# lijx10/USIP

Measured on AMD Instinct MI355X. Metric: point-clouds/sec detector fwd+bwd, higher is better.
Workload: dtype f32 results; matrix-bound products emulated from 2 fp16 planes per operand (22-bit operands, 3 plane products, exact ...; 1 GPU; KITTI detector N=16384 M=512 K=64 batch=8 pairs/GPU (BASELINE configs[2]); detector=RPN_Detector_Ball, clouds_per_gpu=16, surface_normal_len=4, node_knn_k_1=16, ball_radius=2, ball_k=64, cloud=slab, matmul=f32x2, step=fwd+losses+bwd+adam, launch=HIP graph replay (ONE graph per step: forward, backward, Adam), parallelism=dp1

## Files before the change

### include/usip_hip.h

```cpp
#ifndef USIP_HIP_H
#define USIP_HIP_H

#include <stdint.h>

#ifdef __cplusplus
extern "C" {
#endif

#define USIP_OK      0
#define USIP_EINVAL (-1)

const char* usip_version(void);

enum { USIP_TUNE_INDEX_MAX_CH = 0, USIP_TUNE_INDEX_MAX_UNROLL, USIP_TUNE_X3_WGRAD_TILE, USIP_TUNE_X3_GEMM_TILE,
       USIP_TUNE_GEMM_SPLIT3, USIP_TUNE_INDEX_MAX_THREADS, USIP_TUNE_X2_DIRECT, USIP_TUNE_R5_FORMS, USIP_TUNE_COUNT };
int usip_set_tuning(const char* name, int value);
int usip_tuning_value(int knob);

int usip_launch_log(int on);
const char* usip_launch_log_entry(int i, unsigned* workgroups);

int usip_index_max_f32(const float* data, const int32_t* index, int32_t* max_idx,
                       int B, int C, int N, int K, void* stream);
int usip_index_max_geometry(int B, int C, int N, int K, int* channel_rows, int* prefetch_depth, int* threads);

int usip_index_max_f32_cpu(const float* data, const int32_t* index, int32_t* max_idx,
                           int B, int C, int N, int K, int num_threads);

int usip_ball_query_f32(const float* dist, int32_t* out_idx, float radius, int K,
                        int B, int M, int N, void* stream);

int usip_ball_query_f32_cpu(const float* dist, int32_t* out_idx, float radius, int K, int B, int M, int N);

int usip_pairwise_dist_f32_cpu(const float* a, const float* x, float* dist, int B, int M, int N);
int usip_pairwise_dist_f32(const float* a, const float* x, float* dist,
                           int B, int M, int N, void* stream);

int usip_ball_query_coords_f32(const float* node, const float* x, int32_t* out_idx, float radius,
                               int K, int B, int M, int N, void* stream);

int usip_som_assign_f32(const float* x, const float* node, int32_t* min_idx,
                        int B, int N, int M, void* stream);

int usip_som_cluster_f32(const float* x, const int32_t* min_idx, float* cluster_mean,
                         int32_t* count, float* x_decentered, int B, int N, int M, void* stream);
int usip_som_cluster_csr_f32(const float* x, const int32_t* min_idx, const int32_t* start, const int32_t* perm,
                             float* cluster_mean, int32_t* count, float* x_decentered, int B, int N, int M,
                             void* stream);

int usip_index_max_values_f32(const float* data, const int32_t* index, const int32_t* count, int32_t* max_idx,
                              float* max_val, int B, int C, int Ctot, int N, int K, void* stream);
int usip_index_max_values_backward_add_f32(const float* g, const int32_t* max_idx, const int32_t* count, float* ddata,
                                           int B, int C, int Ctot, int coff, int N, int K, void* stream);
int usip_index_max_values_backward_f32(const float* g, const int32_t* max_idx, const int32_t* count,
                                       const int32_t* index, const float* src, int Csrc, int soff, float* dz,
                                       int B, int C, int N, int K, void* stream);

int usip_csr_by_index_i32(const int32_t* idx, int32_t* start, int32_t* perm, int B, int P, int N, void* stream);
int usip_segment_sum_supported(int N, int P);
int usip_segment_sum_f32(const float* src, const int32_t* start, const int32_t* perm, float* dx,
                         int B, int C, int N, int P, int Ctot, int coff, void* stream);

long long usip_nearest_workspace(int B, int Ma, int Nb);
int usip_nearest_f32(const float* a, const float* b, float* min_d, int32_t* arg,
                     float* ws_d, int32_t* ws_j, int B, int Ma, int Nb, void* stream);
int usip_nearest_backward_f32(const float* a, const float* b, const float* d, const int32_t* arg,
                              const float* gd, float* ga, float* gb, int B, int C, int Ma, int Nb, void* stream);

int usip_detector_head_f32(const float* ks, const float* centre, float sigma_lower_bound, float* keypoints,
                           float* sigmas, int B, int M, void* stream);
int usip_detector_head_backward_f32(const float* g_keypoints, const float* g_sigmas, const float* ks, float* g_ks,
                                    int B, int M, void* stream);
int usip_rigid_transform_f32(const float* x, const float* R, const float* scale, const float* shift, float* out,
                             int transpose, int B, int M, void* stream);
int usip_detector_loss_combine_f32(const float* d, const float* chamfer, float alpha, float* out3, long long half,
                                   void* stream);
int usip_fill_scaled_f32(const float* g, float factor, float* out, long long n, void* stream);

int usip_adam_step_f32(float* param, const float* grad, float* exp_avg, float* exp_avg_sq, float* step_count,
                       float lr, float beta1, float beta2, float eps, long long n, void* stream);
int usip_adam_step_hyper_f32(float* param, const float* grad, float* exp_avg, float* exp_avg_sq, float* step_count,
                             const float* hyper, long long n, void* stream);

int usip_bn_group_dy_sum_f32(const float* gsum0, const float* gsum1, const float* coef4, float* out,
                             int nb, int C, int G, int K, void* stream);

int usip_chamfer_prob_f32(const float* a, const int32_t* J, const float* c, const int32_t* I,
                          const float* sigma_src, const float* sigma_dst, float* out3,
                          int B, int M, int N, void* stream);
int usip_chamfer_prob_backward_f32(const float* gloss, const float* a, const int32_t* J, const float* c,
                                   const int32_t* I, const float* sigma_src, const float* sigma_dst,
                                   float* da, float* dc, float* dsigma_src, float* dsigma_dst,
                                   int B, int M, int N, void* stream);

int usip_nearest_nd_f32(const float* a, const float* b, float* min_d, int32_t* arg,
                        int B, int C, int Ma, int Nb, void* stream);

int usip_mlp_gemm_tiles(int M, int P, int nb);
int usip_mlp_gemm_f32(const float* At, int lda, const float* X, const float* X2, const float* coef,
                      int pro, const float* bias, const float* rowbias, int rb_group,
                      const float* pool_dp, const int32_t* pool_arg, int pool_group,
                      float* Y, int y_rows, float* stats, int M, int K, int P, int nb, void* stream);
int usip_mlp_gemm_bf16(const float* At, int lda, const float* X, const float* X2, const float* coef,
                       int pro, const float* bias, const float* rowbias, int rb_group,
                       const float* pool_dp, const int32_t* pool_arg, int pool_group,
                        float* Y, int y_rows, float* stats, int M, int K, int P, int nb, void* stream);
int usip_mlp_gemm_f32x3(const float* At, int lda, const float* X, const float* X2, const float* coef,
                       int pro, const float* bias, const float* rowbias, int rb_group,
                       const float* pool_dp, const int32_t* pool_arg, int pool_group,
                        float* Y, int y_rows, float* stats, int M, int K, int P, int nb, void* stream);
int usip_mlp_gemm_f32x3_used(int M, int K, int P, int nb);
int usip_mlp_narrow_forward_blocks(int M, int K, int P, int nb);
int usip_mlp_narrow_forward_f32(const float* At, int lda, const float* X, const float* coef, int pro,
                                const float* bias, const float* rowbias, int rb_group, float* Y, int y_rows,
                                float* stats, int M, int K, int P, int nb, void* stream);

int usip_mlp_x3p_tile_rows(int M, int P, int nb);
typedef struct usip_split3_desc {
    const float* At; void* planes; int32_t lda, M, K, first_block;
    int32_t tile_rows, reserved;
} usip_split3_desc;
int usip_mlp_split3_blocks(int M, int K, int tile_rows);
int usip_mlp_split3_multi_f32(const usip_split3_desc* descs_device, int n, int total_blocks, void* stream);
int usip_mlp_x3p_tile_cols(int M, int P, int nb, int pro, int with_stats);
long long usip_mlp_split3_bytes(int M, int K);
int usip_mlp_split3_f32(const float* At, int lda, int M, int K, int tile_rows, void* planes, void* stream);
int usip_mlp_gemm_x3p_f32(const void* planes, const float* X, const float* X2, const float* coef, int pro,
                          const float* bias, const float* rowbias, int rb_group, const float* pool_dp,
                          const int32_t* pool_arg, int pool_group, float* Y, int y_rows, float* stats,
                          int M, int K, int P, int nb, void* stream);
int usip_mlp_split2h_f32(const float* At, int lda, int M, int K, int tile_rows, void* planes, void* stream);
int usip_mlp_gemm_x2h_f32(const void* planes, const float* X, const float* X2, const float* coef, int pro,
                          const float* bias, const float* rowbias, int rb_group, const float* pool_dp,
                          const int32_t* pool_arg, int pool_group, float* Y, int y_rows, float* stats,
                          int M, int K, int P, int nb, void* stream);

int usip_mlp_gemm_x2d_red_tiles(int M, int K, int P, int nb, int red_group);
int usip_mlp_gemm_x2h_red_f32(const void* planes, const float* X, const float* X2, const float* coef, int pro,
                              const float* pool_dp, const int32_t* pool_arg, int pool_group, float* Y,
                              const float* red_y, const float* red_coef, float* red_out, float* red_gsum,
                              int red_group, int M, int K, int P, int nb, void* stream);
int usip_mlp_gemm_x2r_tiles(int P, int nb);
int usip_mlp_gemm_x2r_f32(const void* planes, const float* X, const float* X2, const float* coef, int pro,
                          const float* bias, const float* rowbias, int rb_group, const float* pool_dp,
                          const int32_t* pool_arg, int pool_group, float* Y, int y_rows, float* stats, int M, int K,
                          int P, int nb, void* stream);

int usip_multi_transpose_f32(const float* src, float* dst, const int32_t* table, int ntensors, int total_tiles,
                             void* stream);

int usip_bn_finalize_f32(const float* stats, int tiles, int C, long long count,
                         const float* gamma, const float* beta, float eps, float momentum,
                         float* running_mean, float* running_var, float* mean, float* invstd,
                         float* coef, void* stream);

int usip_bn_apply_f32(const float* Y, const float* coef, float* Z, int relu,
                      int nb, int C, int P, void* stream);

int usip_bn_backward_reduce_f32(const float* dZ, const float* Y, const float* coef_fwd,
                                const float* mean, const float* invstd, const float* gamma, int relu,
                                float* partial, float* dgamma, float* dbeta, float* coef4,
                                float* gsum, int group, int nb, int C, int P, int want_bound, void* stream);


int usip_bn_pool_backward_reduce_f32(const float* dpooled, const int32_t* arg, const float* Y, const float* yarg,
                                     const float* coef_fwd, const float* mean, const float* invstd,
                                     const float* gamma, int relu, float* partial, float* dgamma, float* dbeta,
                                     float* coef4, int nb, int C, int M, int K, int want_bound, void* stream);

long long usip_mlp_wgrad_workspace(int M, int N, int P, int nb);
int usip_mlp_wgrad_f32(const float* G, const float* G2, const float* coef, int pro, const float* X,
                       const float* xcoef, const float* pool_dp, const int32_t* pool_arg, int pool_group,
                       float* workspace, float* dW, int ldw, int coloff,
                       int M, int N, int P, int nb, void* stream);
int usip_wgrad_defer(int on);
int usip_wgrad_defer_on(void* stream);
int usip_wgrad_defer_hold(int hold);
int usip_wgrad_flush(void* stream);

int usip_mlp_narrow_backward_supported(int Cin, int Cout, int P);
long long usip_mlp_narrow_backward_workspace(int Cout, int P, int nb);
int usip_mlp_narrow_backward_blocks(int Cout, int P, int nb);
int usip_mlp_narrow_backward_f32(const float* dZ, const float* Y, const float* coef4, const float* X, int x_rows,
                                 const float* xcoef, const float* W, int ldw, float* dX, int dx_rows,
                                 float* workspace, float* dW, int lddw, float* red_partial, int Cin, int Cout,
                                 int P, int nb, void* stream);

int usip_mlp_layer_backward_x2h_supported(int Cin, int Cout, int P, int pooled);
long long usip_mlp_layer_backward_x2h_workspace(int Cin, int Cout, int P, int nb);
int usip_mlp_layer_backward_x2h_blocks(int Cin, int Cout, int P, int nb);
int usip_mlp_layer_backward_x2h_f32(const float* dZ, const float* Y, const float* coef4, const float* pool_dp,
                                    const int32_t* pool_arg, int pool_group, const float* X, int x_rows,
                                    const float* xcoef, const void* planes, float* dX, int dx_rows, float* workspace,
                                    float* dW, int lddw, float* red_partial, float* group_sums, int Cin, int Cout,
                                    int P, int nb, void* stream);
int usip_mlp_layer_backward_x2h_ws_f32(const float* dZ, const float* Y, const float* coef4, const float* X, int x_rows,
                                       const float* xcoef, const void* planes, float* dX, int dx_rows, float* workspace,
                                       float* dW, int lddw, float* red_partial, const float* wsrc, int ws_rows,
                                       float* wsum, float* wsum3, int Cin, int Cout, int P, int nb, void* stream);
int usip_mlp_wsum_finalize_f32(const float* wsum, const float* wsum3, int blocks, int C, const float* coef4,
                               const float* mean, int ws_rows, float* dW, int lddw, void* stream);
int usip_bn_backward_finalize_f32(const float* partial, int rows, int C, long long count, const float* coef_fwd,
                                  const float* mean, const float* invstd, float* dgamma, float* dbeta, float* coef4,
                                  void* stream);
int usip_bn_backward_finalize_max_f32(const float* partial, int rows, int C, long long count, const float* coef_fwd,
                                      const float* mean, const float* invstd, float* dgamma, float* dbeta,
                                      float* coef4, const float* max0, int n0, const float* max1, int n1, void* stream);
int usip_mlp_wgrad_bf16(const float* G, const float* G2, const float* coef, int pro, const float* X,
                        const float* xcoef, const float* pool_dp, const int32_t* pool_arg, int pool_group,
                        float* workspace, float* dW, int ldw, int coloff,
                        int M, int N, int P, int nb, void* stream);
int usip_mlp_wgrad_f32x3(const float* G, const float* G2, const float* coef, int pro, const float* X,
                        const float* xcoef, const float* pool_dp, const int32_t* pool_arg, int pool_group,
                        float* workspace, float* dW, int ldw, int coloff,
                        int M, int N, int P, int nb, void* stream);
int usip_mlp_wgrad_x2h_f32(const float* G, const float* G2, const float* coef, int pro, const float* X,
                        const float* xcoef, const float* pool_dp, const int32_t* pool_arg, int pool_group,
                        float* workspace, float* dW, int ldw, int coloff,
                        int M, int N, int P, int nb, void* stream);
int usip_mlp_wgrad_f32x3_used(int M, int N, int P, int nb);

int usip_group_gather_f32(const float* x, const int32_t* idx, const float* sub, float* out,
                          int B, int C, int N, int M, int K, int nsub, int Ctot, int coff, void* stream);
int usip_group_gather_backward_f32(const float* dout, const int32_t* idx, float* dx,
                                   int B, int C, int N, int M, int K, int Ctot, int coff, void* stream);
int usip_group_max_f32(const float* z, float* pooled, int32_t* arg, long long rows, int K, void* stream);
int usip_group_max_act_f32(const float* y, const float* coef, int relu, float* pooled, int32_t* arg, float* yarg,
                           int B, int C, int M, int K, void* stream);
int usip_group_max_backward_f32(const float* dpooled, const int32_t* arg, float* dz,
                                long long rows, int K, void* stream);
int usip_group_max_backward_add_f32(const float* dpooled, const int32_t* arg, float* dz,
                                    long long rows, int K, void* stream);

int usip_knn_f32(const float* query, const float* database, int32_t* idx,
                 int B, int M, int N, int K, void* stream);

int usip_knn_layer_supported(int N, int M, int K);
int usip_knn_layer_forward_f32(const float* U, const float* W, int ldw, const float* database, const float* query,
                               const int32_t* idx, float* Y, float* stats, int B, int Cout, int N, int M, int K,
                               void* stream);
int usip_knn_layer_backward_f32(const float* dZ, const float* Y, const float* coef4, int relu, const float* dcoord,
                                const int32_t* start, const int32_t* perm, float* dU, float* dWc_part,
                                int B, int Cout, int N, int M, int K, void* stream);

int usip_knn_points_f32(const float* node, const float* x, int32_t* idx, int B, int M, int N, int K, void* stream);

int usip_fps_f32(const float* pts, const int32_t* first_idx, int32_t* out_idx, int B, int n, int k, void* stream);

int usip_nms_f32(const float* keypoints, const float* sigmas, float radius, int32_t* order, int32_t* count,
                 int B, int M, void* stream);

#define USIP_PAIRS_NPARAM 24
typedef struct usip_pairs_recipe {
    double aug_scale_lo, aug_scale_hi;
    double shift_range;
    double height_lo, height_hi;
    double pc_sigma, pc_clip;
    double sn_sigma, sn_clip;
    double node_sigma, node_clip;
    double pert_sigma, pert_clip;
    double dst_scale_thre, dst_shift_thre;
    int N, M, Cs, n_sub, row_len;
    int sn_last;
    int train;
    int rot_horizontal, rot_3d, rot_perturbation, translation_perturbation;
    int height_scaling;
    int enu_to_cam;
    int require_full;
    int dst_rot_type;
    int dst_rot_perturbation;
} usip_pairs_recipe;
typedef struct usip_pairs_draws {
    const int32_t* rows;
    const int32_t* cand;
    const int32_t* first;
    const double* jit_pc;
    const double* jit_sn;
    const double* jit_node;
    const double* params;
} usip_pairs_draws;
typedef struct usip_pairs_out {
    float* pc[2];
    float* sn[2];
    float* node[2];
    float* R;
    float* scale;
    float* shift;
    int32_t* rows;
    int32_t* node_slots;
} usip_pairs_out;
long long usip_pairs_workspace_bytes(const usip_pairs_recipe* recipe, int P);
long long usip_pairs_workspace_offset(const usip_pairs_recipe* recipe, int P, int part);
int usip_pairs_build_f32(const usip_pairs_recipe* recipe, const float* bank, const int64_t* offsets, int num_scans,
                         const int32_t* scan_ids, int P, long long min_rows, uint64_t seed, uint64_t step,
// ... 247 lines not shown
```

### usip_amd/_lib.py

```python
import ctypes
import os

_HERE = os.path.dirname(os.path.abspath(__file__))
LIB_PATH = os.environ.get("USIP_LIB") or os.path.join(_HERE, "libusip_hip.so")
ABI = 6
_lib = None

_f32p = ctypes.c_void_p
_i32p = ctypes.c_void_p
_int = ctypes.c_int
_flt = ctypes.c_float
_dbl = ctypes.c_double
_stream = ctypes.c_void_p

SIGNATURES = {
    "usip_version": ([], ctypes.c_char_p),
    "usip_set_tuning": ([ctypes.c_char_p, _int], _int),
    "usip_tuning_value": ([_int], _int),
    "usip_launch_log": ([_int], _int),
    "usip_launch_log_entry": ([_int, ctypes.POINTER(ctypes.c_uint)], ctypes.c_char_p),
    "usip_wgrad_defer": ([_int], _int),
    "usip_wgrad_defer_on": ([_stream], _int),
    "usip_wgrad_defer_hold": ([_int], _int),
    "usip_wgrad_flush": ([_stream], _int),
    "usip_index_max_f32": ([_f32p, _i32p, _i32p, _int, _int, _int, _int, _stream], _int),
    "usip_index_max_geometry": ([_int, _int, _int, _int] + [ctypes.POINTER(_int)] * 3, _int),
    "usip_index_max_f32_cpu": ([_f32p, _i32p, _i32p, _int, _int, _int, _int, _int], _int),
    "usip_ball_query_f32": ([_f32p, _i32p, _flt, _int, _int, _int, _int, _stream], _int),
    "usip_ball_query_f32_cpu": ([_f32p, _i32p, _flt, _int, _int, _int, _int], _int),
    "usip_pairwise_dist_f32_cpu": ([_f32p, _f32p, _f32p, _int, _int, _int], _int),
    "usip_pairwise_dist_f32": ([_f32p, _f32p, _f32p, _int, _int, _int, _stream], _int),
    "usip_som_assign_f32": ([_f32p, _f32p, _i32p, _int, _int, _int, _stream], _int),
    "usip_som_cluster_f32": ([_f32p, _i32p, _f32p, _i32p, _f32p, _int, _int, _int, _stream], _int),
    "usip_som_cluster_csr_f32": ([_f32p, _i32p, _i32p, _i32p, _f32p, _i32p, _f32p, _int, _int, _int, _stream], _int),
    "usip_index_max_values_f32": ([_f32p, _i32p, _i32p, _i32p, _f32p, _int, _int, _int, _int, _int, _stream], _int),
    "usip_index_max_values_backward_add_f32": ([_f32p, _i32p, _i32p, _f32p, _int, _int, _int, _int, _int, _int,
                                                _stream], _int),
    "usip_index_max_values_backward_f32": ([_f32p, _i32p, _i32p, _i32p, _f32p, _int, _int, _f32p, _int, _int, _int, _int,
                                            _stream], _int),
    "usip_mlp_narrow_forward_blocks": ([_int, _int, _int, _int], _int),
    "usip_mlp_narrow_forward_f32": ([_f32p, _int, _f32p, _f32p, _int, _f32p, _f32p, _int, _f32p, _int, _f32p, _int, _int,
                                     _int, _int, _stream], _int),
    "usip_detector_head_f32": ([_f32p, _f32p, _flt, _f32p, _f32p, _int, _int, _stream], _int),
    "usip_detector_head_backward_f32": ([_f32p, _f32p, _f32p, _f32p, _int, _int, _stream], _int),
    "usip_rigid_transform_f32": ([_f32p, _f32p, _f32p, _f32p, _f32p, _int, _int, _int, _stream], _int),
    "usip_detector_loss_combine_f32": ([_f32p, _f32p, _flt, _f32p, ctypes.c_longlong, _stream], _int),
    "usip_fill_scaled_f32": ([_f32p, _flt, _f32p, ctypes.c_longlong, _stream], _int),
    "usip_mlp_split3_blocks": ([_int, _int, _int], _int),
    "usip_mlp_split3_multi_f32": ([ctypes.c_void_p, _int, _int, _stream], _int),
    "usip_bn_group_dy_sum_f32": ([_f32p, _f32p, _f32p, _f32p, _int, _int, _int, _int, _stream], _int),
    "usip_csr_by_index_i32": ([_i32p, _i32p, _i32p, _int, _int, _int, _stream], _int),
    "usip_segment_sum_supported": ([_int, _int], _int),
    "usip_segment_sum_f32": ([_f32p, _i32p, _i32p, _f32p, _int, _int, _int, _int, _int, _int, _stream], _int),
    "usip_nearest_backward_f32": ([_f32p, _f32p, _f32p, _i32p, _f32p, _f32p, _f32p, _int, _int, _int, _int, _stream],
                                  _int),
    "usip_nearest_nd_f32": ([_f32p, _f32p, _f32p, _i32p, _int, _int, _int, _int, _stream], _int),
    "usip_chamfer_prob_f32": ([_f32p, _i32p, _f32p, _i32p, _f32p, _f32p, _f32p, _int, _int, _int, _stream], _int),
    "usip_chamfer_prob_backward_f32": ([_f32p, _f32p, _i32p, _f32p, _i32p, _f32p, _f32p, _f32p, _f32p, _f32p, _f32p,
                                        _int, _int, _int, _stream], _int),
    "usip_nearest_workspace": ([_int, _int, _int], ctypes.c_longlong),
    "usip_nearest_f32": ([_f32p, _f32p, _f32p, _i32p, _f32p, _i32p, _int, _int, _int, _stream], _int),
    "usip_mlp_gemm_tiles": ([_int, _int, _int], _int),
    "usip_mlp_gemm_f32": ([_f32p, _int, _f32p, _f32p, _f32p, _int, _f32p, _f32p, _int, _f32p, _i32p, _int,
                           _f32p, _int, _f32p, _int, _int, _int, _int, _stream], _int),
    "usip_mlp_gemm_bf16": ([_f32p, _int, _f32p, _f32p, _f32p, _int, _f32p, _f32p, _int, _f32p, _i32p, _int,
                            _f32p, _int, _f32p, _int, _int, _int, _int, _stream], _int),
    "usip_mlp_gemm_f32x3": ([_f32p, _int, _f32p, _f32p, _f32p, _int, _f32p, _f32p, _int, _f32p, _i32p, _int,
                             _f32p, _int, _f32p, _int, _int, _int, _int, _stream], _int),
    "usip_mlp_gemm_f32x3_used": ([_int, _int, _int, _int], _int),
    "usip_mlp_x3p_tile_rows": ([_int, _int, _int], _int),
    "usip_mlp_x3p_tile_cols": ([_int, _int, _int, _int, _int], _int),
    "usip_mlp_split3_bytes": ([_int, _int], ctypes.c_longlong),
    "usip_mlp_split3_f32": ([_f32p, _int, _int, _int, _int, ctypes.c_void_p, _stream], _int),
    "usip_mlp_gemm_x3p_f32": ([ctypes.c_void_p, _f32p, _f32p, _f32p, _int, _f32p, _f32p, _int, _f32p, _i32p, _int,
                               _f32p, _int, _f32p, _int, _int, _int, _int, _stream], _int),
    "usip_mlp_gemm_x2r_tiles": ([_int, _int], _int),
    "usip_mlp_gemm_x2r_f32": ([ctypes.c_void_p, _f32p, _f32p, _f32p, _int, _f32p, _f32p, _int, _f32p, _i32p, _int, _f32p,
                               _int, _f32p, _int, _int, _int, _int, _stream], _int),
    "usip_mlp_split2h_f32": ([_f32p, _int, _int, _int, _int, ctypes.c_void_p, _stream], _int),
    "usip_mlp_gemm_x2h_f32": ([ctypes.c_void_p, _f32p, _f32p, _f32p, _int, _f32p, _f32p, _int, _f32p, _i32p, _int,
                               _f32p, _int, _f32p, _int, _int, _int, _int, _stream], _int),
    "usip_mlp_gemm_x2d_red_tiles": ([_int, _int, _int, _int, _int], _int),
    "usip_mlp_gemm_x2h_red_f32": ([ctypes.c_void_p, _f32p, _f32p, _f32p, _int, _f32p, _i32p, _int, _f32p, _f32p, _f32p, _f32p,
                                   _f32p, _int, _int, _int, _int, _int, _stream], _int),
    "usip_mlp_wgrad_f32x3_used": ([_int, _int, _int, _int], _int),
    "usip_bn_pool_backward_reduce_f32": ([_f32p, _i32p, _f32p, _f32p, _f32p, _f32p, _f32p, _f32p, _int, _f32p, _f32p,
                                          _f32p, _f32p, _int, _int, _int, _int, _int, _stream], _int),
    "usip_bn_finalize_f32": ([_f32p, _int, _int, ctypes.c_longlong, _f32p, _f32p, _flt, _flt, _f32p, _f32p, _f32p,
                              _f32p, _f32p, _stream], _int),
    "usip_bn_apply_f32": ([_f32p, _f32p, _f32p, _int, _int, _int, _int, _stream], _int),
    "usip_bn_backward_reduce_f32": ([_f32p, _f32p, _f32p, _f32p, _f32p, _f32p, _int, _f32p, _f32p, _f32p, _f32p,
                                     _f32p, _int, _int, _int, _int, _int, _stream], _int),
    "usip_mlp_wgrad_workspace": ([_int, _int, _int, _int], ctypes.c_longlong),
    "usip_mlp_wgrad_f32": ([_f32p, _f32p, _f32p, _int, _f32p, _f32p, _f32p, _i32p, _int, _f32p, _f32p, _int, _int,
                            _int, _int, _int, _int, _stream], _int),
    "usip_mlp_wgrad_bf16": ([_f32p, _f32p, _f32p, _int, _f32p, _f32p, _f32p, _i32p, _int, _f32p, _f32p, _int, _int,
                             _int, _int, _int, _int, _stream], _int),
    "usip_mlp_wgrad_f32x3": ([_f32p, _f32p, _f32p, _int, _f32p, _f32p, _f32p, _i32p, _int, _f32p, _f32p, _int, _int,
                              _int, _int, _int, _int, _stream], _int),
    "usip_mlp_wgrad_x2h_f32": ([_f32p, _f32p, _f32p, _int, _f32p, _f32p, _f32p, _i32p, _int, _f32p, _f32p, _int, _int,
                                _int, _int, _int, _int, _stream], _int),
    "usip_mlp_narrow_backward_supported": ([_int, _int, _int], _int),
    "usip_mlp_narrow_backward_workspace": ([_int, _int, _int], ctypes.c_longlong),
    "usip_mlp_narrow_backward_blocks": ([_int, _int, _int], _int),
    "usip_mlp_layer_backward_x2h_supported": ([_int, _int, _int, _int], _int),
    "usip_mlp_layer_backward_x2h_workspace": ([_int, _int, _int, _int], ctypes.c_longlong),
    "usip_mlp_layer_backward_x2h_blocks": ([_int, _int, _int, _int], _int),
    "usip_mlp_layer_backward_x2h_f32": ([_f32p, _f32p, _f32p, _f32p, _i32p, _int, _f32p, _int, _f32p, ctypes.c_void_p,
                                         _f32p, _int, _f32p, _f32p, _int, _f32p, _f32p, _int, _int, _int, _int, _stream],
                                        _int),
    "usip_mlp_layer_backward_x2h_ws_f32": ([_f32p, _f32p, _f32p, _f32p, _int, _f32p, ctypes.c_void_p, _f32p, _int, _f32p,
                                            _f32p, _int, _f32p, _f32p, _int, _f32p, _f32p, _int, _int, _int, _int, _stream],
                                           _int),
    "usip_mlp_wsum_finalize_f32": ([_f32p, _f32p, _int, _int, _f32p, _f32p, _int, _f32p, _int, _stream], _int),
    "usip_mlp_narrow_backward_f32": ([_f32p, _f32p, _f32p, _f32p, _int, _f32p, _f32p, _int, _f32p, _int, _f32p, _f32p,
                                      _int, _f32p, _int, _int, _int, _int, _stream], _int),
    "usip_bn_backward_finalize_f32": ([_f32p, _int, _int, ctypes.c_longlong, _f32p, _f32p, _f32p, _f32p, _f32p, _f32p,
                                       _stream], _int),
    "usip_bn_backward_finalize_max_f32": ([_f32p, _int, _int, ctypes.c_longlong, _f32p, _f32p, _f32p, _f32p, _f32p, _f32p,
                                           _f32p, _int, _f32p, _int, _stream], _int),
    "usip_group_max_act_f32": ([_f32p, _f32p, _int, _f32p, _i32p, _f32p, _int, _int, _int, _int, _stream], _int),
    "usip_group_gather_f32": ([_f32p, _i32p, _f32p, _f32p, _int, _int, _int, _int, _int, _int, _int, _int,
                               _stream], _int),
    "usip_group_gather_backward_f32": ([_f32p, _i32p, _f32p, _int, _int, _int, _int, _int, _int, _int, _stream], _int),
    "usip_group_max_f32": ([_f32p, _f32p, _i32p, ctypes.c_longlong, _int, _stream], _int),
    "usip_group_max_backward_f32": ([_f32p, _i32p, _f32p, ctypes.c_longlong, _int, _stream], _int),
    "usip_group_max_backward_add_f32": ([_f32p, _i32p, _f32p, ctypes.c_longlong, _int, _stream], _int),
    "usip_multi_transpose_f32": ([_f32p, _f32p, _i32p, _int, _int, _stream], _int),
    "usip_adam_step_f32": ([_f32p, _f32p, _f32p, _f32p, _f32p, _flt, _flt, _flt, _flt, ctypes.c_longlong, _stream], _int),
    "usip_adam_step_hyper_f32": ([_f32p, _f32p, _f32p, _f32p, _f32p, _f32p, ctypes.c_longlong, _stream], _int),
    "usip_knn_f32": ([_f32p, _f32p, _i32p, _int, _int, _int, _int, _stream], _int),
    "usip_knn_points_f32": ([_f32p, _f32p, _i32p, _int, _int, _int, _int, _stream], _int),
    "usip_knn_layer_supported": ([_int, _int, _int], _int),
    "usip_knn_layer_forward_f32": ([_f32p, _f32p, _int, _f32p, _f32p, _i32p, _f32p, _f32p, _int, _int, _int, _int, _int,
                                    _stream], _int),
    "usip_knn_layer_backward_f32": ([_f32p, _f32p, _f32p, _int, _f32p, _i32p, _i32p, _f32p, _f32p, _int, _int, _int, _int,
                                     _int, _stream], _int),
    "usip_fps_f32": ([_f32p, _i32p, _i32p, _int, _int, _int, _stream], _int),
    "usip_nms_f32": ([_f32p, _f32p, _flt, _i32p, _i32p, _int, _int, _stream], _int),
    "usip_ball_query_coords_f32": ([_f32p, _f32p, _i32p, _flt, _int, _int, _int, _int, _stream], _int),
    "usip_pairs_workspace_bytes": ([ctypes.c_void_p, _int], ctypes.c_longlong),
    "usip_pairs_workspace_offset": ([ctypes.c_void_p, _int, _int], ctypes.c_longlong),
    "usip_pairs_build_f32": ([ctypes.c_void_p, _f32p, ctypes.c_void_p, _int, _i32p, _int, ctypes.c_longlong,
                              ctypes.c_uint64, ctypes.c_uint64, ctypes.c_longlong, ctypes.c_void_p, ctypes.c_void_p,
                              _stream], _int),
    "usip_pairs_apply_f32": ([ctypes.c_void_p, ctypes.c_void_p, _f32p, ctypes.c_void_p, _int, _i32p, _int,
                              ctypes.c_longlong, ctypes.c_void_p, ctypes.c_void_p, _stream], _int),
    "usip_pairs_build_f32_cpu": ([ctypes.c_void_p, ctypes.c_void_p, _f32p, ctypes.c_void_p, _int, _i32p, _int,
                                  ctypes.c_uint64, ctypes.c_uint64, ctypes.c_longlong, ctypes.c_void_p], _int),
    "usip_ransac_trials_f32": ([_f32p, _f32p, _i32p, _int, _int, _int, _dbl, ctypes.c_uint64, ctypes.c_void_p, _i32p,
                                ctypes.c_void_p, _i32p, _stream], _int),
    "usip_ransac_trials_explicit_f32": ([_f32p, _f32p, _i32p, _int, _int, _int, _dbl, _i32p, _i32p, ctypes.c_void_p,
                                         _stream], _int),
    "usip_ransac_select_f32": ([_f32p, _f32p, _i32p, _int, _int, _int, _int, _dbl, ctypes.c_uint64, ctypes.c_void_p,
                                _i32p, _i32p] + [ctypes.c_void_p] * 9 + [_stream], _int),
    "usip_compare_transform_f64": ([ctypes.c_void_p] * 2 + [_int] + [ctypes.c_void_p] * 2 + [_stream], _int),
    "usip_repeatability_f32": ([_f32p, _i32p, _f32p, _i32p, ctypes.c_void_p, _dbl, _int, _int, _int, ctypes.c_void_p,
                                _i32p, ctypes.c_void_p, _stream], _int),
    "usip_nearest_nd_counted_f32": ([_f32p, _f32p, _i32p, _i32p, _f32p, _i32p, _int, _int, _int, _int, _stream], _int),
    "usip_ransac_trials_f32_cpu": ([_f32p, _f32p, _i32p, _int, _int, _int, _dbl, ctypes.c_uint64, ctypes.c_void_p, _i32p,
                                    _i32p, ctypes.c_void_p, _i32p, _int], _int),
    "usip_ransac_select_f32_cpu": ([_f32p, _f32p, _i32p, _int, _int, _int, _int, _dbl, ctypes.c_uint64, ctypes.c_void_p,
                                    _i32p, _i32p] + [ctypes.c_void_p] * 9, _int),
    "usip_compare_transform_f64_cpu": ([ctypes.c_void_p] * 2 + [_int] + [ctypes.c_void_p] * 2, _int),
    "usip_repeatability_f32_cpu": ([_f32p, _i32p, _f32p, _i32p, ctypes.c_void_p, _dbl, _int, _int, _int, ctypes.c_void_p,
                                    _i32p, ctypes.c_void_p], _int),
    "usip_nearest_nd_counted_f32_cpu": ([_f32p, _f32p, _i32p, _i32p, _f32p, _i32p, _int, _int, _int, _int], _int),
    "usip_scan_knn_f32": ([_f32p, _i32p, _int, _int, _i32p, _i32p, _stream], _int),
    "usip_scan_normals_f32": ([_f32p, _i32p, _int, _int, ctypes.c_void_p, ctypes.c_void_p, _f32p, _stream], _int),
    "usip_scan_voxel_keys_f32": ([_f32p, _int, _f32p, _dbl, ctypes.c_void_p, _stream], _int),
    "usip_scan_voxel_average_f32": ([_f32p, ctypes.c_void_p, _i32p, _i32p, _int, _int, _f32p, _stream], _int),
    "usip_scan_knn_f32_cpu": ([_f32p, _int, _int, _i32p, _int], _int),
    "usip_scan_normals_f32_cpu": ([_f32p, _i32p, _int, _int, ctypes.c_void_p, ctypes.c_void_p, _f32p], _int),
    "usip_scan_voxel_keys_f32_cpu": ([_f32p, _int, _f32p, _dbl, ctypes.c_void_p], _int),
    "usip_scan_voxel_average_f32_cpu": ([_f32p, ctypes.c_void_p, _i32p, _i32p, _int, _int, _f32p], _int),
    "usip_desc_pairs_workspace_bytes": ([ctypes.c_void_p, _int], ctypes.c_longlong),
    "usip_desc_pairs_workspace_offset": ([ctypes.c_void_p, _int, _int], ctypes.c_longlong),
    "usip_desc_pairs_build_f32": ([ctypes.c_void_p, ctypes.c_void_p, _i32p, _int, ctypes.c_uint64, ctypes.c_uint64,
                                   ctypes.c_longlong, ctypes.c_void_p, ctypes.c_void_p, _stream], _int),
    "usip_desc_pairs_apply_f32": ([ctypes.c_void_p, ctypes.c_void_p, ctypes.c_void_p, _i32p, _int, ctypes.c_void_p,
                                   ctypes.c_void_p, _stream], _int),
    "usip_desc_pairs_build_f32_cpu": ([ctypes.c_void_p, ctypes.c_void_p, ctypes.c_void_p, _i32p, _int, ctypes.c_uint64,
                                       ctypes.c_uint64, ctypes.c_longlong, ctypes.c_void_p], _int),
    "usip_knn_nd_counted_f32": ([_f32p, _f32p, _i32p, _i32p, _int, _f32p, _i32p, _i32p, _int, _int, _int, _int, _stream],
                                _int),
    "usip_match_union_i32": ([_i32p] * 4 + [_int] * 4 + [_i32p, _i32p, _stream], _int),
    "usip_information_f32": ([_f32p, ctypes.c_void_p, _int, _int, ctypes.c_void_p, _stream], _int),
    "usip_overlap_keys_f32": ([_f32p, _int, ctypes.c_void_p, _int, ctypes.c_longlong, _i32p, ctypes.c_void_p, _int, _int,
                               ctypes.c_void_p, _stream], _int),
    "usip_overlap_ratio_f32": ([_f32p, _int, ctypes.c_void_p, _int, ctypes.c_longlong, _i32p, _i32p, ctypes.c_void_p, _i32p,
                                _i32p, _int, _int, _dbl, _i32p, ctypes.c_void_p, _stream], _int),
    "usip_knn_nd_counted_f32_cpu": ([_f32p, _f32p, _i32p, _i32p, _int, _f32p, _i32p, _i32p, _int, _int, _int, _int, _int],
                                    _int),
    "usip_match_union_i32_cpu": ([_i32p] * 4 + [_int] * 4 + [_i32p, _i32p], _int),
    "usip_information_f32_cpu": ([_f32p, ctypes.c_void_p, _int, _int, ctypes.c_void_p], _int),
    "usip_overlap_keys_f32_cpu": ([_f32p, _int, ctypes.c_void_p, _int, ctypes.c_longlong, _i32p, ctypes.c_void_p, _int, _int,
                                   ctypes.c_void_p], _int),
    "usip_overlap_ratio_f32_cpu": ([_f32p, _int, ctypes.c_void_p, _int, ctypes.c_longlong, _i32p, _i32p, ctypes.c_void_p,
                                    _i32p, _i32p, _int, _int, _dbl, _int, _i32p, ctypes.c_void_p, _int], _int),
    "usip_iss_saliency_f32": ([_f32p, _i32p, _i32p, _int, _int, _dbl, _dbl, _dbl, _int, ctypes.c_void_p, _i32p, _i32p,
                               _stream], _int),
    "usip_iss_nms_f32": ([_f32p, _i32p, _i32p, ctypes.c_void_p, _int, _int, _dbl, _int, ctypes.c_void_p, _stream], _int),
    "usip_iss_saliency_f32_cpu": ([_f32p, _i32p, _int, _int, _dbl, _dbl, _dbl, _int, ctypes.c_void_p, _i32p, _int], _int),
    "usip_iss_nms_f32_cpu": ([_f32p, _i32p, ctypes.c_void_p, _int, _int, _dbl, _int, ctypes.c_void_p, _int], _int),
    "usip_fgr_tuples_f32": ([_f32p, _f32p] + [_i32p] * 4 + [_int, _int, ctypes.c_uint64, ctypes.c_void_p, _i32p, _i32p,
                            ctypes.c_void_p, _i32p, _i32p, _i32p, _i32p, _int, _stream], _int),
    "usip_fgr_tuples_explicit_f32": ([_f32p, _f32p] + [_i32p] * 4 + [_int, _int, _i32p, _int, _i32p, _i32p, ctypes.c_void_p,
                                     _i32p, _i32p, _i32p, _stream], _int),
    "usip_fgr_optimize_f32": ([_f32p, _f32p, _i32p, _i32p, ctypes.c_void_p, _i32p, _i32p, _int, _int, _dbl]
                              + [ctypes.c_void_p] * 3 + [_i32p, _stream], _int),
    "usip_fgr_tuples_f32_cpu": ([_f32p, _f32p] + [_i32p] * 4 + [_int, _int, ctypes.c_uint64, ctypes.c_void_p, _i32p, _int,
                                _i32p, _i32p, ctypes.c_void_p, _i32p, _i32p, _i32p, _i32p, _int, _int], _int),
    "usip_fgr_tuples_explicit_f32_cpu": ([_f32p, _f32p] + [_i32p] * 4 + [_int, _int, _i32p, _int, _i32p, _i32p,
                                         ctypes.c_void_p, _i32p, _i32p, _i32p, _int], _int),
    "usip_fgr_optimize_f32_cpu": ([_f32p, _f32p, _i32p, _i32p, ctypes.c_void_p, _i32p, _i32p, _int, _int, _dbl]
                                  + [ctypes.c_void_p] * 3 + [_i32p, _int], _int),
    "usip_fgr_sincos_f64_cpu": ([ctypes.c_void_p, _int, ctypes.c_void_p, ctypes.c_void_p], _int),
    "usip_icp_workspace_bytes": ([_int, _int], ctypes.c_longlong),
    "usip_icp_nearest_f32": ([_f32p, _int, ctypes.c_void_p, _int, ctypes.c_longlong, _i32p, _i32p, _i32p]
                             + [ctypes.c_void_p] * 2 + [_i32p, _int, _int, _i32p, ctypes.c_void_p, ctypes.c_void_p, _stream],
                             _int),
    "usip_icp_refine_f32": ([_f32p, _int, ctypes.c_void_p, _int, ctypes.c_longlong, _i32p, _i32p, _i32p]
                            + [ctypes.c_void_p] * 2 + [_i32p, _int, _int, _dbl, _int, _dbl, _dbl, _dbl, ctypes.c_void_p,
                                                       ctypes.c_longlong, ctypes.c_void_p, _i32p, ctypes.c_void_p,
                                                       ctypes.c_void_p, _i32p, ctypes.c_void_p, ctypes.c_void_p, _i32p,
                                                       ctypes.c_void_p, ctypes.c_void_p, _stream], _int),
    "usip_icp_nearest_f32_cpu": ([_f32p, _int, ctypes.c_void_p, _int, ctypes.c_longlong, _i32p, _i32p, _i32p]
                                 + [ctypes.c_void_p] * 2 + [_i32p, _int, _int, _i32p, ctypes.c_void_p, _int], _int),
    "usip_icp_refine_f32_cpu": ([_f32p, _int, ctypes.c_void_p, _int, ctypes.c_longlong, _i32p, _i32p, _i32p]
                                + [ctypes.c_void_p] * 2 + [_i32p, _int, _int, _dbl, _int, _dbl, _dbl, _dbl, ctypes.c_void_p,
                                                           _i32p, ctypes.c_void_p, ctypes.c_void_p, _i32p, ctypes.c_void_p,
                                                           ctypes.c_void_p, _i32p, _i32p, ctypes.c_void_p, _int], _int),
    "usip_icp_information_f32": ([_f32p, _int, ctypes.c_void_p, _int, ctypes.c_longlong, _i32p, _i32p, _i32p]
                                 + [ctypes.c_void_p] * 2 + [_int, _int, _dbl, ctypes.c_void_p, _i32p, _stream], _int),
    "usip_posegraph_workspace_bytes": ([_int, _int, _int], ctypes.c_longlong),
    "usip_posegraph_optimize_f64": ([_i32p] * 4 + [ctypes.c_void_p] * 3 + [_int, _int, _int, _dbl, _dbl, _int, _int,
                                                                           ctypes.c_void_p, ctypes.c_longlong]
# ... 80 lines not shown
```

### usip_amd/csrc/gemm_x2f.hip

```cpp
#include "mlp_common.h"
#include "split_common.h"
#include <type_traits>

using namespace usip_mlp;

namespace {

constexpr int FBM = 256, FBN = 256, FNT = 256, FSLOTS = 4;
constexpr int FPL = FBM * 32;
constexpr int FSTAGE = 2 * FPL;
constexpr int FTRS = 68;
constexpr int FSCR_FLOATS = 4 * 2 * 32 * FTRS + 2 * 4 * FBM;

__device__ __forceinline__ int f_lds_off(int row, int half) { return row * 32 + ((half ^ (row >> 3)) & 1) * 16; }

__device__ __forceinline__ void f_split_pair(float x, float y, unsigned& hi, unsigned& lo)
{
    const f32x2 v = {x, y};
    hi = __builtin_bit_cast(unsigned, __builtin_convertvector(v, f16x2));
    asm("v_fma_mixlo_f16 %0, %1, 1.0, -%2 op_sel_hi:[0,0,1]" : "=v"(lo) : "v"(x), "v"(hi));
    asm("v_fma_mixhi_f16 %0, %1, 1.0, -%2 op_sel:[0,0,1] op_sel_hi:[0,0,1]" : "+v"(lo) : "v"(y), "v"(hi));
}

typedef unsigned u32x4 __attribute__((ext_vector_type(4)));
typedef unsigned u32x2 __attribute__((ext_vector_type(2)));

__device__ __forceinline__ float f_aread(const f32x16& t, int r)
{
    float x;
    asm volatile("v_accvgpr_read_b32 %0, %1" : "=v"(x) : "a"(t[r]));
    return x;
}

__device__ __forceinline__ void stats_flush_x2f(const GemmArgs& a, const float* scratch, int m0, int tn128, int tpc128)
{
    const float* red = scratch + 4 * 2 * 32 * FTRS;
    const int tid = threadIdx.x;
    const long long ntn = (long long)a.nb * tpc128;
#pragma unroll
    for (int hf = 0; hf < 2; ++hf) {
        const float s = red[(2 * hf) * FBM + tid] + red[(2 * hf + 1) * FBM + tid];
        const float q = red[4 * FBM + (2 * hf) * FBM + tid] + red[4 * FBM + (2 * hf + 1) * FBM + tid];
        a.stats[(long long)(m0 + tid) * ntn + tn128 + hf] = s;
        a.stats[ntn * a.M + (long long)(m0 + tid) * ntn + tn128 + hf] = q;
    }
}

template <int EPI, bool RB>
__device__ __forceinline__ void epilogue_x2f(const GemmArgs& a, f32x16 (&acc)[8][2], float out_scale, float* scratch,
                                             int b, int m0, int p0, int prev_m0, int prev_tn128, int tpc128)
{
    if (EPI != EPI_NONE && prev_tn128 >= 0) {
        stats_flush_x2f(a, scratch, prev_m0, prev_tn128, tpc128);
        asm volatile("s_waitcnt lgkmcnt(0)" ::: "memory");
        __builtin_amdgcn_s_barrier();
        asm volatile("" ::: "memory");
    }
    const int tid = threadIdx.x, lane = tid & 63, c = lane & 31, half = lane >> 5;
    const int wave = __builtin_amdgcn_readfirstlane(tid >> 6);
    float* tr = scratch + wave * (2 * 32 * FTRS);
    float* red = scratch + 4 * 2 * 32 * FTRS;
    const int pw = p0 + wave * 64;
    const int rr = lane >> 4, cc = lane & 15;
    const __amdgpu_buffer_rsrc_t rY = __builtin_amdgcn_make_buffer_rsrc(
        (void*)(a.Y + (long long)b * a.y_rows * a.P), 0, (unsigned)a.y_rows * (unsigned)a.P * 4u, 0x00020000);
    const int st_voff = ((m0 + rr) * a.P + pw + 4 * cc) * 4;
    float* const trw = tr + c * FTRS + 8 * half;
    const float* const trr = tr + rr * FTRS + 4 * cc;
    const int ngrp = RB ? a.P / a.rb_group : 0;
    int grp[4];
#pragma unroll
    for (int g = 0; g < 4; ++g) grp[g] = RB ? (pw + 16 * g + 8 * half) / a.rb_group : 0;
    const float* rbp = RB ? a.rowbias + ((long long)b * a.M + m0 + c) * ngrp : nullptr;
    const float* biasp = a.bias ? a.bias + m0 + c : nullptr;
    const f32x2 os2 = {out_scale, out_scale};
    auto produce = [&](int i) {
#if defined(USIP_X2F_EXP) && USIP_X2F_EXP == 2
        return;
#endif
        const float bv = biasp ? biasp[i * 32] : 0.0f;
        float rb[4] = {0.f, 0.f, 0.f, 0.f};
        if (RB) {
#pragma unroll
            for (int g = 0; g < 4; ++g) rb[g] = rbp[(long long)i * 32 * ngrp + grp[g]];
        }
        f32x2 s2g[4], q2g[4];
        float* w = trw + (i & 1) * (32 * FTRS);
#pragma unroll
        for (int g = 0; g < 4; ++g) {
            f32x2 u[4];
#pragma unroll
            for (int e = 0; e < 4; ++e) {
#if defined(USIP_X2F_EXP) && USIP_X2F_EXP == 3
#pragma unroll
                for (int bk = 0; bk < 2; ++bk) {
                    float t = __builtin_fmaf(f_aread(acc[i][bk], 4 * g + e), out_scale, bv);
                    if (RB) t += rb[g];
                    u[e][bk] = t;
                }
                if (EPI == EPI_STATS) {
                    s2g[g] = (e == 0) ? u[e] : s2g[g] + u[e];
                    q2g[g] = (e == 0) ? u[e] * u[e] : __builtin_elementwise_fma(u[e], u[e], q2g[g]);
                }
                continue;
#endif
                const f32x2 av = {f_aread(acc[i][0], 4 * g + e), f_aread(acc[i][1], 4 * g + e)};
                u[e] = __builtin_elementwise_fma(av, os2, (f32x2){bv, bv});
                if (RB) u[e] = u[e] + (f32x2){rb[g], rb[g]};
                if (EPI == EPI_STATS) {
                    s2g[g] = (e == 0) ? u[e] : s2g[g] + u[e];
                    q2g[g] = (e == 0) ? u[e] * u[e] : __builtin_elementwise_fma(u[e], u[e], q2g[g]);
                }
            }
            *reinterpret_cast<float4*>(w + 16 * g) = make_float4(u[0][0], u[0][1], u[1][0], u[1][1]);
            *reinterpret_cast<float4*>(w + 16 * g + 4) = make_float4(u[2][0], u[2][1], u[3][0], u[3][1]);
        }
        if (EPI != EPI_NONE) {
            const f32x2 s2 = (s2g[0] + s2g[1]) + (s2g[2] + s2g[3]), q2 = (q2g[0] + q2g[1]) + (q2g[2] + q2g[3]);
            float s = s2[0] + s2[1], q = q2[0] + q2[1];
            s += __shfl_xor(s, 32);
            q += __shfl_xor(q, 32);
            if (half == 0) { red[wave * FBM + i * 32 + c] = s; red[4 * FBM + wave * FBM + i * 32 + c] = q; }
        }
    };
    produce(0);
#pragma unroll
    for (int i = 0; i < 8; ++i) {
        asm volatile("s_waitcnt lgkmcnt(0)" ::: "memory");
        float4 w[8];
        const float* r = trr + (i & 1) * (32 * FTRS);
#pragma unroll
        for (int k = 0; k < 8; ++k) w[k] = *reinterpret_cast<const float4*>(r + 4 * k * FTRS);
        __builtin_amdgcn_sched_barrier(0);
        if (i < 7) produce(i + 1);
        __builtin_amdgcn_sched_barrier(0);
#pragma unroll
        for (int k = 0; k < 8; ++k) {
            const u32x4 d = {__float_as_uint(w[k].x), __float_as_uint(w[k].y), __float_as_uint(w[k].z), __float_as_uint(w[k].w)};
#if defined(USIP_X2F_EXP) && USIP_X2F_EXP == 1
            asm volatile("" ::"v"(d));
#else
            __builtin_amdgcn_raw_buffer_store_b128(d, rY, st_voff, (i * 32 + 4 * k) * a.P * 4, st_aux<ST_X2F_FWD>());
#endif
        }
        asm volatile("s_nop 7" ::: "memory");
        __builtin_amdgcn_sched_barrier(0);
    }
}

__device__ __forceinline__ void epilogue_x2f_direct(const GemmArgs& a, f32x16 (&acc)[8][2], float out_scale, int b, int m0, int p0)
{
    const int tid = threadIdx.x, lane = tid & 63, c = lane & 31, half = lane >> 5;
    const int wave = __builtin_amdgcn_readfirstlane(tid >> 6);
    const __amdgpu_buffer_rsrc_t rY = __builtin_amdgcn_make_buffer_rsrc(
        (void*)(a.Y + (long long)b * a.y_rows * a.P), 0, (unsigned)a.y_rows * (unsigned)a.P * 4u, 0x00020000);
    const int voff = ((m0 + 4 * half) * a.P + p0 + wave * 64 + 2 * c) * 4;
    const int rowb = a.P * 4;
#pragma unroll
    for (int i = 0; i < 8; ++i) {
#pragma unroll
        for (int g = 0; g < 4; ++g) {
            u32x2 v[4];
#pragma unroll
            for (int e = 0; e < 4; ++e)
                v[e] = u32x2{__float_as_uint(f_aread(acc[i][0], 4 * g + e) * out_scale),
                             __float_as_uint(f_aread(acc[i][1], 4 * g + e) * out_scale)};
#pragma unroll
            for (int e = 0; e < 4; ++e)
                __builtin_amdgcn_raw_buffer_store_b64(v[e], rY, voff, (i * 32 + 8 * g + e) * rowb, st_aux<ST_X2F_DGRAD>());
            asm volatile("s_nop 7" ::: "memory");
            __builtin_amdgcn_sched_barrier(0);
        }
    }
}

__host__ __device__ constexpr int f_ns(int sl) { return (sl % 6) >= 2 ? (sl / 6) * 4 + (sl % 6) - 2 : -1; }

#ifdef USIP_X2F_TRACE
}
__device__ unsigned g_x2f_trace[8 * 4 * 128];
extern "C" int usip_x2f_trace_read(void* dst, void* stream)
{
    return (int)hipMemcpyFromSymbolAsync(dst, HIP_SYMBOL(g_x2f_trace), sizeof(unsigned) * 8 * 4 * 128, 0, hipMemcpyDeviceToDevice,
                                         (hipStream_t)stream);
}
namespace {
#define X2F_TP(REG_, IDX_)                                                                                      \
    {                                                                                                           \
        unsigned long long tt_;                                                                                 \
        asm volatile("s_memtime %0\n\ts_waitcnt lgkmcnt(0)" : "=&s"(tt_)::"memory");                            \
        unsigned keep_;                                                                                         \
        asm volatile("s_mov_b32 %1, m0\n\ts_mov_b32 m0, %3\n\ts_nop 0\n\tv_writelane_b32 %0, %2, m0\n\ts_mov_b32 m0, %1" \
                     : "+v"(REG_), "=&s"(keep_) : "s"((unsigned)tt_), "s"((int)(IDX_)));                        \
    }
#else
#define X2F_TP(REG_, IDX_)
#endif

template <int PRO, int EPI, bool DIRECT>
__global__ __launch_bounds__(FNT) __attribute__((amdgpu_waves_per_eu(1, 1))) void gemm_x2f_kernel(
    const GemmArgs a, const uint4* __restrict__ planes)
{
    constexpr bool POOL = (PRO == PRO_BN_BWD_POOL);
    constexpr bool TWO = (PRO == PRO_BN_BWD) || POOL;
    constexpr int NC = TWO ? 4 : 2;
    constexpr int KMAX = TWO ? 512 : 640;
    constexpr int KPAD = KMAX + 16;
    constexpr int RING = FSLOTS * FSTAGE;
    constexpr int SCR = DIRECT ? 64 : FSCR_FLOATS * 4;
    __shared__ __attribute__((aligned(16))) unsigned char smem[RING + SCR + NC * KPAD * 4];
    float* scr = reinterpret_cast<float*>(smem + RING);
    float* cf = reinterpret_cast<float*>(smem + RING + SCR);

    const int tid = threadIdx.x, lane = tid & 63, c = lane & 31, h = lane >> 5;
    const int wave = __builtin_amdgcn_readfirstlane(tid >> 6);

    const int tpc = a.P / FBN, nmt = a.M / FBM;
    const int total = a.nb * tpc * nmt;
    const int nk = a.K / XBK;

    float xs, out_scale;
    {
        float* redm = scr;
        float bnd = 0.f;
        if (PRO == PRO_AFFINE_RELU) {
            const float rn = sqrtf((float)a.nb * (float)a.P);
            for (int k = tid; k < a.K; k += FNT) {
                const float c0 = a.coef[k], c1 = a.coef[a.K + k], mu = a.coef[2 * a.K + k], is = a.coef[3 * a.K + k];
                bnd = fmaxf(bnd, fabsf(c0) / is * rn + fabsf(__builtin_fmaf(mu, c0, c1)));
            }
        } else {
            for (int i = tid; i < (a.K + 63) / 64; i += FNT) bnd = fmaxf(bnd, a.coef[4 * a.K + i]);
        }
#pragma unroll
        for (int off = 32; off > 0; off >>= 1) bnd = fmaxf(bnd, __shfl_xor(bnd, off));
        if (lane == 0) redm[wave] = bnd;
        __syncthreads();
        bnd = fmaxf(fmaxf(redm[0], redm[1]), fmaxf(redm[2], redm[3]));
        xs = pow2_scale(bnd, X2H_TOP);
        const float ws = __uint_as_float(planes[(long long)nmt * nk * (FSTAGE / 16)].x);
        out_scale = __uint_as_float(__builtin_amdgcn_readfirstlane(__float_as_uint(1.0f / (xs * ws))));
        for (int i = tid; i < nk * XBK * NC; i += FNT) {
            const int k = i / NC, j = i % NC;
            cf[i] = a.coef[j * a.K + k] * xs;
        }
        __syncthreads();
    }

    typedef int v4i32 __attribute__((ext_vector_type(4)));
    auto make_rsrc = [](const void* base, unsigned bytes) {
        const unsigned long long p = (unsigned long long)reinterpret_cast<uintptr_t>(base);
        return v4i32{(int)__builtin_amdgcn_readfirstlane((unsigned)p),
                     (int)__builtin_amdgcn_readfirstlane((unsigned)(p >> 32) & 0xffffu),
                     (int)__builtin_amdgcn_readfirstlane(bytes), 0x00020000};
    };
    const v4i32 rAv = make_rsrc(planes, (unsigned)nmt * (unsigned)nk * FSTAGE);
    const int a_voff = wave * 4096 + lane * 16;
    const unsigned ring_lds = (unsigned)reinterpret_cast<uintptr_t>((__attribute__((address_space(3))) unsigned char*)smem);
    const int pgrp = POOL ? a.P / a.pool_group : 0;
    const unsigned x_bytes = (unsigned)a.nb * (unsigned)a.K * (unsigned)a.P * 4u;
    const unsigned pool_bytes = (unsigned)a.nb * (unsigned)a.K * (unsigned)pgrp * 4u;
    const int rs = a.P * 4, rsg = pgrp * 4;
    const __amdgpu_buffer_rsrc_t rX = __builtin_amdgcn_make_buffer_rsrc((void*)(POOL ? a.X2 : a.X), 0, x_bytes, 0x00020000);
    const __amdgpu_buffer_rsrc_t rX2 = __builtin_amdgcn_make_buffer_rsrc((void*)(TWO ? a.X2 : a.X), 0, x_bytes, 0x00020000);
    const __amdgpu_buffer_rsrc_t rPd = __builtin_amdgcn_make_buffer_rsrc((void*)(POOL ? a.pool_dp : a.X), 0,
                                                                         POOL ? pool_bytes : 4u, 0x00020000);
    const __amdgpu_buffer_rsrc_t rPa = __builtin_amdgcn_make_buffer_rsrc((void*)(POOL ? (const float*)a.pool_arg : a.X), 0,
                                                                         POOL ? pool_bytes : 4u, 0x00020000);
    const int pl = wave * 64 + 2 * c;
    int xv[8], gv[POOL ? 8 : 1];
#pragma unroll
    for (int i = 0; i < 8; ++i) {
        xv[i] = pl * 4 + (h * 8 + i) * rs;
        if (POOL) gv[POOL ? i : 0] = (pl / a.pool_group) * 4 + (h * 8 + i) * rsg;
    }
    const int xkin = POOL ? pl % a.pool_group : 0;

    struct XSet { f32x2 rx[POOL ? 1 : 8]; float rd[POOL ? 8 : 1]; int rarg[POOL ? 8 : 1]; f32x2 ry[TWO ? 8 : 1]; };
    struct Frag { f16x8 lo, hi; };
    constexpr int NX = POOL ? 24 : (TWO ? 16 : 8);
    constexpr int BARRIER_VMCNT = 2 * NX + 4;
    static_assert(BARRIER_VMCNT <= 63, "vmcnt is six bits");

    const int fa0 = f_lds_off(c, h);
    const float4* cfl = reinterpret_cast<const float4*>(cf) + h * (8 * NC / 4);

    struct Tile { int b, m0, p0, tn128; int xo, go, wo; };
    auto tile_of = [&](int v) {
        int L = v;
        if ((total & 7) == 0) L = (v & 7) * (total >> 3) + (v >> 3);
        const int mt = L % nmt, tn = L / nmt;
        const int b = tn / tpc, pt = tn % tpc;
        const int p0 = pt * FBN;
        return Tile{b, mt * FBM, p0, (b * tpc + pt) * 2, (b * a.K * a.P + p0) * 4,
                    POOL ? (b * a.K * pgrp + p0 / a.pool_group) * 4 : 0, mt * nk * FSTAGE};
    };

    XSet xs0, xs1;
    auto dma_pair = [&](int wo, int kt, int pair) {
        const unsigned dst = ring_lds + (unsigned)((kt & (FSLOTS - 1)) * FSTAGE) + (unsigned)(wave * 4096) + (unsigned)(pair * 2048);
        unsigned keep;
        asm volatile("s_mov_b32 %0, m0\n\ts_mov_b32 m0, %1\n\ts_nop 0\n\t"
                     "buffer_load_dwordx4 %2, %3, %4 offen lds\n\t"
                     "buffer_load_dwordx4 %2, %3, %4 offen offset:1024 lds\n\t"
                     "s_mov_b32 m0, %0"
                     : "=&s"(keep) : "s"(dst), "v"(a_voff), "s"(rAv), "s"(wo + kt * FSTAGE + pair * 2048) : "memory");
    };
    auto load_x1 = [&](int so, int sg, XSet& S, int i) {
        if (POOL) {
            S.rd[POOL ? i : 0] = __builtin_bit_cast(float, __builtin_amdgcn_raw_buffer_load_b32(rPd, gv[POOL ? i : 0], sg, 0));
            S.rarg[POOL ? i : 0] = (int)__builtin_amdgcn_raw_buffer_load_b32(rPa, gv[POOL ? i : 0], sg, 0);
        } else {
            S.rx[POOL ? 0 : i] = __builtin_bit_cast(f32x2, __builtin_amdgcn_raw_buffer_load_b64(rX, xv[i], so, st_aux<(PRO >= PRO_BN_BWD) ? LD_X2F_DGRAD : LD_X2F_FWD>()));
        }
        if (TWO) S.ry[TWO ? i : 0] = __builtin_bit_cast(f32x2, __builtin_amdgcn_raw_buffer_load_b64(rX2, xv[i], so, st_aux<LD_X2F_DGRAD>()));
    };

    float4 cq[TWO ? 8 : 4];
    float cv[2][8];
    auto cf_read = [&](int kt, int i) { cq[i] = cfl[kt * (XBK * NC / 4) + i]; };
    auto conv_blk = [&](const XSet& S, int i, int bk) {
        if (TWO) {
            const float4 c4 = cq[TWO ? i : 0];
            float x;
            if (POOL) x = (S.rarg[POOL ? i : 0] == xkin + bk) ? S.rd[POOL ? i : 0] : 0.f;
            else x = S.rx[POOL ? 0 : i][bk];
            cv[bk][i] = pro_apply<PRO_BN_BWD>(x, S.ry[TWO ? i : 0][bk], c4.x, c4.y, c4.z, c4.w);
        } else {
            const float4 c4 = cq[TWO ? 0 : i / 2];
            cv[bk][i] = (i & 1) ? pro_apply<PRO_AFFINE_RELU>(S.rx[POOL ? 0 : i][bk], 0.f, c4.z, c4.w, 0.f, 0.f)
                                : pro_apply<PRO_AFFINE_RELU>(S.rx[POOL ? 0 : i][bk], 0.f, c4.x, c4.y, 0.f, 0.f);
        }
    };
    auto convert_all = [&](int kt, const XSet& S, unsigned (&ph)[2][4], unsigned (&pl_)[2][4]) {
#pragma unroll
        for (int i = 0; i < (TWO ? 8 : 4); ++i) cf_read(kt, i);
#pragma unroll
        for (int i = 0; i < 8; ++i) { conv_blk(S, i, 0); conv_blk(S, i, 1); }
#pragma unroll
        for (int bk = 0; bk < 2; ++bk)
#pragma unroll
            for (int j = 0; j < 4; ++j) f_split_pair(cv[bk][2 * j], cv[bk][2 * j + 1], ph[bk][j], pl_[bk][j]);
    };

    f32x16 acc[8][2];
    Frag FA, FB;
    auto read_frag = [&](int kt, int t, int which, Frag& F) {
        const unsigned char* As = smem + (kt & (FSLOTS - 1)) * FSTAGE + fa0 + t * 1024;
        if (which == 0) F.lo = *reinterpret_cast<const f16x8*>(As + FPL);
        else F.hi = *reinterpret_cast<const f16x8*>(As);
    };

    auto stage = [&](auto first_tag, int kt, int k1, int k3, int xo3, int go3, int wo3, XSet& S, const unsigned (&chh)[2][4],
                     const unsigned (&cll)[2][4], unsigned (&nh)[2][4], unsigned (&nl)[2][4]) {
        constexpr bool FIRST = decltype(first_tag)::value;
        const f16x8 xh0 = __builtin_bit_cast(f16x8, make_uint4(chh[0][0], chh[0][1], chh[0][2], chh[0][3]));
        const f16x8 xh1 = __builtin_bit_cast(f16x8, make_uint4(chh[1][0], chh[1][1], chh[1][2], chh[1][3]));
        const f16x8 xl0 = __builtin_bit_cast(f16x8, make_uint4(cll[0][0], cll[0][1], cll[0][2], cll[0][3]));
        const f16x8 xl1 = __builtin_bit_cast(f16x8, make_uint4(cll[1][0], cll[1][1], cll[1][2], cll[1][3]));
        const int so3 = xo3 + k3 * (XBK * rs), sg3 = go3 + k3 * (XBK * rsg);
        auto slot = [&](auto sl_tag) {
            constexpr int sl = decltype(sl_tag)::value;
            constexpr int t = sl / 6, i6 = sl % 6, bk = i6 & 1, prod = i6 / 2;
            if (sl == 42) {
                asm volatile("s_waitcnt vmcnt(%0) lgkmcnt(0)" ::"n"(BARRIER_VMCNT) : "memory");
                __builtin_amdgcn_s_barrier();
            }
            {
                Frag& F = (t & 1) ? FB : FA;
                const f16x8& x = (prod == 1) ? (bk ? xl1 : xl0) : (bk ? xh1 : xh0);
                const f16x8& f = (prod == 0) ? F.lo : F.hi;
                if constexpr (FIRST && prod == 0) {
                    if constexpr (DIRECT) asm volatile("v_mfma_f32_32x32x16_f16 %0, %2, %1, 0" : "=a"(acc[t][bk]) : "v"(x), "v"(f));
                    else asm volatile("v_mfma_f32_32x32x16_f16 %0, %1, %2, 0" : "=a"(acc[t][bk]) : "v"(x), "v"(f));
                } else {
                    if constexpr (DIRECT) asm volatile("v_mfma_f32_32x32x16_f16 %0, %2, %1, %0" : "+a"(acc[t][bk]) : "v"(x), "v"(f));
                    else asm volatile("v_mfma_f32_32x32x16_f16 %0, %1, %2, %0" : "+a"(acc[t][bk]) : "v"(x), "v"(f));
                }
            }
            if (i6 < 2) {
                if (t < 7) read_frag(kt, t + 1, i6, (t & 1) ? FA : FB);
                else read_frag(kt + 1, 0, i6, FA);
            }
            constexpr int ns = f_ns(sl);
            if (ns == 28) dma_pair(wo3, k3, 0);
            if (ns == 30) dma_pair(wo3, k3, 1);
            if (!TWO) {
                if (ns == 0) { cf_read(k1, 0); cf_read(k1, 1); cf_read(k1, 2); cf_read(k1, 3); }
#pragma unroll
                for (int j = 0; j < 4; ++j) {
                    const int base = 2 + 5 * j;
                    if (ns == base) { conv_blk(S, 2 * j, 0); conv_blk(S, 2 * j, 1); }
                    if (ns == base + 1) { conv_blk(S, 2 * j + 1, 0); conv_blk(S, 2 * j + 1, 1); }
                    if (ns == base + 2) {
                        f_split_pair(cv[0][2 * j], cv[0][2 * j + 1], nh[0][j], nl[0][j]);
                        load_x1(so3, sg3, S, 2 * j);
                    }
                    if (ns == base + 3) {
                        f_split_pair(cv[1][2 * j], cv[1][2 * j + 1], nh[1][j], nl[1][j]);
                        load_x1(so3, sg3, S, 2 * j + 1);
                    }
                }
            } else {
                if (ns == 0) { cf_read(k1, 0); cf_read(k1, 1); }
                if (ns == 1) { cf_read(k1, 2); cf_read(k1, 3); }
                if (ns == 8) cf_read(k1, 4);
                if (ns == 9) cf_read(k1, 5);
                if (ns == 14) cf_read(k1, 6);
                if (ns == 15) cf_read(k1, 7);
#pragma unroll
                for (int j = 0; j < 4; ++j) {
                    const int base = 2 + 6 * j;
                    if (ns == base) conv_blk(S, 2 * j, 0);
                    if (ns == base + 1) conv_blk(S, 2 * j, 1);
                    if (ns == base + 2) conv_blk(S, 2 * j + 1, 0);
                    if (ns == base + 3) conv_blk(S, 2 * j + 1, 1);
                    if (ns == base + 4) {
                        f_split_pair(cv[0][2 * j], cv[0][2 * j + 1], nh[0][j], nl[0][j]);
                        load_x1(so3, sg3, S, 2 * j);
                    }
                    if (ns == base + 5) {
                        f_split_pair(cv[1][2 * j], cv[1][2 * j + 1], nh[1][j], nl[1][j]);
                        load_x1(so3, sg3, S, 2 * j + 1);
                    }
                }
            }
            __builtin_amdgcn_sched_barrier(0);
        };
#define USIP_X2F_SLOT(N_) slot(std::integral_constant<int, N_>{});
#define USIP_X2F_SLOT6(N_) USIP_X2F_SLOT(N_) USIP_X2F_SLOT(N_ + 1) USIP_X2F_SLOT(N_ + 2) USIP_X2F_SLOT(N_ + 3) USIP_X2F_SLOT(N_ + 4) USIP_X2F_SLOT(N_ + 5)
        USIP_X2F_SLOT6(0) USIP_X2F_SLOT6(6) USIP_X2F_SLOT6(12) USIP_X2F_SLOT6(18)
        USIP_X2F_SLOT6(24) USIP_X2F_SLOT6(30) USIP_X2F_SLOT6(36) USIP_X2F_SLOT6(42)
#undef USIP_X2F_SLOT6
#undef USIP_X2F_SLOT
    };

    [[maybe_unused]] unsigned trp = 0, trs = 0;
    [[maybe_unused]] int tix = 0;
    int v = blockIdx.x;
    if (v >= total) return;
    unsigned ah[2][4], al[2][4], bh[2][4], bl[2][4];
    Tile T = tile_of(v);
    {
#pragma unroll
        for (int st = 0; st < 3; ++st) { dma_pair(T.wo, st, 0); dma_pair(T.wo, st, 1); }
#pragma unroll
        for (int i = 0; i < 8; ++i) load_x1(T.xo, T.go, xs0, i);
#pragma unroll
        for (int i = 0; i < 8; ++i) load_x1(T.xo + XBK * rs, T.go + XBK * rsg, xs1, i);
        convert_all(0, xs0, ah, al);
#pragma unroll
        for (int i = 0; i < 8; ++i) load_x1(T.xo + 2 * XBK * rs, T.go + 2 * XBK * rsg, xs0, i);
        asm volatile("s_waitcnt vmcnt(%0)" ::"n"(2 * NX) : "memory");
        __builtin_amdgcn_s_barrier();
        read_frag(0, 0, 0, FA); read_frag(0, 0, 1, FA);
    }
    int prev_m0 = 0, prev_tn128 = -1;
    for (;;) {
        const int vn = v + (int)gridDim.x;
        const bool more = vn < total;
        const Tile Tn = more ? tile_of(vn) : T;
        X2F_TP(trp, tix * 8 + 0)
        stage(std::true_type{}, 0, 1, 3, T.xo, T.go, T.wo, xs1, ah, al, bh, bl);
        stage(std::false_type{}, 1, 2, 4 < nk ? 4 : 0, 4 < nk ? T.xo : Tn.xo, 4 < nk ? T.go : Tn.go, 4 < nk ? T.wo : Tn.wo,
              xs0, bh, bl, ah, al);
        X2F_TP(trp, tix * 8 + 1)
        X2F_TP(trp, tix * 8 + 2)
        for (int kt = 2; kt < nk; kt += 2) {
            const bool w3 = kt + 3 >= nk, w4 = kt + 4 >= nk;
            stage(std::false_type{}, kt, kt + 1, w3 ? kt + 3 - nk : kt + 3, w3 ? Tn.xo : T.xo, w3 ? Tn.go : T.go, w3 ? Tn.wo : T.wo,
                  xs1, ah, al, bh, bl);
#ifdef USIP_X2F_TRACE
            if (tix == 1 && kt < 64) X2F_TP(trs, kt)
#endif
            stage(std::false_type{}, kt + 1, kt + 2 >= nk ? 0 : kt + 2, w4 ? kt + 4 - nk : kt + 4, w4 ? Tn.xo : T.xo, w4 ? Tn.go : T.go,
                  w4 ? Tn.wo : T.wo, xs0, bh, bl, ah, al);
#ifdef USIP_X2F_TRACE
            if (tix == 1 && kt < 63) X2F_TP(trs, kt + 1)
#endif
        }
        X2F_TP(trp, tix * 8 + 3)
        X2F_TP(trp, tix * 8 + 4)
        asm volatile("s_nop 7\n\ts_nop 7\n\ts_nop 7" ::: "memory");
        __builtin_amdgcn_sched_barrier(0);
        X2F_TP(trp, tix * 8 + 5)
        if constexpr (DIRECT) epilogue_x2f_direct(a, acc, out_scale, T.b, T.m0, T.p0);
        else if (a.rowbias) epilogue_x2f<EPI, true>(a, acc, out_scale, scr, T.b, T.m0, T.p0, prev_m0, prev_tn128, tpc * 2);
        else epilogue_x2f<EPI, false>(a, acc, out_scale, scr, T.b, T.m0, T.p0, prev_m0, prev_tn128, tpc * 2);
        prev_m0 = T.m0;
        prev_tn128 = T.tn128;
        X2F_TP(trp, tix * 8 + 6)
#ifdef USIP_X2F_TRACE
        ++tix;
#endif
        if (!more) break;
        v = vn;
        T = Tn;
    }
    if constexpr (!DIRECT && EPI != EPI_NONE) {
        asm volatile("s_waitcnt lgkmcnt(0)" ::: "memory");
        __builtin_amdgcn_s_barrier();
        asm volatile("" ::: "memory");
        stats_flush_x2f(a, scr, prev_m0, prev_tn128, tpc * 2);
    }
    asm volatile("s_waitcnt vmcnt(0)" ::: "memory");
#ifdef USIP_X2F_TRACE
    if (blockIdx.x < 8) {
        g_x2f_trace[(blockIdx.x * 4 + wave) * 128 + lane] = trp;
        g_x2f_trace[(blockIdx.x * 4 + wave) * 128 + 64 + lane] = trs;
    }
#endif
}

}

namespace usip_mlp {

bool gemm_x2f_takes(const GemmArgs& a, int pro)
{
    const int knob = usip_tuning_value(USIP_TUNE_X2_DIRECT);
    if (knob != 0 && (knob < 13 || knob > 15)) return false;
    if ((knob == 13 && pro != PRO_AFFINE_RELU) || (knob == 14 && pro == PRO_BN_BWD) || (knob == 15 && pro == PRO_BN_BWD_POOL)) return false;
    if (pro != PRO_AFFINE_RELU && pro != PRO_BN_BWD && pro != PRO_BN_BWD_POOL) return false;
    if (a.red_out) return false;
    if (a.M % FBM != 0 || a.P % FBN != 0 || a.K % (4 * XBK) != 0) return false;
    if (a.K > (pro == PRO_AFFINE_RELU ? 640 : 512)) return false;
    if (!a.y_vec || (a.rowbias && a.rb_group % 8 != 0)) return false;
    if ((long long)a.y_rows * a.P * 4 >= (1LL << 31) || (long long)a.nb * a.K * a.P * 4 >= (1LL << 31)) return false;
    if ((reinterpret_cast<uintptr_t>(a.X) & 7u) != 0 || (reinterpret_cast<uintptr_t>(a.X2) & 7u) != 0) return false;
    if (pro == PRO_BN_BWD_POOL && (a.pool_group % 2 != 0 || FBN % a.pool_group != 0)) return false;
    if (pro != PRO_AFFINE_RELU && (a.stats || a.bias || a.rowbias)) return false;
    return true;
}

int launch_gemm_x2f(const GemmArgs& a_in, const uint4* pl, int pro, hipStream_t st)
{
    const GemmArgs& a = a_in;
    const int tpc = a.P / FBN, nmt = a.M / FBM;
    const long long total = (long long)a.nb * tpc * nmt;
    if (total > 0x7fffffffLL) return USIP_EINVAL;
    const int cus = usip_cu_count();
    const long long slots = (long long)cus / 8 * 8;
    dim3 grid((unsigned)((total <= slots || (total & 7)) ? total : slots)), block(FNT);
    if (pro == PRO_AFFINE_RELU) {
        if (a.stats) USIP_LAUNCH((gemm_x2f_kernel<PRO_AFFINE_RELU, EPI_STATS, false>), grid, block, 0, st, a, pl);
        else USIP_LAUNCH((gemm_x2f_kernel<PRO_AFFINE_RELU, EPI_NONE, false>), grid, block, 0, st, a, pl);
    } else if (pro == PRO_BN_BWD) {
        USIP_LAUNCH((gemm_x2f_kernel<PRO_BN_BWD, EPI_NONE, true>), grid, block, 0, st, a, pl);
    } else {
        USIP_LAUNCH((gemm_x2f_kernel<PRO_BN_BWD_POOL, EPI_NONE, true>), grid, block, 0, st, a, pl);
    }
    USIP_LAUNCH_CHECK();
    return USIP_OK;
}

}
```

### usip_amd/csrc/mlp_common.h

```cpp
#pragma once
#include "common.h"

typedef float f32x16 __attribute__((ext_vector_type(16)));

namespace usip_mlp {

enum { ST_NARROW_FWD = 1, ST_X2R = 2, ST_TILE_EPI = 4, ST_X2F_FWD = 8, ST_X2F_DGRAD = 16, ST_X2D = 32, ST_LAYER_BWD_DX = 64,
       ST_WGRAD_PART = 128, LD_WGRAD_G = 256, ST_TILE_EPI_PLAIN = 512, LD_LAYER_BWD_G = 1024, LD_X2F_FWD = 2048,
       LD_X2F_DGRAD = 4096, LD_NARROW_FWD = 8192, LD_X2R = 16384, LD_WGRAD_X = 32768, LD_WGRAD3_G = 65536,
       LD_X3P_FWD = 131072, LD_LAYER_BWD_X = 262144, LD_BN_REDUCE_Z = 524288, LD_BN_REDUCE_Y = 1048576, LD_WGRAD_GEN_G = 2097152, ST_X2R_PLAIN = 4194304 };
#ifndef USIP_ST_NT
#define USIP_ST_NT (ST_X2F_DGRAD | ST_WGRAD_PART | LD_WGRAD_G | LD_LAYER_BWD_G | LD_X2F_FWD)
#endif
template <int SITE> constexpr int st_aux() { return (USIP_ST_NT & SITE) ? 2 : 0; }
typedef float st_f4v __attribute__((ext_vector_type(4)));
template <int SITE>
__device__ __forceinline__ void st_out(float* p, float v)
{
    if (USIP_ST_NT & SITE) __builtin_nontemporal_store(v, p); else *p = v;
}
template <int SITE>
__device__ __forceinline__ float4 ld_in4(const float* p)
{
    if (USIP_ST_NT & SITE) {
        const st_f4v q = __builtin_nontemporal_load(reinterpret_cast<const st_f4v*>(p));
        return make_float4(q.x, q.y, q.z, q.w);
    }
    return *reinterpret_cast<const float4*>(p);
}
template <int SITE>
__device__ __forceinline__ void st_out4(float* p, float x, float y, float z, float w)
{
    if (USIP_ST_NT & SITE) { st_f4v q = {x, y, z, w}; __builtin_nontemporal_store(q, reinterpret_cast<st_f4v*>(p)); }
    else *reinterpret_cast<float4*>(p) = make_float4(x, y, z, w);
}

enum { PRO_NONE = 0, PRO_AFFINE_RELU = 1, PRO_BN_BWD = 2, PRO_BN_BWD_POOL = 3 };

struct GemmArgs {
    const float* At; int lda;
    const float* X;
    const float* X2;
    const float* coef;
    const float* bias;
    float* Y;
    float* stats;
    int M, K, P, nb;
    const float* rowbias; int rb_group;
    const float* pool_dp; const int* pool_arg; int pool_group;
    int a_trans;
    int y_rows;
    int y_vec;
    const float* red_y; const float* red_coef; float* red_out; float* red_gsum; int red_group;
};

template <int PRO>
__device__ __forceinline__ float pro_apply(float x, float x2, float c0, float c1, float c2, float c3)
{
    if (PRO == PRO_AFFINE_RELU) return fmaxf(__builtin_fmaf(x, c0, c1), 0.0f);
    if (PRO == PRO_BN_BWD) {
        const float dyh = (__builtin_fmaf(x2, c0, c1) > 0.0f) ? x : 0.0f;
        return __builtin_fmaf(c0, dyh, __builtin_fmaf(c2, x2, c3));
    }
    return x;
}

enum { EPI_NONE = 0, EPI_STATS = 1 };

template <int WM, int WN, int EPI, int TM = 2, int NJ = 2>
__device__ __forceinline__ void gemm_epilogue(const GemmArgs& a, f32x16 (&acc)[TM][NJ], float* scratch,
                                              int scratch_floats, int b, int m0, int p0, int tn, int tpc)
{
    constexpr int BM = WM * 32 * TM, BN = WN * 32 * NJ;
    const int tid = threadIdx.x, lane = tid & 63, c = lane & 31, half = lane >> 5;
    const int wave = __builtin_amdgcn_readfirstlane(tid >> 6);
    const int wm = wave / WN, wn = wave % WN;
    float* Yb = a.Y + (long long)b * a.y_rows * a.P;
    float* red = scratch;
    const int ngrp = a.rowbias ? a.P / a.rb_group : 0;
    float* rbs = red + 2 * WN * BM;
    const int g0 = a.rowbias ? p0 / a.rb_group : 0;
    const int G = a.rowbias ? (min(p0 + BN, a.P) - 1) / a.rb_group - g0 + 1 : 0;
    const bool rb_lds = a.rowbias && BM * G <= scratch_floats - 2 * WN * BM;
    if (rb_lds) {
        for (int e = tid; e < BM * G; e += 256) {
            const int rl = e / G, g = e % G;
            rbs[e] = (m0 + rl < a.M) ? a.rowbias[((long long)b * a.M + m0 + rl) * ngrp + g0 + g] : 0.f;
        }
        __syncthreads();
    }
    const bool run_one_group = a.rowbias && (a.rb_group % 4 == 0);
#pragma unroll
    for (int i = 0; i < TM; ++i) {
        const int row_l = (wm * TM + i) * 32 + c;
        const int row = m0 + row_l;
        const int rowc = min(row, a.M - 1);
        const bool rok = row < a.M;
        const float bv = a.bias ? a.bias[rowc] : 0.0f;
        float* yrow = Yb + (long long)rowc * a.P;
        float s = 0.f, q = 0.f;
#pragma unroll
        for (int j = 0; j < NJ; ++j) {
#pragma unroll
            for (int g = 0; g < 4; ++g) {
                const int pb = p0 + wn * (32 * NJ) + j * 32 + 8 * g + 4 * half;
                float v[4];
#pragma unroll
                for (int e = 0; e < 4; ++e) v[e] = acc[i][j][4 * g + e] + bv;
                if (a.rowbias) {
                    if (run_one_group) {
                        const int grp = min(pb, a.P - 1) / a.rb_group;
                        const float rb = rb_lds ? rbs[row_l * G + grp - g0]
                                                : a.rowbias[((long long)b * a.M + rowc) * ngrp + grp];
#pragma unroll
                        for (int e = 0; e < 4; ++e) v[e] += rb;
                    } else {
#pragma unroll
                        for (int e = 0; e < 4; ++e) {
                            const int grp = min(pb + e, a.P - 1) / a.rb_group;
                            v[e] += rb_lds ? rbs[row_l * G + grp - g0]
                                           : a.rowbias[((long long)b * a.M + rowc) * ngrp + grp];
                        }
                    }
                }
                if (rok) {
                    if (a.y_vec && pb + 3 < a.P) {
                        st_out4<(EPI == EPI_STATS) ? ST_TILE_EPI : ST_TILE_EPI_PLAIN>(yrow + pb, v[0], v[1], v[2], v[3]);
                        if (EPI == EPI_STATS) {
#pragma unroll
                            for (int e = 0; e < 4; ++e) { s += v[e]; q = __builtin_fmaf(v[e], v[e], q); }
                        }
                    } else {
#pragma unroll
                        for (int e = 0; e < 4; ++e)
                            if (pb + e < a.P) {
                                yrow[pb + e] = v[e];
                                if (EPI == EPI_STATS) { s += v[e]; q = __builtin_fmaf(v[e], v[e], q); }
                            }
                    }
                }
            }
        }
        if (EPI != EPI_NONE) {
            s += __shfl_xor(s, 32); q += __shfl_xor(q, 32);
            if (half == 0) {
                red[wn * BM + row_l] = s;
                red[WN * BM + wn * BM + row_l] = q;
            }
        }
    }
    if (EPI != EPI_NONE) {
        __syncthreads();
        if (tid < BM && m0 + tid < a.M) {
            float s = 0.f, q = 0.f;
#pragma unroll
            for (int w = 0; w < WN; ++w) { s += red[w * BM + tid]; q += red[WN * BM + w * BM + tid]; }
            const long long ntn = (long long)a.nb * tpc;
            a.stats[(long long)(m0 + tid) * ntn + tn] = s;
            a.stats[ntn * a.M + (long long)(m0 + tid) * ntn + tn] = q;
        }
    }
}

struct WgradArgs {
    const float* G;  const float* G2; const float* coef;
    const float* X;
    const float* xcoef;
    const float* pool_dp; const int* pool_arg; int pool_group;
    float* part;
    int M, N, P, nb, seglen, segs;
};

template <int N4, bool TWO, bool VEC, int Q4 = 8>
__device__ __forceinline__ void wgrad_load_rows(const float* __restrict__ base, const float* __restrict__ base2,
                                                int rows, int P, int r0, int p, int pend, int tid,
                                                float4 (&dst)[N4], float4 (&dst2)[TWO ? N4 : 1])
{
#pragma unroll
    for (int i = 0; i < N4; ++i) {
        const int f = tid + i * 256, row = f / Q4, kq = (f % Q4) * 4;
        float4 v = make_float4(0.f, 0.f, 0.f, 0.f), w = v;
        if (VEC) {
            const long long off = (long long)min(r0 + row, rows - 1) * P + min(p + kq, P - 4);
            if (TWO) {
                v = ld_in4<LD_WGRAD_GEN_G>(base + off);
                w = ld_in4<LD_WGRAD_GEN_G>(base2 + off);
            } else {
                v = *reinterpret_cast<const float4*>(base + off);
            }
        } else if (r0 + row < rows) {
            const long long off = (long long)(r0 + row) * P + p + kq;
            if (p + kq + 0 < pend) { v.x = base[off + 0]; if (TWO) w.x = base2[off + 0]; }
            if (p + kq + 1 < pend) { v.y = base[off + 1]; if (TWO) w.y = base2[off + 1]; }
            if (p + kq + 2 < pend) { v.z = base[off + 2]; if (TWO) w.z = base2[off + 2]; }
            if (p + kq + 3 < pend) { v.w = base[off + 3]; if (TWO) w.w = base2[off + 3]; }
        }
        dst[i] = v;
        if (TWO) dst2[i] = w;
    }
}

template <int TM, int TN>
__device__ __forceinline__ void wgrad_store_partial(const WgradArgs& a, f32x16 (&acc)[TM][TN], int slice,
                                                    int m0, int n0, int wm, int wn, int lane)
{
    float* out = a.part + (long long)slice * a.M * a.N;
// ... 30 lines not shown
```

### usip_amd/csrc/shared_mlp_x3.hip

```cpp
#include "mlp_common.h"
#include "split_common.h"
#include <type_traits>

using namespace usip_mlp;

namespace {

__device__ __forceinline__ int lds_off(int row, int half) { return row * 32 + ((half ^ (row >> 3)) & 1) * 16; }

constexpr int X2H_PARTS = 32;

__device__ __forceinline__ float* x2h_trailer(const usip_split3_desc& d)
{
    const int bm = d.tile_rows, ksteps = (d.K + XBK - 1) / XBK;
    return reinterpret_cast<float*>(reinterpret_cast<unsigned char*>(d.planes) +
                                    (long long)((d.M + bm - 1) / bm) * ksteps * 2 * bm * 32);
}

__device__ __forceinline__ void absmax_part(const usip_split3_desc& d, int part)
{
    __shared__ float red[4];
    const long long total = (long long)d.M * d.K, per = (total + X2H_PARTS - 1) / X2H_PARTS;
    const long long i0 = part * per, i1 = i0 + per < total ? i0 + per : total;
    float mx = 0.f;
// ... 989 lines not shown
    const int t = usip_tuning_value(USIP_TUNE_X3_GEMM_TILE);
    if (M <= 128 || t == 1) return 128;
    const long long wide = (long long)((M + 255) / 256) * nb * ((P + 127) / 128);
    return wide >= 256 ? 256 : 128;
}


extern "C" long long usip_mlp_split3_bytes(int M, int K)
{
    if (M < 1 || K < 1) return 0;
    const int bm = M > 128 ? 256 : 128;
    return (long long)((M + bm - 1) / bm) * ((K + XBK - 1) / XBK) * 3 * bm * 32;
}

extern "C" int usip_mlp_split3_f32(const float* At, int lda, int M, int K, int tile_rows, void* planes, void* stream)
{
    if (!At || !planes || M < 1 || K < 1 || lda < M || (reinterpret_cast<uintptr_t>(planes) & 15u)) return USIP_EINVAL;
    if (tile_rows != 128 && tile_rows != 256) return USIP_EINVAL;
    const int bm = tile_rows;
    const int ksteps = (K + XBK - 1) / XBK, mts = (M + bm - 1) / bm;
    USIP_LAUNCH(split3_tiles_kernel, dim3((unsigned)(mts * ksteps)), dim3(2 * bm), 0, (hipStream_t)stream, At, lda, M, K,
                reinterpret_cast<uint4*>(planes), ksteps, bm, 3);
    USIP_LAUNCH_CHECK();
    return USIP_OK;
}

extern "C" int usip_mlp_split2h_f32(const float* At, int lda, int M, int K, int tile_rows, void* planes, void* stream)
{
    if (!At || !planes || M < 1 || K < 1 || lda < M || (reinterpret_cast<uintptr_t>(planes) & 15u)) return USIP_EINVAL;
    if (tile_rows != 128 && tile_rows != 256) return USIP_EINVAL;
    const int bm = tile_rows;
    const int ksteps = (K + XBK - 1) / XBK, mts = (M + bm - 1) / bm;
    usip_split3_desc d{At, planes, lda, M, K, 0, bm, 2};
    USIP_LAUNCH(absmax_one_kernel, dim3(X2H_PARTS), dim3(256), 0, (hipStream_t)stream, d);
    USIP_LAUNCH_CHECK();
    USIP_LAUNCH(split3_tiles_kernel, dim3((unsigned)(mts * ksteps)), dim3(2 * bm), 0, (hipStream_t)stream, At, lda, M, K,
                reinterpret_cast<uint4*>(planes), ksteps, bm, 2);
    USIP_LAUNCH_CHECK();
    return USIP_OK;
}

extern "C" int usip_mlp_split3_blocks(int M, int K, int tile_rows)
{
    if (M < 1 || K < 1 || (tile_rows != 128 && tile_rows != 256)) return 0;
    const int bm = tile_rows;
    return ((M + bm - 1) / bm) * ((K + XBK - 1) / XBK);
}

extern "C" int usip_mlp_split3_multi_f32(const usip_split3_desc* descs_device, int n, int total_blocks, void* stream)
{
    if (n < 0 || total_blocks < 0) return USIP_EINVAL;
    if (n == 0 || total_blocks == 0) return USIP_OK;
    if (!descs_device) return USIP_EINVAL;
    USIP_LAUNCH(absmax_multi_kernel, dim3((unsigned)(n * X2H_PARTS)), dim3(256), 0, (hipStream_t)stream, descs_device, n);
    USIP_LAUNCH_CHECK();
    USIP_LAUNCH(split3_multi_kernel, dim3((unsigned)total_blocks), dim3(512), 0, (hipStream_t)stream, descs_device, n);
    USIP_LAUNCH_CHECK();
    return USIP_OK;
}

template <int TM, int WN, int NPL = 3>
static int launch_x3p(const GemmArgs& a, const uint4* pl, int pro, hipStream_t st)
{
    constexpr int BM = 64 * TM, BN = 64 * WN;
    const int tpc = (a.P + BN - 1) / BN, nmt = (a.M + BM - 1) / BM;
    const long long total = (long long)a.nb * tpc * nmt;
    if (total > 0x7fffffffLL) return USIP_EINVAL;
    const int epi = a.stats ? EPI_STATS : EPI_NONE;
    dim3 grid((unsigned)total), block(128 * WN);
    const bool deep = TM == 2 && !(usip_tuning_value(USIP_TUNE_R5_FORMS) & 32);
#define USIP_X3P_CASE(P_, E_)                                                                 \
    if (pro == P_ && epi == E_) {                                                             \
        if constexpr (TM == 2) {                                                              \
            if (deep) {                                                                       \
                USIP_LAUNCH((gemm_x3p_kernel<P_, E_, TM, WN, NPL, 3>), grid, block, 0, st, a, pl); \
                USIP_LAUNCH_CHECK();                                                          \
                return USIP_OK;                                                               \
            }                                                                                 \
        }                                                                                     \
        USIP_LAUNCH((gemm_x3p_kernel<P_, E_, TM, WN, NPL>), grid, block, 0, st, a, pl);       \
        USIP_LAUNCH_CHECK();                                                                  \
        return USIP_OK;                                                                       \
    }
    if constexpr (NPL == 3) {
        USIP_X3P_CASE(PRO_NONE, EPI_STATS)
        USIP_X3P_CASE(PRO_NONE, EPI_NONE)
    }
    USIP_X3P_CASE(PRO_AFFINE_RELU, EPI_STATS)
    USIP_X3P_CASE(PRO_AFFINE_RELU, EPI_NONE)
    USIP_X3P_CASE(PRO_BN_BWD, EPI_NONE)
    USIP_X3P_CASE(PRO_BN_BWD_POOL, EPI_NONE)
#undef USIP_X3P_CASE
    return USIP_EINVAL;
}

extern "C" int usip_mlp_x3p_tile_cols(int M, int P, int nb, int pro, int with_stats)
{
    if (usip_mlp_x3p_tile_rows(M, P, nb) == 128 || with_stats) return 128;
    const int knob = usip_tuning_value(USIP_TUNE_X3_GEMM_TILE);
    const long long wide_tiles = (long long)((M + 255) / 256) * ((P + 255) / 256) * nb;
    return (knob == 4 || (knob == 5 && pro >= 2 && wide_tiles >= 256)) ? 256 : 128;
}

extern "C" int usip_mlp_gemm_x3p_f32(const void* planes, const float* X, const float* X2, const float* coef, int pro,
                                     const float* bias, const float* rowbias, int rb_group, const float* pool_dp,
                                     const int32_t* pool_arg, int pool_group, float* Y, int y_rows, float* stats,
                                     int M, int K, int P, int nb, void* stream)
{
    if (M < 1 || K < 1 || K > 640 || P < 0 || nb < 0) return USIP_EINVAL;
    if ((pro == PRO_BN_BWD || pro == PRO_BN_BWD_POOL) && K > 512) return USIP_EINVAL;
    if ((long long)P * nb == 0) return USIP_OK;
    if (!planes || !Y || pro < 0 || pro > 3 || (reinterpret_cast<uintptr_t>(planes) & 15u)) return USIP_EINVAL;
    if (pro != PRO_BN_BWD_POOL && !X) return USIP_EINVAL;
    if (pro != PRO_NONE && !coef) return USIP_EINVAL;
    if ((pro == PRO_BN_BWD || pro == PRO_BN_BWD_POOL) && (!X2 || stats)) return USIP_EINVAL;
    if (pro == PRO_BN_BWD_POOL && (!pool_dp || !pool_arg || pool_group < 1 || P % pool_group != 0)) return USIP_EINVAL;
    if (rowbias && (rb_group < 1 || P % rb_group != 0)) return USIP_EINVAL;
    if (y_rows == 0) y_rows = M;
    if (y_rows < M) return USIP_EINVAL;
    GemmArgs a{nullptr, 0, X, X2, coef, bias, Y, stats, M, K, P, nb, rowbias, rb_group, pool_dp, pool_arg, pool_group,
               0, y_rows, (P % 4 == 0 && (reinterpret_cast<uintptr_t>(Y) & 15u) == 0) ? 1 : 0};
    hipStream_t st = (hipStream_t)stream;
    const uint4* pl = reinterpret_cast<const uint4*>(planes);
    if (usip_mlp_x3p_tile_rows(M, P, nb) == 128) return launch_x3p<2, 2>(a, pl, pro, st);
    if (usip_mlp_x3p_tile_cols(M, P, nb, pro, stats != nullptr) == 256) return launch_x3p<4, 4>(a, pl, pro, st);
    return launch_x3p<4, 2>(a, pl, pro, st);
}

extern "C" int usip_mlp_gemm_x2h_f32(const void* planes, const float* X, const float* X2, const float* coef, int pro,
                                     const float* bias, const float* rowbias, int rb_group, const float* pool_dp,
                                     const int32_t* pool_arg, int pool_group, float* Y, int y_rows, float* stats,
                                     int M, int K, int P, int nb, void* stream)
{
    if (M < 1 || K < 1 || K > 640 || P < 0 || nb < 0) return USIP_EINVAL;
    if (pro != PRO_AFFINE_RELU && pro != PRO_BN_BWD && pro != PRO_BN_BWD_POOL) return USIP_EINVAL;
    if ((pro == PRO_BN_BWD || pro == PRO_BN_BWD_POOL) && K > 512) return USIP_EINVAL;
    if ((long long)P * nb == 0) return USIP_OK;
    if (!planes || !Y || !coef || (reinterpret_cast<uintptr_t>(planes) & 15u)) return USIP_EINVAL;
    if (pro != PRO_BN_BWD_POOL && !X) return USIP_EINVAL;
    if ((pro == PRO_BN_BWD || pro == PRO_BN_BWD_POOL) && (!X2 || stats)) return USIP_EINVAL;
    if (pro == PRO_BN_BWD_POOL && (!pool_dp || !pool_arg || pool_group < 1 || P % pool_group != 0)) return USIP_EINVAL;
    if (rowbias && (rb_group < 1 || P % rb_group != 0)) return USIP_EINVAL;
    if (y_rows == 0) y_rows = M;
    if (y_rows < M) return USIP_EINVAL;
    GemmArgs a{nullptr, 0, X, X2, coef, bias, Y, stats, M, K, P, nb, rowbias, rb_group, pool_dp, pool_arg, pool_group,
               0, y_rows, (P % 4 == 0 && (reinterpret_cast<uintptr_t>(Y) & 15u) == 0) ? 1 : 0};
    hipStream_t st = (hipStream_t)stream;
    const uint4* pl = reinterpret_cast<const uint4*>(planes);
    if (usip_mlp_x3p_tile_rows(M, P, nb) == 128) return launch_x3p<2, 2, 2>(a, pl, pro, st);
    if (usip_mlp_x3p_tile_cols(M, P, nb, pro, stats != nullptr) == 256) return launch_x3p<4, 4, 2>(a, pl, pro, st);
    if ((usip_tuning_value(USIP_TUNE_X2_DIRECT) & 15) != 1 && (long long)K * P * 4 < (1LL << 31))
        return launch_gemm_x2d(a, pl, pro, st);
    return launch_x3p<4, 2, 2>(a, pl, pro, st);
}

extern "C" int usip_mlp_gemm_x2d_red_tiles(int M, int K, int P, int nb, int red_group)
{
    if (M < 256 || M % 256 || P < 128 || P % 128 || nb < 1 || K < 1 || K > 512) return 0;
    if (red_group != 0 && red_group != 16 && red_group != 32) return 0;
    if (usip_mlp_x3p_tile_rows(M, P, nb) != 256 || usip_mlp_x3p_tile_cols(M, P, nb, 2, 0) != 128) return 0;
    if ((usip_tuning_value(USIP_TUNE_X2_DIRECT) & 15) == 1 || (usip_tuning_value(USIP_TUNE_X2_DIRECT) & 15) == 8) return 0;
    if ((long long)K * P * 4 >= (1LL << 31) || (long long)M * P * 4 >= (1LL << 31)) return 0;
    return nb * (P / 128);
}

extern "C" int usip_mlp_gemm_x2h_red_f32(const void* planes, const float* X, const float* X2, const float* coef, int pro,
                                         const float* pool_dp, const int32_t* pool_arg, int pool_group, float* Y,
                                         const float* red_y, const float* red_coef, float* red_out, float* red_gsum,
                                         int red_group, int M, int K, int P, int nb, void* stream)
{
    if (pro != PRO_BN_BWD && pro != PRO_BN_BWD_POOL) return USIP_EINVAL;
    if (!usip_mlp_gemm_x2d_red_tiles(M, K, P, nb, red_gsum ? red_group : 0)) return USIP_EINVAL;
    if (!planes || !Y || !coef || !X2 || !red_y || !red_coef || !red_out || (reinterpret_cast<uintptr_t>(planes) & 15u))
        return USIP_EINVAL;
    if ((reinterpret_cast<uintptr_t>(Y) | reinterpret_cast<uintptr_t>(red_y)) & 15u) return USIP_EINVAL;
    if (pro == PRO_BN_BWD && !X) return USIP_EINVAL;
    if (pro == PRO_BN_BWD_POOL && (!pool_dp || !pool_arg || pool_group < 1 || P % pool_group != 0)) return USIP_EINVAL;
    GemmArgs a{nullptr, 0, X, X2, coef, nullptr, Y, nullptr, M, K, P, nb, nullptr, 1, pool_dp, pool_arg, pool_group,
               0, M, 1, red_y, red_coef, red_out, red_gsum, red_gsum ? red_group : 0};
    return launch_gemm_x2d(a, reinterpret_cast<const uint4*>(planes), pro, (hipStream_t)stream);
}

extern "C" int usip_mlp_gemm_x2r_tiles(int P, int nb)
{
    const long long total = (long long)nb * ((P + 63) / 64);
    return (int)(total < 512 ? total : 512);
}

extern "C" int usip_mlp_gemm_x2r_f32(const void* planes, const float* X, const float* X2, const float* coef, int pro,
                                     const float* bias, const float* rowbias, int rb_group, const float* pool_dp,
                                     const int32_t* pool_arg, int pool_group, float* Y, int y_rows, float* stats, int M,
                                     int K, int P, int nb, void* stream)
{
    if (rowbias && (pro != PRO_AFFINE_RELU || rb_group < 32 || rb_group % 32 != 0 || P % rb_group != 0)) return USIP_EINVAL;
    if (M < 1 || M > 128 || K < 1 || K > 128 || P < 0 || nb < 0) return USIP_EINVAL;
    if (pro != PRO_AFFINE_RELU && pro != PRO_BN_BWD && pro != PRO_BN_BWD_POOL) return USIP_EINVAL;
    if ((long long)P * nb == 0) return USIP_OK;
    if (!planes || !Y || !coef || (reinterpret_cast<uintptr_t>(planes) & 15u)) return USIP_EINVAL;
    if (pro != PRO_BN_BWD_POOL && !X) return USIP_EINVAL;
    if ((pro == PRO_BN_BWD || pro == PRO_BN_BWD_POOL) && (!X2 || stats)) return USIP_EINVAL;
    if (pro == PRO_BN_BWD_POOL && (!pool_dp || !pool_arg || pool_group < 1 || P % pool_group != 0)) return USIP_EINVAL;
    if ((long long)K * P >= (1LL << 30)) return USIP_EINVAL;
    if (y_rows == 0) y_rows = M;
    if (y_rows < M) return USIP_EINVAL;
    GemmArgs a{nullptr, 0, X, X2, coef, bias, Y, stats, M, K, P, nb, rowbias, rowbias ? rb_group : 1, pool_dp, pool_arg,
               pool_group, 0, y_rows, (P % 4 == 0 && (reinterpret_cast<uintptr_t>(Y) & 15u) == 0) ? 1 : 0};
    const long long total = (long long)nb * ((P + 63) / 64);
    const unsigned grid = (unsigned)(total < 512 ? total : 512);
    hipStream_t st = (hipStream_t)stream;
    const uint4* pl = reinterpret_cast<const uint4*>(planes);
    if (pro == PRO_AFFINE_RELU && rowbias) {
        if (stats) USIP_LAUNCH((gemm_x2r_kernel<PRO_AFFINE_RELU, EPI_STATS, true>), dim3(grid), dim3(256), 0, st, a, pl);
        else USIP_LAUNCH((gemm_x2r_kernel<PRO_AFFINE_RELU, EPI_NONE, true>), dim3(grid), dim3(256), 0, st, a, pl);
    } else if (pro == PRO_AFFINE_RELU) {
        if (stats) USIP_LAUNCH((gemm_x2r_kernel<PRO_AFFINE_RELU, EPI_STATS>), dim3(grid), dim3(256), 0, st, a, pl);
        else USIP_LAUNCH((gemm_x2r_kernel<PRO_AFFINE_RELU, EPI_NONE>), dim3(grid), dim3(256), 0, st, a, pl);
    } else if (pro == PRO_BN_BWD) {
        USIP_LAUNCH((gemm_x2r_kernel<PRO_BN_BWD, EPI_NONE>), dim3(grid), dim3(256), 0, st, a, pl);
    } else {
        USIP_LAUNCH((gemm_x2r_kernel<PRO_BN_BWD_POOL, EPI_NONE>), dim3(grid), dim3(256), 0, st, a, pl);
    }
    USIP_LAUNCH_CHECK();
    return USIP_OK;
}

namespace usip_mlp {

void wgrad_x3_plan(int M, int N, int P, int nb, int* seglen, int* segs, int* tiles)
{
    *tiles = ((M + 255) / 256) * ((N + 255) / 256);
    long long want = (usip_tuning_value(USIP_TUNE_X3_WGRAD_TILE) == 2 ? 512 : 256) / (*tiles);
    if (want < 1) want = 1;
    long long per_cloud = (want + nb - 1) / nb;
    if (per_cloud < 1) per_cloud = 1;
    long long sl = (P + per_cloud - 1) / per_cloud;
    sl = ((sl + 31) / 32) * 32;
    long long floor_sl = 512;
    if (usip_tuning_value(USIP_TUNE_X3_WGRAD_TILE) != 4)
        while (floor_sl > 128 && (long long)(*tiles) * nb * ((P + floor_sl - 1) / floor_sl) < 192) floor_sl /= 2;
    if (sl < floor_sl) sl = floor_sl;
    *seglen = (int)sl;
    *segs = (int)((P + sl - 1) / sl);
}

int launch_wgrad_x2h_256(const WgradArgs& a, int pro, unsigned blocks, hipStream_t st)
{
    dim3 grid(blocks), block(512);
    const bool line = !(usip_tuning_value(USIP_TUNE_R5_FORMS) & 1) &&
                      (long long)(a.M > a.N ? a.M : a.N) * a.P < (1LL << 30);
    if (line && pro == PRO_BN_BWD) { USIP_LAUNCH((wgrad_x2l_kernel<PRO_BN_BWD>), grid, block, 0, st, a); USIP_LAUNCH_CHECK(); return USIP_OK; }
    if (line && pro == PRO_BN_BWD_POOL) { USIP_LAUNCH((wgrad_x2l_kernel<PRO_BN_BWD_POOL>), grid, block, 0, st, a); USIP_LAUNCH_CHECK(); return USIP_OK; }
    if (pro == PRO_BN_BWD) USIP_LAUNCH((wgrad_x3_kernel<PRO_BN_BWD, true, 2>), grid, block, 0, st, a);
    else if (pro == PRO_BN_BWD_POOL) USIP_LAUNCH((wgrad_x3_kernel<PRO_BN_BWD_POOL, true, 2>), grid, block, 0, st, a);
    else return USIP_EINVAL;
    USIP_LAUNCH_CHECK();
    return USIP_OK;
}

int launch_wgrad_x3_256(const WgradArgs& a, int pro, bool xpro, unsigned blocks, hipStream_t st)
{
    dim3 grid(blocks), block(512);
#define USIP_X3W_CASE(P_, X_)                                                             \
    if (pro == P_ && xpro == X_) {                                                        \
        USIP_LAUNCH((wgrad_x3_kernel<P_, X_>), grid, block, 0, st, a);                    \
        USIP_LAUNCH_CHECK();                                                              \
        return USIP_OK;                                                                   \
    }
    USIP_X3W_CASE(PRO_NONE, false) USIP_X3W_CASE(PRO_NONE, true)
    USIP_X3W_CASE(PRO_BN_BWD, false) USIP_X3W_CASE(PRO_BN_BWD, true)
    USIP_X3W_CASE(PRO_BN_BWD_POOL, false) USIP_X3W_CASE(PRO_BN_BWD_POOL, true)
#undef USIP_X3W_CASE
    return USIP_EINVAL;
}

}
```

### usip_amd/functional.py

```python
from typing import Optional, Tuple

import torch
import torch.nn.functional as F

from . import ops, prof


GRAD_SINK = False
DEFER_BN_COUNTERS = False


FUSED_NARROW_BWD = True
FUSED_NARROW_RED = True
import os as _os
if _os.environ.get("USIP_NARROW_BWD") is not None:
    FUSED_NARROW_BWD = _os.environ["USIP_NARROW_BWD"] not in ("0", "off")
if _os.environ.get("USIP_NARROW_RED") is not None:
    FUSED_NARROW_RED = _os.environ["USIP_NARROW_RED"] not in ("0", "off")


SEGMENT_BACKWARD = _os.environ.get("USIP_SEGMENT_BWD", "1") not in ("0", "off")


WT_CACHE = None
# ... 119 lines not shown
                raise RuntimeError("usip_amd: a parameter is used twice in one step while the gradient sink is on "
                                   "(its backward overwrites .grad); run this step without DetectorStep's sink")
            p._usip_sink_used = True
    return tuple(out)


def require_device(t: torch.Tensor, what: str):
    if not t.is_cuda:
        raise RuntimeError("usip_amd: %s needs device tensors; the HIP path has no CPU fallback" % what)


class _NearestDistance(torch.autograd.Function):

    @staticmethod
    def forward(ctx, a, b):
        a, b = a.contiguous(), b.contiguous()
        d, arg32 = ops.nearest(a, b) if a.shape[1] == 3 else ops.nearest_nd(a, b)
        ctx.save_for_backward(a, b, d, arg32)
        ctx.mark_non_differentiable(arg32)
        ctx.set_materialize_grads(False)
        return d, arg32

    @staticmethod
    def backward(ctx, gd, _garg):
        if gd is None:
            return None, None
        a, b, d, arg32 = ctx.saved_tensors
        ga, gb = ops.nearest_backward(a, b, d, arg32, gd.contiguous(), ctx.needs_input_grad[1])
        return (ga if ctx.needs_input_grad[0] else None), gb


def nearest_distance_i32(a: torch.Tensor, b: torch.Tensor) -> Tuple[torch.Tensor, torch.Tensor]:
    require_device(a, "nearest_distance")
    return _NearestDistance.apply(a, b)


class _ChamferProb(torch.autograd.Function):

    @staticmethod
    def forward(ctx, a, J, c, I, sigma_src, sigma_dst):
        sigma_src, sigma_dst = sigma_src.contiguous(), sigma_dst.contiguous()
        out = ops.chamfer_prob(a, J, c, I, sigma_src, sigma_dst)
        ctx.save_for_backward(a, J, c, I, sigma_src, sigma_dst)
        ctx.set_materialize_grads(False)
        loss, pure, weighted = out[0], out[1], out[2]
        ctx.mark_non_differentiable(pure, weighted)
        return loss, pure, weighted

    @staticmethod
    def backward(ctx, gloss, _gp, _gw):
        if gloss is None:
            return (None,) * 6
        a, J, c, I, ss, sd = ctx.saved_tensors
        da, dc, dss, dsd = ops.chamfer_prob_backward(gloss.contiguous(), a, J, c, I, ss, sd)
        return da, None, dc, None, dss, dsd


def chamfer_prob(a, J32, c, I32, sigma_src, sigma_dst):
    return _ChamferProb.apply(a, J32, c, I32, sigma_src, sigma_dst)


class _DetectorHead(torch.autograd.Function):

    @staticmethod
    def forward(ctx, ks, centre, lower):
        ks = ks.contiguous()
        kp, sg = ops.detector_head(ks, centre.contiguous(), lower)
        ctx.save_for_backward(ks)
        ctx.set_materialize_grads(False)
        return kp, sg

    @staticmethod
    def backward(ctx, g_kp, g_sg):
        (ks,) = ctx.saved_tensors
        if g_kp is None and g_sg is None:
            return None, None, None
        return ops.detector_head_backward(None if g_kp is None else g_kp.contiguous(),
                                          None if g_sg is None else g_sg.contiguous(), ks), None, None


def detector_head(ks, centre, sigma_lower_bound: float):
    require_device(ks, "detector_head")
    return _DetectorHead.apply(ks, centre.detach(), float(sigma_lower_bound))


class _RigidTransform(torch.autograd.Function):

    @staticmethod
    def forward(ctx, x, R, scale, shift):
        R, scale = R.contiguous(), scale.contiguous()
        ctx.save_for_backward(R, scale)
        return ops.rigid_transform(x.contiguous(), R, scale, shift.contiguous())

    @staticmethod
    def backward(ctx, g):
        R, scale = ctx.saved_tensors
        return ops.rigid_transform(g.contiguous(), R, scale, None, transpose=True), None, None, None


def rigid_transform(x, R, scale, shift):
    require_device(x, "rigid_transform")
    return _RigidTransform.apply(x, R, scale.reshape(-1), shift.reshape(shift.shape[0], 3))


class _DetectorLossCombine(torch.autograd.Function):

    @staticmethod
    def forward(ctx, d, chamfer, alpha):
        d = d.contiguous()
        out = ops.detector_loss_combine(d, chamfer.reshape(1), alpha)
        ctx.shape, ctx.alpha = tuple(d.shape), float(alpha)
        loss, on_src, on_dst = out[0], out[1], out[2]
        ctx.mark_non_differentiable(on_src, on_dst)
        ctx.set_materialize_grads(False)
        return loss, on_src, on_dst

    @staticmethod
    def backward(ctx, gloss, _g1, _g2):
        if gloss is None:
            return None, None, None
        gloss = gloss.contiguous().reshape(1)
        n = 1
        for v in ctx.shape:
            n *= v
        return ops.fill_scaled(gloss, ctx.alpha / (n // 2), ctx.shape), gloss.reshape(()), None


def detector_loss_combine(d, chamfer, alpha: float):
    return _DetectorLossCombine.apply(d, chamfer, float(alpha))


def nearest_distance(a: torch.Tensor, b: torch.Tensor) -> Tuple[torch.Tensor, torch.Tensor]:
    d, arg32 = nearest_distance_i32(a, b)
    return d, arg32.long()


def knn_indices(query: torch.Tensor, database: torch.Tensor, K: int) -> torch.Tensor:
    require_device(query, "knn_indices")
    q, d = query.detach().contiguous(), database.detach().contiguous()
    if d.shape[2] <= 1024:
        return ops.knn(q, d, K)
    return torch.topk(ops.pairwise_dist(q, d), k=K, dim=2, largest=False, sorted=True)[1].int()


def gather_neighbours(x: torch.Tensor, idx: torch.Tensor) -> torch.Tensor:
    B, C, _ = x.shape
    _, M, K = idx.shape
    flat = idx.reshape(B, 1, M * K).expand(B, C, M * K)
    return torch.gather(x, 2, flat).view(B, C, M, K)


class LazyAct:

    def __init__(self, y: torch.Tensor, coef: torch.Tensor, relu: bool, shape, wsrc=None):
        self.y, self.coef, self.relu, self.shape = y, coef, relu, tuple(shape)
        self.wsrc = wsrc

    def materialize(self) -> torch.Tensor:
        return _Materialize.apply(self.y, self.coef, self.relu).view(self.shape)


class _Materialize(torch.autograd.Function):
    @staticmethod
    def forward(ctx, y, coef, relu):
        return ops.bn_apply(y, coef, relu)

    @staticmethod
    def backward(ctx, dz):
        return dz, None, None


def as_tensor(x):
    return x.materialize() if isinstance(x, LazyAct) else x


PRE_BN_SUMS = {}
POOLED_LAYER_RED = _os.environ.get("USIP_POOLED_LAYER_RED", "1") != "0"


def _register_pre_bn_sums(dx, partials):
    if GRAD_SINK:
        PRE_BN_SUMS[dx.data_ptr()] = (tuple(dx.shape), partials, dx._version)


def _take_pre_bn_sums(dz, shape=None):
    pre = PRE_BN_SUMS.pop(dz.data_ptr(), None)
    if pre is None or pre[0] != tuple(dz.shape if shape is None else shape) or pre[2] != dz._version:
        return None
    return pre


def _own_bn_backward(dz, y, coef, mean, invstd, gamma, relu, sink, group=0, took=None):
    go, bo = (sink[2], sink[3]) if sink else (None, None)
    pre = _take_pre_bn_sums(dz)
    if pre is not None and group == 0 and relu:
        if took is not None:
            took.extend(pre[1])
        return ops.bn_backward_from_partials(pre[1], dz.shape[0] * dz.shape[2], coef, mean, invstd, go, bo)
    if pre is not None and group and relu and len(pre[1]) == 1:
        gsum = getattr(pre[1][0], "gsum", None)
        if gsum is not None and gsum.shape[3] * group == dz.shape[2]:
            return ops.bn_backward_from_partials(pre[1], dz.shape[0] * dz.shape[2], coef, mean, invstd, go, bo) + (gsum,)
    dgamma, dbeta, coef4, gsum = ops.bn_backward_reduce(dz, y, coef, mean, invstd, gamma, relu, group=group,
                                                        dgamma_out=go, dbeta_out=bo)
    return (dgamma, dbeta, coef4, gsum) if group else (dgamma, dbeta, coef4)


GEMM_RED = _os.environ.get("USIP_GEMM_RED", "0") not in ("0", "off")


def _dgrad(x, w2c, dz, pro, X2=None, coef=None, pool=None, M=None, a_offset=0, xcoef=None, red_group=0):
    if (GEMM_RED and FUSED_NARROW_RED and GRAD_SINK and pro >= 2 and xcoef is not None and xcoef.shape[0] >= 4
            and (M is None or M == x.shape[1]) and a_offset >= 0):
        dx, _, r = ops.mlp_gemm(w2c, dz, pro=pro, X2=X2, coef=coef, tag="dgrad", pool=pool, M=M, a_offset=a_offset,
                                red=(x, xcoef), red_group=red_group)
        if r is not None:
            _register_pre_bn_sums(dx, [r])
        return dx
    return ops.mlp_gemm(w2c, dz, pro=pro, X2=X2, coef=coef, tag="dgrad", pool=pool, M=M, a_offset=a_offset)[0]


class _SharedMLPLayer(torch.autograd.Function):

    @staticmethod
    def forward(ctx, x, xcoef, w2, bias, gamma, beta, running_mean, running_var, training, momentum, eps,
                relu, defer, sink, nograd_prefix=0, wsrc=None):
        ctx.sink = sink
        ctx.nograd_prefix = int(nograd_prefix)
        ctx.wsrc = wsrc
        ctx.set_materialize_grads(False)
        x = x.contiguous()
        wt = _kmajor(w2)
        nb, _, P = x.shape
        ctx.has_bn = gamma is not None
        ctx.relu = bool(relu)
        ctx.train_stats = bool(training)
        pro = 0 if xcoef is None else 1
        if not ctx.has_bn:
            if relu:
                raise NotImplementedError("usip_amd: ReLU without BatchNorm is outside the detector path")
            y, _ = ops.mlp_gemm(wt, x, bias, pro=pro, coef=xcoef)
            ctx.save_for_backward(x, xcoef, w2)
            return y, None
        if training:
            y, stats = ops.mlp_gemm(wt, x, bias, want_stats=True, pro=pro, coef=xcoef)
            mean, invstd, coef = ops.bn_finalize(stats, nb * P, gamma, beta, eps, momentum,
                                                 running_mean, running_var)
            if relu:
                y = _relu_hook(y, coef)
        else:
            y, _ = ops.mlp_gemm(wt, x, bias, pro=pro, coef=xcoef)
            invstd = torch.rsqrt(running_var + eps)
            mean = running_mean
            scale = gamma * invstd
            coef = torch.stack((scale, beta - running_mean * scale)).contiguous()
        ctx.save_for_backward(x, xcoef, w2, y, coef, mean, invstd, gamma)
        if defer:
            ctx.mark_non_differentiable(coef)
            return y, coef
        return ops.bn_apply(y, coef, relu), None

    @staticmethod
    def backward(ctx, dz, _dcoef):
        if dz is None:
            return (None,) * 16
        dz = dz.contiguous()
        need_x, need_w = ctx.needs_input_grad[0], ctx.needs_input_grad[2]
        tail = (None,) * 10
        sink = ctx.sink
        if not ctx.has_bn:
            x, xcoef, w2 = ctx.saved_tensors
            dx = None
            if need_x:
                dx = _dgrad(x, w2.contiguous(), dz, pro=0)
            dw = db = None
            if need_w:
                dw = ops.mlp_wgrad(dz, x, xcoef=xcoef, out=sink[0].view(w2.shape) if sink else None)
            if ctx.needs_input_grad[3]:
                db = ops.bn_backward_reduce(dz, None, None, None, None, None, False,
                                            dbeta_out=sink[1] if sink else None)[1]
            if sink:
                dw = db = None
            return (dx, None, dw, db, None, None) + tail
        if not ctx.train_stats:
            raise NotImplementedError("usip_amd: backward through eval-mode BatchNorm is outside the path")
        x, xcoef, w2, y, coef, mean, invstd, gamma = ctx.saved_tensors
        took = []
        dgamma, dbeta, coef4 = _own_bn_backward(dz, y, coef, mean, invstd, gamma, ctx.relu, sink, took=took)
        if not ctx.relu:
            C = dz.shape[1]
            dy = torch.addcmul(torch.addcmul(coef4[3].view(1, C, 1), y, coef4[2].view(1, C, 1)),
                               dz, coef4[0].view(1, C, 1))
            dx = _dgrad(x, w2.contiguous(), dy, pro=0) if need_x else None
            dw = None
            if need_w:
                dw = ops.mlp_wgrad(dy, x, xcoef=xcoef, out=sink[0].view(w2.shape) if sink else None)
            db = torch.zeros_like(gamma) if (ctx.needs_input_grad[3] and not sink) else None
            if sink:
                dw = db = dgamma = dbeta = None
            return (dx, None, dw, db, dgamma, dbeta) + tail
        x2 = (FUSED_NARROW_BWD and need_x and need_w and ctx.relu and ctx.nograd_prefix == 0
              and ops.layer_backward_x2_supported(x.shape[1], w2.shape[0], x.shape[2], (dz, y, x), coef4, xcoef))
        if x2 or (FUSED_NARROW_BWD and need_x and need_w and ctx.relu and ctx.nograd_prefix == 0
                  and ops.narrow_backward_supported(x.shape[1], w2.shape[0], x.shape[2], (dz, y, x))):
            red = FUSED_NARROW_RED and xcoef is not None and xcoef.shape[0] >= 4
            if x2:
                res = ops.mlp_layer_backward_x2(dz, y, coef4, x, xcoef, w2.contiguous(), Cin=x.shape[1],
                                                dw_out=sink[0].view(w2.shape) if sink else None, want_red=red,
                                                wsrc=ctx.wsrc if red else None)
            else:
                res = ops.mlp_narrow_backward(dz, y, coef4, x, xcoef, w2.contiguous(),
                                              dw_out=sink[0].view(w2.shape) if sink else None, want_red=red)
            dx, dw = res[0], res[1]
            if red:
                _register_pre_bn_sums(dx, [res[2]])
            db = torch.zeros_like(gamma) if (ctx.needs_input_grad[3] and not sink) else None
            if sink:
                dw = db = dgamma = dbeta = None
            return (dx, None, dw, db, dgamma, dbeta) + tail
        dx = None
        if need_x:
            pre = ctx.nograd_prefix
            if pre > 0:
                dx = torch.empty_like(x)
                dx[:, :pre].zero_()
                ops.mlp_gemm(w2.contiguous(), dz, pro=2, X2=y, coef=coef4, tag="dgrad", M=x.shape[1] - pre,
                             a_offset=pre, out=dx, out_row_offset=pre)
            else:
                dx = _dgrad(x, w2.contiguous(), dz, pro=2, X2=y, coef=coef4, xcoef=xcoef)
        dw = None
        if need_w:
            pack = took[0].wsum if (len(took) == 1 and getattr(took[0], "wsum", None) is not None) else None
            if (pack is not None and not need_x and xcoef is None and pack[2].data_ptr() == x.data_ptr()
                    and tuple(pack[2].shape) == tuple(x.shape) and w2.shape[1] == x.shape[1] and w2.is_contiguous()):
                dw = ops.wsum_finalize(pack, coef4, mean, sink[0].view(w2.shape) if sink else torch.empty_like(w2))
            else:
                dw = ops.mlp_wgrad(dz, x, pro=2, G2=y, coef4=coef4, xcoef=xcoef,
                                   out=sink[0].view(w2.shape) if sink else None)
        db = torch.zeros_like(gamma) if (ctx.needs_input_grad[3] and not sink) else None
        if sink:
            dw = db = dgamma = dbeta = None
        return (dx, None, dw, db, dgamma, dbeta) + tail


class _SharedMLPLayerMax(torch.autograd.Function):

    @staticmethod
    def forward(ctx, x, xcoef, dims, w2, bias, gamma, beta, running_mean, running_var, momentum, eps, sink):
        B, Cin, M, K = dims
        x3 = x.contiguous().view(B, Cin, M * K)
        Cout = w2.shape[0]
        y, stats = ops.mlp_gemm(_kmajor(w2), x3, bias, want_stats=True,
                                pro=0 if xcoef is None else 1, coef=xcoef)
        mean, invstd, coef = ops.bn_finalize(stats, B * M * K, gamma, beta, eps, momentum, running_mean, running_var)
        y = _relu_hook(y, coef)
        pooled, arg, yarg = _pooled_act(y.view(B, Cout, M, K), coef, True, want_yarg=True)
        ctx.save_for_backward(x3, xcoef, w2, y, coef, mean, invstd, gamma, arg, yarg)
        ctx.dims, ctx.sink, ctx.x_shape = (B, Cin, Cout, M, K), sink, tuple(x.shape)
        return pooled

    @staticmethod
    def backward(ctx, dpooled):
        x3, xcoef, w2, y, coef, mean, invstd, gamma, arg, yarg = ctx.saved_tensors
        B, Cin, Cout, M, K = ctx.dims
        sink = ctx.sink
        dpooled = dpooled.contiguous()
        dgamma, dbeta, coef4 = ops.bn_pool_backward_reduce(dpooled, arg, y.view(B, Cout, M, K), coef, mean, invstd,
                                                           gamma, True, dgamma_out=sink[2] if sink else None,
                                                           dbeta_out=sink[3] if sink else None, yarg=yarg)
        pool = (dpooled, arg, K)
        dx = dw = None
        if (FUSED_NARROW_BWD and ctx.needs_input_grad[0] and ctx.needs_input_grad[3]
                and ops.layer_backward_x2_supported(Cin, Cout, M * K, (y, x3), coef4, xcoef, pooled=True)):
            red = (POOLED_LAYER_RED and FUSED_NARROW_RED and xcoef is not None and xcoef.shape[0] >= 4 and K % 32 == 0
                   and bool(GRAD_SINK))
            res = ops.mlp_layer_backward_x2(None, y, coef4, x3, xcoef, w2.contiguous(), Cin=Cin, pool=pool,
                                            dw_out=sink[0].view(w2.shape) if sink else None, want_red=red, want_gsum=red)
            dx, dw = res[0], res[1]
            if red:
                _register_pre_bn_sums(dx, [res[2]])
            db = torch.zeros_like(gamma) if (ctx.needs_input_grad[4] and not sink) else None
            if sink:
                dw = db = dgamma = dbeta = None
            return (dx.view(ctx.x_shape), None, None, dw, db, dgamma, dbeta) + (None,) * 5
        if ctx.needs_input_grad[0]:
            dx = _dgrad(x3, w2.contiguous(), None, pro=3, X2=y, coef=coef4, pool=pool, xcoef=xcoef,
                        red_group=K if (POOLED_LAYER_RED and K in (16, 32)) else 0)
            dx = dx.view(ctx.x_shape)
        if ctx.needs_input_grad[3]:
            dw = ops.mlp_wgrad(None, x3, pro=3, G2=y, coef4=coef4, xcoef=xcoef, pool=pool,
                               out=sink[0].view(w2.shape) if sink else None)
        db = torch.zeros_like(gamma) if (ctx.needs_input_grad[4] and not sink) else None
        if sink:
            dw = db = dgamma = dbeta = None
        return (dx, None, None, dw, db, dgamma, dbeta) + (None,) * 5


def conv1x1_bn_relu_max(x, weight: torch.Tensor, bias: Optional[torch.Tensor], bn) -> torch.Tensor:
    shape = x.shape
    K = shape[3]
    fused = (bn is not None and bn.training and bias is not None and _group_sums_supported(K)
             and torch.is_grad_enabled())
    if not fused:
        return group_max(conv1x1_bn_act(x, weight, bias, bn, True, defer=True))
    xcoef = None
    if isinstance(x, LazyAct):
        if not x.relu:
            x = x.materialize()
        else:
            x, xcoef = x.y, x.coef
    require_device(x, "the shared MLP")
    w2 = weight.reshape(weight.shape[0], weight.shape[1])
    if bn.num_batches_tracked is not None and not DEFER_BN_COUNTERS:
        bn.num_batches_tracked.add_(1)
    return _SharedMLPLayerMax.apply(x, xcoef, tuple(shape), w2, bias, bn.weight, bn.bias, bn.running_mean,
                                    bn.running_var, bn.momentum, bn.eps, _sink(weight, bias, bn.weight, bn.bias))


def _group_sums_supported(K: int) -> bool:
    lpg = K // 4
    return K >= 4 and K % 4 == 0 and (lpg & (lpg - 1)) == 0 and lpg <= 64


class _SharedMLPLayerPooled(torch.autograd.Function):

    @staticmethod
    def forward(ctx, h, hcoef, dims, pooled, w2, bias, gamma, beta, running_mean, running_var, training, momentum,
                eps, relu, pooled_first, defer, sink):
        ctx.sink = sink
        B, Ch, M, K = dims
        Cp = pooled.shape[1]
        Cout = w2.shape[0]
        ctx.set_materialize_grads(False)
        poff, hoff = (0, Cp) if pooled_first else (Ch, 0)
        h3 = h.contiguous().view(B, Ch, M * K)
        pooled = pooled.contiguous()
        wt = _kmajor(w2)
        r, _ = ops.mlp_gemm(wt[poff:poff + Cp], pooled, tag="fwd_pooled")
        y, stats = ops.mlp_gemm(wt[hoff:hoff + Ch], h3, bias, want_stats=True, rowbias=r, rb_group=K,
                                pro=0 if hcoef is None else 1, coef=hcoef)
        mean, invstd, coef = ops.bn_finalize(stats, B * M * K, gamma, beta, eps, momentum,
                                             running_mean, running_var)
        if relu:
            y = _relu_hook(y, coef)
        ctx.save_for_backward(h3, hcoef, pooled, w2, y, coef, mean, invstd, gamma)
        ctx.dims = (B, Ch, Cp, Cout, M, K, poff, hoff)
        ctx.h_shape = tuple(h.shape)
        ctx.relu = bool(relu)
        if defer:
            ctx.mark_non_differentiable(coef)
            return y, coef
        return ops.bn_apply(y, coef, relu), None

    @staticmethod
    def backward(ctx, dz, _dcoef):
        if dz is None:
            return (None,) * 17
        h3, hcoef, pooled, w2, y, coef, mean, invstd, gamma = ctx.saved_tensors
        B, Ch, Cp, Cout, M, K, poff, hoff = ctx.dims
        dz = dz.contiguous().view(B, Cout, M * K)
        sink = ctx.sink
        dgamma, dbeta, coef4, gsum = _own_bn_backward(dz, y, coef, mean, invstd, gamma, ctx.relu, sink, group=K)
        sdy = ops.bn_group_dy_sum(gsum, coef4, K)
        w2c = w2.contiguous()
        dpooled = dh = dw = None
        if ctx.needs_input_grad[3]:
            dpooled = ops.mlp_gemm(w2c, sdy, tag="dgrad_pooled", M=Cp, a_offset=poff)[0]
        want = FUSED_NARROW_BWD and ctx.needs_input_grad[0] and ctx.needs_input_grad[4] and ctx.relu
        x2 = want and ops.layer_backward_x2_supported(Ch, Cout, M * K, (dz, y, h3), coef4, hcoef)
        fused = x2 or (want and ops.narrow_backward_supported(Ch, Cout, M * K, (dz, y, h3)))
        if fused:
            dw = sink[0].view(w2c.shape) if sink else torch.empty_like(w2c)
            red = FUSED_NARROW_RED and hcoef is not None and hcoef.shape[0] >= 4
            back = ops.mlp_layer_backward_x2 if x2 else ops.mlp_narrow_backward
            with ops.reduce_now(not sink):
                res = back(dz, y, coef4, h3, hcoef, w2c, wcol=hoff, dw_out=dw, Cin=Ch, want_red=red)
                ops.mlp_wgrad(sdy, pooled, out=dw, coloff=poff)
            if red:
                _register_pre_bn_sums(res[0], [res[2]])
            dh = res[0].view(ctx.h_shape)
        if ctx.needs_input_grad[0] and not fused:
            dh = _dgrad(h3, w2c, dz, pro=2, X2=y, coef=coef4, M=Ch, a_offset=hoff, xcoef=hcoef).view(ctx.h_shape)
        if ctx.needs_input_grad[4] and not fused:
            dw = sink[0].view(w2c.shape) if sink else torch.empty_like(w2c)
            with ops.reduce_now(not sink):
                ops.mlp_wgrad(dz, h3, pro=2, G2=y, coef4=coef4, out=dw, coloff=hoff, xcoef=hcoef)
                ops.mlp_wgrad(sdy, pooled, out=dw, coloff=poff)
        db = torch.zeros_like(gamma) if (ctx.needs_input_grad[5] and not sink) else None
        if sink:
            dw = db = dgamma = dbeta = None
        return (dh, None, None, dpooled, dw, db, dgamma, dbeta) + (None,) * 9


def conv1x1_bn_act_pooled(h, pooled: torch.Tensor, weight: torch.Tensor, bias: Optional[torch.Tensor], bn,
                          relu: bool, pooled_first: bool, defer: bool = False):
    hshape = h.shape
    K = hshape[3]
    fused = (bn is not None and bn.training and bias is not None and _group_sums_supported(K)
             and torch.is_grad_enabled())
    if not fused:
        ht = as_tensor(h)
        e = pooled.unsqueeze(3).expand(-1, -1, -1, K)
        return conv1x1_bn_act(torch.cat((e, ht) if pooled_first else (ht, e), dim=1), weight, bias, bn, relu,
                              defer=defer)
    hcoef = None
    if isinstance(h, LazyAct):
        if not h.relu:
            h = h.materialize()
        else:
            h, hcoef = h.y, h.coef
    require_device(h, "the shared MLP")
    w2 = weight.reshape(weight.shape[0], weight.shape[1])
    if bn.num_batches_tracked is not None and not DEFER_BN_COUNTERS:
        bn.num_batches_tracked.add_(1)
    out, coef = _SharedMLPLayerPooled.apply(h, hcoef, tuple(hshape), pooled, w2, bias, bn.weight, bn.bias,
                                            bn.running_mean, bn.running_var, True, bn.momentum, bn.eps, relu,
                                            pooled_first, defer, _sink(weight, bias, bn.weight, bn.bias))
    oshape = (hshape[0], w2.shape[0], hshape[2], K)
    return LazyAct(out, coef, relu, oshape) if defer else out.view(oshape)


def conv1x1_bn_act(x, weight: torch.Tensor, bias: Optional[torch.Tensor],
                   bn: Optional[torch.nn.modules.batchnorm._BatchNorm], relu: bool, defer: bool = False,
                   nograd_prefix: int = 0):
    shape = x.shape
    xcoef = wsrc_in = None
    if isinstance(x, LazyAct):
        if not x.relu:
            x = x.materialize()
        else:
            x, xcoef, wsrc_in = x.y, x.coef, x.wsrc
    require_device(x, "the shared MLP")
    w2 = weight.reshape(weight.shape[0], weight.shape[1])
    x3 = x.reshape(shape[0], shape[1], -1)
    oshape = (shape[0], w2.shape[0]) + tuple(shape[2:])
    if bn is None:
        y, _ = _SharedMLPLayer.apply(x3, xcoef, w2, bias, None, None, None, None, False, 0.0, 0.0, relu, False,
                                     _sink(weight, bias))
        return y.view(oshape)
    training = bn.training or bn.running_mean is None
    if bn.training and bn.num_batches_tracked is not None and not DEFER_BN_COUNTERS:
        bn.num_batches_tracked.add_(1)
    y, coef = _SharedMLPLayer.apply(x3, xcoef, w2, bias, bn.weight, bn.bias, bn.running_mean, bn.running_var,
                                    training, bn.momentum, bn.eps, relu, defer,
                                    _sink(weight, bias, bn.weight, bn.bias) if training else None, nograd_prefix, wsrc_in)
    if not defer:
        return y.view(oshape)
    first = (training and relu and xcoef is None and not x3.requires_grad and x3.shape[1] <= 8 and x3.is_contiguous()
             and torch.is_grad_enabled())
    return LazyAct(y, coef, relu, oshape, wsrc=x3 if first else None)


class _GroupMax(torch.autograd.Function):

    @staticmethod
    def forward(ctx, z):
        pooled, arg = _pooled_act(z.contiguous(), None, False)
        ctx.save_for_backward(arg)
        ctx.K = z.shape[3]
        return pooled

    @staticmethod
    def backward(ctx, dpooled):
        (arg,) = ctx.saved_tensors
        return ops.group_max_backward(dpooled.contiguous(), arg, ctx.K)


class _GroupMaxAct(torch.autograd.Function):

    @staticmethod
    def forward(ctx, y4, coef, relu):
        pooled, arg = _pooled_act(y4.contiguous(), coef, relu)
        ctx.save_for_backward(arg)
        ctx.K = y4.shape[3]
        return pooled

    @staticmethod
    def backward(ctx, dpooled):
        (arg,) = ctx.saved_tensors
        return ops.group_max_backward(dpooled.contiguous(), arg, ctx.K), None, None


class _GroupMaxActFork(torch.autograd.Function):

    @staticmethod
    def forward(ctx, y4, coef, relu):
        pooled, arg, yarg = _pooled_act(y4.contiguous(), coef, relu, want_yarg=True)
        ctx.save_for_backward(arg, y4, coef, yarg)
        ctx.K = y4.shape[3]
        ctx.relu = bool(relu)
        ctx.set_materialize_grads(False)
        return pooled, y4.view_as(y4)

    @staticmethod
    def backward(ctx, dpooled, dy):
        arg, y4, coef, yarg = ctx.saved_tensors
        if dpooled is None:
            return dy, None, None
        if dy is None:
            return ops.group_max_backward(dpooled.contiguous(), arg, ctx.K), None, None
        B, C, M, K = y4.shape
        pre = _take_pre_bn_sums(dy, (B, C, M * K))
        dy = dy.contiguous() if GRAD_SINK else dy.clone(memory_format=torch.contiguous_format)
        dpooled = dpooled.contiguous()
        out = ops.group_max_backward_add_(dy, dpooled, arg)
        if pre is not None and coef.shape[0] >= 4 and GRAD_SINK:
            sparse = ops.bn_pool_backward_partials(dpooled, arg, y4, coef, coef[2], coef[3], ctx.relu, yarg=yarg)
            out3 = out.view(B, C, M * K)
            PRE_BN_SUMS[out3.data_ptr()] = ((B, C, M * K), pre[1] + [sparse], out3._version)
        return out, None, None


def group_max_fork(z):
    if isinstance(z, LazyAct) and _group_sums_supported(z.shape[3]):
        pooled, y = _GroupMaxActFork.apply(z.y.view(z.shape), z.coef, z.relu)
        return pooled, LazyAct(y.view(z.y.shape), z.coef, z.relu, z.shape)
    return group_max(z), z


def group_max(z) -> torch.Tensor:
    if isinstance(z, LazyAct):
        K = z.shape[3]
        if _group_sums_supported(K):
            return _GroupMaxAct.apply(z.y.view(z.shape), z.coef, z.relu)
        z = z.materialize()
    require_device(z, "group_max")
    return _GroupMax.apply(z)


class _KnnGroup(torch.autograd.Function):

    @staticmethod
    def forward(ctx, feat, database, query, idx32):
        B, C, N = feat.shape
        _, M, K = idx32.shape
        out = torch.empty((B, 3 + C, M, K), dtype=torch.float32, device=feat.device)
        ops.group_gather(database.contiguous(), idx32, sub=query.contiguous(), out=out, coff=0)
        ops.group_gather(feat.contiguous(), idx32, out=out, coff=3)
        ctx.dims = (C, N)
        ctx.csr = SEGMENT_BACKWARD and feat.requires_grad and ops.segment_sum_supported(N, M * K)
        if ctx.csr:
            ctx.save_for_backward(*ops.csr_by_index(idx32.view(B, M * K), N))
        else:
            ctx.save_for_backward(idx32)
        return out

    @staticmethod
    def backward(ctx, dout):
        C, N = ctx.dims
        if ctx.csr:
            start, perm = ctx.saved_tensors
            return ops.segment_sum(dout.contiguous(), start, perm, C, coff=3), None, None, None
        (idx32,) = ctx.saved_tensors
        return ops.group_gather_backward(dout.contiguous(), idx32, C, N, coff=3), None, None, None


KNN_FIRST_LAYER = _os.environ.get("USIP_KNN_LAYER", "1") not in ("0", "off")


class _KnnFirstLayer(torch.autograd.Function):

    @staticmethod
    def forward(ctx, feat, database, query, idx32, w2, bias, gamma, beta, running_mean, running_var, momentum, eps, sink):
        B, C, N = feat.shape
        _, M, K = idx32.shape
        ctx.set_materialize_grads(False)
        feat = feat.contiguous()
        database, query = database.contiguous(), query.contiguous()
        w2c = w2.contiguous()
        U, _ = ops.mlp_gemm(_kmajor(w2)[3:], feat, bias, tag="fwd_knn_nodes")
        y, stats = ops.knn_layer_forward(U, w2c, database, query, idx32)
        mean, invstd, coef = ops.bn_finalize(stats.view(2, w2.shape[0], B), B * M * K, gamma, beta, eps, momentum,
                                             running_mean, running_var)
        y = _relu_hook(y, coef)
        start, perm = ops.csr_by_index(idx32.view(B, M * K), N)
        dcoord = ops.group_gather(database, idx32, sub=query)
        ctx.save_for_backward(feat, dcoord, w2, y, coef, mean, invstd, gamma, start, perm)
        ctx.sink = sink
        ctx.mark_non_differentiable(coef)
        return y, coef

    @staticmethod
    def backward(ctx, dz, _dcoef):
        if dz is None:
            return (None,) * 13
        feat, dcoord, w2, y, coef, mean, invstd, gamma, start, perm = ctx.saved_tensors
        sink = ctx.sink
        C = feat.shape[1]
        dz = dz.contiguous().view(y.shape)
        dgamma, dbeta, coef4 = _own_bn_backward(dz, y, coef, mean, invstd, gamma, True, sink)
        dU, dwc = ops.knn_layer_backward(dz, y, coef4, True, dcoord.view(dcoord.shape[0], 3, -1), start, perm,
                                         dcoord.shape[2], dcoord.shape[3])
        w2c = w2.contiguous()
        dfeat = dw = None
        if ctx.needs_input_grad[0]:
            dfeat = ops.mlp_gemm(w2c, dU, tag="dgrad_knn_nodes", M=C, a_offset=3)[0]
        if ctx.needs_input_grad[4]:
            dw = sink[0].view(w2c.shape) if sink else torch.empty_like(w2c)
            with ops.reduce_now(not sink):
                ops.mlp_wgrad(dU, feat, out=dw, coloff=3)
            dw[:, :3].copy_(dwc)
        db = torch.zeros_like(gamma) if (ctx.needs_input_grad[5] and not sink) else None
        if sink:
            dw = db = dgamma = dbeta = None
        return (dfeat, None, None, None, dw, db, dgamma, dbeta) + (None,) * 5


def knn_first_layer_supported(feat, idx32, bias, bn, relu: bool) -> bool:
    return (KNN_FIRST_LAYER and relu and bias is not None and bn is not None and bn.training and torch.is_grad_enabled()
            and isinstance(feat, torch.Tensor) and feat.is_cuda
            and ops.knn_layer_supported(feat.shape[2], idx32.shape[1], idx32.shape[2]))


def knn_first_layer(feat, database, query, idx32, weight, bias, bn) -> "LazyAct":
    require_device(feat, "knn_first_layer")
    w2 = weight.reshape(weight.shape[0], weight.shape[1])
    if bn.num_batches_tracked is not None and not DEFER_BN_COUNTERS:
        bn.num_batches_tracked.add_(1)
    y, coef = _KnnFirstLayer.apply(feat, database.detach(), query.detach(), idx32, w2, bias, bn.weight, bn.bias,
                                   bn.running_mean, bn.running_var, bn.momentum, bn.eps,
                                   _sink(weight, bias, bn.weight, bn.bias))
    return LazyAct(y, coef, True, (feat.shape[0], w2.shape[0], idx32.shape[1], idx32.shape[2]))


class _ClusterBroadcast(torch.autograd.Function):

    @staticmethod
    def forward(ctx, x, idx32, start, perm):
        B, C, M = x.shape
        N = idx32.shape[1]
        ctx.csr = start is not None
        ctx.save_for_backward(*((start, perm) if ctx.csr else (idx32,)))
        ctx.dims = (C, M)
        return ops.group_gather(x.contiguous(), idx32.view(B, N, 1)).view(B, C, N)

    @staticmethod
    def backward(ctx, dout):
        C, M = ctx.dims
        B, _, N = dout.shape
        if ctx.csr:
            start, perm = ctx.saved_tensors
            return ops.segment_sum(dout.contiguous(), start, perm, C), None, None, None
        (idx32,) = ctx.saved_tensors
        return ops.group_gather_backward(dout.contiguous().view(B, C, N, 1), idx32.view(B, N, 1), C, M), None, None, None


def cluster_broadcast(x, idx32, csr=None):
    require_device(x, "cluster_broadcast")
    if csr is None and SEGMENT_BACKWARD and x.requires_grad and ops.segment_sum_supported(x.shape[2], idx32.shape[1]):
        csr = ops.csr_by_index(idx32, x.shape[2])
    start, perm = csr if csr is not None else (None, None)
    return _ClusterBroadcast.apply(x, idx32, start, perm)


class _SomPoolLayer(torch.autograd.Function):

    @staticmethod
    def forward(ctx, x, xcoef, w2, bias, min_idx32, count, start, perm, M, concat, sink):
        x = x.contiguous()
        nb, _, N = x.shape
        C = w2.shape[0]
        wt = _kmajor(w2)
        pro = 0 if xcoef is None else 1
        ctx.set_materialize_grads(False)
        if concat:
            out = torch.empty((nb, 2 * C, N), dtype=torch.float32, device=x.device)
            ops.mlp_gemm(wt, x, bias, pro=pro, coef=xcoef, out=out, out_row_offset=0)
            idx, val = ops.index_max_values(out, min_idx32, count, M, C=C)
            ops.group_gather(val, min_idx32.view(nb, N, 1), out=out.view(nb, 2 * C, N, 1), coff=C)
# ... 50 lines not shown
```

### usip_amd/ops.py

```python
import ctypes
import functools
import math
import os
from typing import Optional

import torch

from . import _lib, prof


def _stream(t: torch.Tensor):
    return ctypes.c_void_p(torch.cuda.current_stream(t.device).cuda_stream)


def _need(t: torch.Tensor, name: str, dtype):
    if not isinstance(t, torch.Tensor):
        raise RuntimeError("%s must be a torch.Tensor" % name)
    if not t.is_cuda:
        raise RuntimeError("%s must be a CUDA tensor/variable" % name)
    if not t.is_contiguous():
        raise RuntimeError("%s must be contiguous" % name)
    if t.dtype != dtype:
        raise RuntimeError("%s must be %s (got %s)" % (name, dtype, t.dtype))

# ... 216 lines not shown
    B, M = a.shape
    N = c.shape[1]
    _need(gloss, "gloss", torch.float32)
    da, dc = torch.empty_like(a), torch.empty_like(c)
    dss, dsd = torch.empty_like(sigma_src), torch.empty_like(sigma_dst)
    with torch.cuda.device(a.device), prof.kernel("chamfer_prob_bwd", 4.0 * 7 * B * (M + N), 0.0):
        _lib.check(_lib.lib().usip_chamfer_prob_backward_f32(_ptr(gloss), _ptr(a), _ptr(J), _ptr(c), _ptr(I),
                                                             _ptr(sigma_src), _ptr(sigma_dst), _ptr(da), _ptr(dc),
                                                             _ptr(dss), _ptr(dsd), B, M, N, _stream(a)),
                   "usip_chamfer_prob_backward_f32")
    return da, dc, dss, dsd


def bn_group_dy_sum(gsum, coef4, K: int):
    g0, g1 = gsum[0], gsum[1]
    nb, C, G = g0.shape
    out = torch.empty_like(g0)
    with torch.cuda.device(g0.device), prof.kernel("bn_group_dy_sum", 12.0 * g0.numel()):
        _lib.check(_lib.lib().usip_bn_group_dy_sum_f32(_ptr(g0), _ptr(g1), _ptr(coef4), _ptr(out), nb, C, G, int(K),
                                                       _stream(g0)), "usip_bn_group_dy_sum_f32")
    return out


def detector_head(ks, centre, sigma_lower_bound: float):
    _need(ks, "ks", torch.float32)
    _need(centre, "centre", torch.float32)
    B, _, M = ks.shape
    kp = torch.empty((B, 3, M), dtype=torch.float32, device=ks.device)
    sg = torch.empty((B, M), dtype=torch.float32, device=ks.device)
    with torch.cuda.device(ks.device), prof.kernel("head", 4.0 * 11 * B * M):
        _lib.check(_lib.lib().usip_detector_head_f32(_ptr(ks), _ptr(centre), float(sigma_lower_bound), _ptr(kp), _ptr(sg),
                                                     B, M, _stream(ks)), "usip_detector_head_f32")
    return kp, sg


def detector_head_backward(g_kp, g_sg, ks):
    B, _, M = ks.shape
    g = torch.empty_like(ks)
    with torch.cuda.device(ks.device), prof.kernel("head_bwd", 4.0 * 9 * B * M):
        _lib.check(_lib.lib().usip_detector_head_backward_f32(_opt(g_kp), _opt(g_sg), _ptr(ks), _ptr(g), B, M,
                                                              _stream(ks)), "usip_detector_head_backward_f32")
    return g


def rigid_transform(x, R, scale, shift, transpose: bool = False):
    _need(x, "x", torch.float32)
    B, _, M = x.shape
    out = torch.empty_like(x)
    with torch.cuda.device(x.device), prof.kernel("rigid_transform", 4.0 * 6 * B * M):
        _lib.check(_lib.lib().usip_rigid_transform_f32(_ptr(x), _ptr(R), _ptr(scale), _opt(shift), _ptr(out),
                                                       int(bool(transpose)), B, M, _stream(x)),
                   "usip_rigid_transform_f32")
    return out


def detector_loss_combine(d, chamfer, alpha: float):
    _need(d, "d", torch.float32)
    out = torch.empty(3, dtype=torch.float32, device=d.device)
    with torch.cuda.device(d.device), prof.kernel("loss_combine", 4.0 * d.numel()):
        _lib.check(_lib.lib().usip_detector_loss_combine_f32(_ptr(d), _ptr(chamfer), float(alpha), _ptr(out),
                                                             d.numel() // 2, _stream(d)),
                   "usip_detector_loss_combine_f32")
    return out


def fill_scaled(g, factor: float, shape):
    out = torch.empty(shape, dtype=torch.float32, device=g.device)
    with torch.cuda.device(g.device), prof.kernel("fill_scaled", 4.0 * out.numel()):
        _lib.check(_lib.lib().usip_fill_scaled_f32(_ptr(g), float(factor), _ptr(out), out.numel(), _stream(g)),
                   "usip_fill_scaled_f32")
    return out


def _opt(t):
    return _ptr(t) if t is not None else None


MATMUL_MODES = ("f32", "bf16", "f32x3", "f32x2")


def _x3_family() -> bool:
    return _matmul_mode in ("f32x3", "f32x2")
_matmul_mode = "f32"
import os as _os
if _os.environ.get("USIP_MATMUL_MODE"):
    if _os.environ["USIP_MATMUL_MODE"] not in MATMUL_MODES:
        raise ValueError("USIP_MATMUL_MODE must be one of %s" % (MATMUL_MODES,))
    _matmul_mode = _os.environ["USIP_MATMUL_MODE"]


def set_matmul_mode(mode: str) -> str:
    global _matmul_mode
    if mode not in MATMUL_MODES:
        raise ValueError("matmul mode must be one of %s" % (MATMUL_MODES,))
    prev, _matmul_mode = _matmul_mode, mode
    return prev


def matmul_mode() -> str:
    return _matmul_mode


PLANES_CACHE = None


def weight_planes(At: torch.Tensor, a_offset: int, M: int, K: int, npl: int = 3, P: int = 0, nb: int = 1) -> torch.Tensor:
    lda = At.shape[1]
    rows = int(_lib.lib().usip_mlp_x3p_tile_rows(int(M), int(P), int(nb)))
    key = (At.data_ptr(), lda, int(a_offset), int(M), int(K), int(npl), rows)
    if PLANES_CACHE is not None and key in PLANES_CACHE:
        return PLANES_CACHE[key][1]
    nbytes = int(_lib.lib().usip_mlp_split3_bytes(M, K))
    planes = torch.empty(nbytes, dtype=torch.uint8, device=At.device)
    fn = "usip_mlp_split2h_f32" if npl == 2 else "usip_mlp_split3_f32"
    with torch.cuda.device(At.device), prof.kernel("weight_split3", 4.0 * M * K + nbytes):
        _lib.check(getattr(_lib.lib(), fn)(ctypes.c_void_p(At.data_ptr() + 4 * int(a_offset)), lda, M, K, rows,
                                           _ptr(planes), _stream(At)), fn)
    if PLANES_CACHE is not None:
        PLANES_CACHE[key] = (At, planes)
    return planes


class PlanesPlan:

    def __init__(self, cache, storages):
        import numpy as np
        spans = [(t.data_ptr(), t.data_ptr() + t.numel() * t.element_size()) for t in storages if t is not None]
        self.entries, rows, blocks = {}, [], 0
        for key, (At, planes) in cache.items():
            ptr, lda, off, M, K, npl, trows = key
            if not any(lo <= ptr < hi for lo, hi in spans):
                continue
            self.entries[key] = (At, planes)
            rows.append((ptr + 4 * off, planes.data_ptr(), lda, M, K, blocks, trows, 2 if npl == 2 else 0))
            blocks += int(_lib.lib().usip_mlp_split3_blocks(M, K, trows))
        self.blocks = blocks
        dt = np.dtype([("At", "<u8"), ("planes", "<u8"), ("lda", "<i4"), ("M", "<i4"), ("K", "<i4"), ("first", "<i4"),
                       ("tile_rows", "<i4"), ("reserved", "<i4")])
        table = np.array(rows, dtype=dt) if rows else np.zeros(0, dtype=dt)
        dev = next(iter(self.entries.values()))[1].device if rows else None
        self.table = torch.from_numpy(table.view(np.uint8).copy()).to(dev) if rows else None

    def refresh(self):
        if self.table is not None:
            with torch.cuda.device(self.table.device), prof.kernel("weight_split3", 0.0):
                _lib.check(_lib.lib().usip_mlp_split3_multi_f32(_ptr(self.table), len(self.entries), self.blocks,
                                                                _stream(self.table)), "usip_mlp_split3_multi_f32")
        return dict(self.entries)


NARROW_FWD = _os.environ.get("USIP_NARROW_FWD", "1") not in ("0", "off")
X2R = _os.environ.get("USIP_X2R", "1") not in ("0", "off")
X2R_NARROW = _os.environ.get("USIP_X2R_NARROW", "1") not in ("0", "off")


def mlp_gemm(At: torch.Tensor, X: torch.Tensor, bias=None, want_stats: bool = False, pro: int = 0,
             X2=None, coef=None, tag: str = "fwd", rowbias=None, rb_group: int = 1,
             M: Optional[int] = None, a_offset: int = 0, pool=None, a_trans: bool = False, out=None,
             out_row_offset: int = 0, red=None, red_group: int = 0):
    _need(At, "At", torch.float32)
    if a_trans:
        M_rows, lda = At.shape
        M = M_rows if M is None else int(M)
        K = X2.shape[1] if X is None else X.shape[1]
    else:
        K, lda = At.shape
        M = lda if M is None else int(M)
    pool_dp = pool_arg = None
    pool_group = 0
    if pool is not None:
        pool_dp, pool_arg, pool_group = pool
        X = X2
    _need(X, "X", torch.float32)
    nb, Kx, P = X.shape
    if Kx != K or a_offset < 0 or a_offset + (K if a_trans else M) > lda:
        raise RuntimeError("mlp_gemm: operand shapes do not match (At %s, X %s, M %d, offset %d)"
                           % (tuple(At.shape), tuple(X.shape), M, a_offset))
    y_rows = 0
    if out is None:
        Y = torch.empty((nb, M, P), dtype=torch.float32, device=X.device)
        y_ptr = _ptr(Y)
    else:
        _need(out, "out", torch.float32)
        if out.dim() != 3 or out.shape[0] != nb or out.shape[2] != P or out_row_offset < 0 \
                or out_row_offset + M > out.shape[1]:
            raise RuntimeError("mlp_gemm: out %s does not hold rows [%d, %d) of [%d, *, %d]"
                               % (tuple(out.shape), out_row_offset, out_row_offset + M, nb, P))
        Y, y_rows = out, out.shape[1]
        y_ptr = ctypes.c_void_p(out.data_ptr() + 4 * int(out_row_offset) * P)
    a_ptr = ctypes.c_void_p(At.data_ptr() + 4 * int(a_offset))
    rb_ok = rowbias is None or (rb_group % 32 == 0 and P % rb_group == 0)
    x2r_direct = (X2R and X2R_NARROW and _matmul_mode == "f32x2" and pro == 1 and coef is not None and coef.shape[0] >= 4
                  and M == 128 and K == 64 and not a_trans and pool is None and X2 is None and rb_ok
                  and nb * P >= 65536 and K * P < 2 ** 30)
    nf_blocks = 0
    if (NARROW_FWD and not x2r_direct and _matmul_mode != "bf16" and not a_trans and pool is None and X2 is None and pro in (0, 1)
            and K == 64 and M in (64, 128) and X.data_ptr() % 16 == 0
            and (rowbias is None or (rb_group % 32 == 0 and P % rb_group == 0))):
        nf_blocks = int(_lib.lib().usip_mlp_narrow_forward_blocks(M, K, P, nb))
    if nf_blocks:
        stats = torch.empty((2, M, nf_blocks), dtype=torch.float32, device=X.device) if want_stats else None
        with torch.cuda.device(X.device), prof.kernel(
                "shared_mlp_gemm_%s %dx%d" % (tag, M, K), 4.0 * nb * P * (K + M), 2.0 * M * K * nb * P, keyed=True):
            _lib.check(_lib.lib().usip_mlp_narrow_forward_f32(a_ptr, lda, _ptr(X), _opt(coef), int(pro), _opt(bias),
                                                              _opt(rowbias), int(rb_group), y_ptr, int(y_rows),
                                                              _opt(stats), M, K, P, nb, _stream(X)),
                       "usip_mlp_narrow_forward_f32")
        return (Y, stats, None) if red is not None else (Y, stats)
    fn_name = {"bf16": "usip_mlp_gemm_bf16", "f32x3": "usip_mlp_gemm_f32x3",
               "f32x2": "usip_mlp_gemm_f32x3"}.get(_matmul_mode, "usip_mlp_gemm_f32")
    x3 = _x3_family() and (x2r_direct or bool(_lib.lib().usip_mlp_gemm_f32x3_used(M, K, P, nb)))
    x3p = x3 and not a_trans and K <= (512 if pro >= 2 else 640)
    x2h = (x3p and _matmul_mode == "f32x2" and coef is not None and
           ((pro == 1 and coef.shape[0] >= 4 and bound_covers(coef, nb * P)) or (pro >= 2 and coef.shape[0] >= 5)))
    x2r = (x2h and M <= 128 and K <= 128 and X2R and K * P < 2 ** 30
           and (rowbias is None or (pro == 1 and rb_ok and rb_group >= 32)))
    stats = None
    if want_stats:
        tiles = _lib.lib().usip_mlp_gemm_x2r_tiles(P, nb) if x2r else _lib.lib().usip_mlp_gemm_tiles(M, P, nb)
        stats = torch.empty((2, M, tiles), dtype=torch.float32, device=X.device)

    planes = weight_planes(At, a_offset, M, K, 2 if x2h else 3, P, nb) if x3p else None
    moved = 0.0
    if x3p:
        bm_ = int(_lib.lib().usip_mlp_x3p_tile_rows(M, P, nb))
        bn_ = 128 if x2h else int(_lib.lib().usip_mlp_x3p_tile_cols(M, P, nb, int(pro), 1 if want_stats else 0))
        ntiles = nb * ((P + bn_ - 1) // bn_) * ((M + bm_ - 1) // bm_)
        moved = ntiles * ((K + 15) // 16) * ((2 if x2h else 3) * bm_ * 32 + 16 * bn_ * 4 * (2 if pro == 2 else 1)) \
            + 4.0 * nb * M * P
        if x2r:
            moved = 4.0 * nb * P * (K * (2 if pro == 2 else 1) + M)
    with torch.cuda.device(X.device), prof.kernel("shared_mlp_gemm_%s %dx%d" % (tag, M, K),
                                                  4.0 * nb * P * (K * (2 if pro == 2 else 1) + M),
                                                  2.0 * M * K * nb * P, keyed=True, moved=moved):
        if x2r:
            _lib.check(_lib.lib().usip_mlp_gemm_x2r_f32(_ptr(planes), None if pool is not None else _ptr(X), _opt(X2),
                                                        _opt(coef), int(pro), _opt(bias), _opt(rowbias), int(rb_group),
                                                        _opt(pool_dp), _opt(pool_arg), int(pool_group), y_ptr,
                                                        int(y_rows), _opt(stats), M, K, P, nb, _stream(X)),
                       "usip_mlp_gemm_x2r_f32")
            return (Y, stats, None) if red is not None else (Y, stats)
        red_tiles = 0
        if (red is not None and x2h and not x2r and pro >= 2 and out is None and bias is None and rowbias is None
                and red[1] is not None and red[1].shape[0] >= 4 and tuple(red[0].shape) == (nb, M, P)
                and red[0].is_contiguous() and red[0].data_ptr() % 16 == 0):
            red_tiles = int(_lib.lib().usip_mlp_gemm_x2d_red_tiles(M, K, P, nb, int(red_group)))
        if red_tiles:
            flat = torch.empty(2 * red_tiles * M + red_tiles * (M // 256), dtype=torch.float32, device=X.device)
            gsum = torch.empty((2, nb, M, P // red_group), dtype=torch.float32, device=X.device) if red_group else None
            _lib.check(_lib.lib().usip_mlp_gemm_x2h_red_f32(_ptr(planes), None if pool is not None else _ptr(X), _opt(X2),
                                                            _opt(coef), int(pro), _opt(pool_dp), _opt(pool_arg),
                                                            int(pool_group), y_ptr, _ptr(red[0]), _ptr(red[1]), _ptr(flat),
                                                            _opt(gsum), int(red_group), M, K, P, nb, _stream(X)),
                       "usip_mlp_gemm_x2h_red_f32")
            r = RedSums(flat, M, blocks=red_tiles)
            r.gsum = gsum
            return Y, stats, r
        if x3p:
            fn = "usip_mlp_gemm_x2h_f32" if x2h else "usip_mlp_gemm_x3p_f32"
            _lib.check(getattr(_lib.lib(), fn)(_ptr(planes), None if pool is not None else _ptr(X), _opt(X2),
                                               _opt(coef), int(pro), _opt(bias), _opt(rowbias), int(rb_group),
                                               _opt(pool_dp), _opt(pool_arg), int(pool_group), y_ptr,
                                               int(y_rows), _opt(stats), M, K, P, nb, _stream(X)), fn)
            return (Y, stats, None) if red is not None else (Y, stats)
        _lib.check(getattr(_lib.lib(), fn_name)(a_ptr, -lda if a_trans else lda,
                                                None if pool is not None else _ptr(X), _opt(X2),
                                                _opt(coef), int(pro), _opt(bias), _opt(rowbias), int(rb_group),
                                                _opt(pool_dp), _opt(pool_arg), int(pool_group),
                                                y_ptr, int(y_rows), _opt(stats), M, K, P, nb, _stream(X)), fn_name)
    return (Y, stats, None) if red is not None else (Y, stats)


def bn_finalize(stats, count, gamma, beta, eps, momentum, running_mean, running_var):
    _, C, tiles = stats.shape
    dev = stats.device
    mean = torch.empty(C, dtype=torch.float32, device=dev)
    invstd = torch.empty(C, dtype=torch.float32, device=dev)
    coef = torch.empty((4, C), dtype=torch.float32, device=dev)
    with torch.cuda.device(dev), prof.kernel("bn_finalize", 4.0 * 2 * tiles * C):
        _lib.check(_lib.lib().usip_bn_finalize_f32(_ptr(stats), tiles, C, int(count), _opt(gamma), _opt(beta),
                                                   float(eps), float(momentum), _opt(running_mean),
                                                   _opt(running_var), _ptr(mean), _ptr(invstd), _ptr(coef),
                                                   _stream(stats)), "usip_bn_finalize_f32")
    declare_samples(coef, int(count))
    return mean, invstd, coef


import collections
_SAMPLES = collections.OrderedDict()
_SAMPLES_MAX = 8192
UNKNOWN_SAMPLE_LOOKUPS = 0


def declare_samples(coef, count: int):
    key = coef.data_ptr()
    _SAMPLES.pop(key, None)
    _SAMPLES[key] = (int(count), int(coef.numel()))
    while len(_SAMPLES) > _SAMPLES_MAX:
        _SAMPLES.popitem(last=False)


def bound_covers(coef, samples: int) -> bool:
    global UNKNOWN_SAMPLE_LOOKUPS
    rec = _SAMPLES.get(coef.data_ptr())
    if rec is not None and rec[1] != int(coef.numel()) and coef._base is None:
        rec = None
    if rec is None:
        UNKNOWN_SAMPLE_LOOKUPS += 1
        return os.environ.get("USIP_ASSUME_LAUNCH_SAMPLES") == "1"
    return rec[0] <= samples


def bn_apply(Y, coef, relu: bool):
    nb, C, P = Y.shape
    Z = torch.empty_like(Y)
    with torch.cuda.device(Y.device), prof.kernel("bn_apply", 8.0 * nb * C * P):
        _lib.check(_lib.lib().usip_bn_apply_f32(_ptr(Y), _ptr(coef), _ptr(Z), int(bool(relu)), nb, C, P,
                                                _stream(Y)), "usip_bn_apply_f32")
    return Z


def bn_backward_reduce(dZ, Y, coef_fwd, mean, invstd, gamma, relu: bool, group: int = 0,
                       dgamma_out=None, dbeta_out=None):
    nb, C, P = dZ.shape
    dev = dZ.device
    want_bound = 1 if (_matmul_mode == "f32x2" and Y is not None) else 0
    partial = torch.empty((3 if want_bound else 2) * nb * C, dtype=torch.float32, device=dev)
    dbeta = dbeta_out if dbeta_out is not None else torch.empty(C, dtype=torch.float32, device=dev)
    dgamma = coef4 = gsum = None
    if Y is not None:
        dgamma = dgamma_out if dgamma_out is not None else torch.empty(C, dtype=torch.float32, device=dev)
        coef4 = torch.empty((5 if want_bound else 4, C), dtype=torch.float32, device=dev)
        if group:
            gsum = torch.empty((2, nb, C, P // group), dtype=torch.float32, device=dev)
    with torch.cuda.device(dev), prof.kernel("bn_backward_reduce", 4.0 * nb * C * P * (1 if Y is None else 2)):
        _lib.check(_lib.lib().usip_bn_backward_reduce_f32(_ptr(dZ), _opt(Y), _opt(coef_fwd), _opt(mean), _opt(invstd),
                                                          _opt(gamma), int(bool(relu)), _ptr(partial), _opt(dgamma),
                                                          _ptr(dbeta), _opt(coef4), _opt(gsum), int(group),
                                                          nb, C, P, want_bound, _stream(dZ)),
                   "usip_bn_backward_reduce_f32")
    return dgamma, dbeta, coef4, gsum


_DEFER_KEEP = None


def _keep(ws):
    if _DEFER_KEEP is not None:
        _DEFER_KEEP.append(ws)
    return ws


def wgrad_defer(on: bool, device=None):
    global _DEFER_KEEP
    if on and device is not None:
        dev = torch.device(device)
        _lib.check(_lib.lib().usip_wgrad_defer_on(ctypes.c_void_p(torch.cuda.current_stream(dev).cuda_stream)),
                   "usip_wgrad_defer_on")
    else:
        _lib.check(_lib.lib().usip_wgrad_defer(1 if on else 0), "usip_wgrad_defer")
    _DEFER_KEEP = [] if on else None


class _reduce_now:

    def __init__(self, private: bool):
        self.on = bool(private) and _DEFER_KEEP is not None

    def __enter__(self):
        if self.on:
            self.was = int(_lib.lib().usip_wgrad_defer_hold(1))

    def __exit__(self, *exc):
        if self.on:
            _lib.lib().usip_wgrad_defer_hold(self.was)
        return False


def wgrad_flush(device) -> int:
    global _DEFER_KEEP
    dev = torch.device(device)
    with torch.cuda.device(dev), prof.kernel("wgrad_reduce_all", 0.0):
        n = int(_lib.lib().usip_wgrad_flush(ctypes.c_void_p(torch.cuda.current_stream(dev).cuda_stream)))
    if n < 0:
        raise RuntimeError("usip_amd: usip_wgrad_flush failed (%d)" % n)
    if _DEFER_KEEP is not None:
        _DEFER_KEEP = []
    return n


def bn_pool_backward_reduce(dpooled, arg, Y4, coef_fwd, mean, invstd, gamma, relu: bool,
                            dgamma_out=None, dbeta_out=None, yarg=None):
    nb, C, M, K = Y4.shape
    dev = Y4.device
    want_bound = 1 if _matmul_mode == "f32x2" else 0
    partial = torch.empty((3 if want_bound else 2) * nb * C, dtype=torch.float32, device=dev)
    dbeta = dbeta_out if dbeta_out is not None else torch.empty(C, dtype=torch.float32, device=dev)
    dgamma = dgamma_out if dgamma_out is not None else torch.empty(C, dtype=torch.float32, device=dev)
    coef4 = torch.empty((5 if want_bound else 4, C), dtype=torch.float32, device=dev)
    with torch.cuda.device(dev), prof.kernel("bn_backward_reduce_pooled", 4.0 * nb * C * M * 3):
        _lib.check(_lib.lib().usip_bn_pool_backward_reduce_f32(_ptr(dpooled), _ptr(arg), _ptr(Y4), _opt(yarg),
                                                               _ptr(coef_fwd), _ptr(mean), _ptr(invstd), _opt(gamma),
                                                               int(bool(relu)), _ptr(partial), _ptr(dgamma), _ptr(dbeta),
                                                               _ptr(coef4), nb, C, M, K, want_bound, _stream(Y4)),
                   "usip_bn_pool_backward_reduce_f32")
    return dgamma, dbeta, coef4


def mlp_wgrad(G, X, pro: int = 0, G2=None, coef4=None, out=None, coloff: int = 0, xcoef=None, pool=None):
    pool_dp = pool_arg = None
    pool_group = 0
    if pool is not None:
        pool_dp, pool_arg, pool_group = pool
        nb, M, P = G2.shape
    else:
        nb, M, P = G.shape
    N = X.shape[1]
    dev = X.device
    ws_n = _lib.lib().usip_mlp_wgrad_workspace(M, N, P, nb)
    ws = _keep(torch.empty(max(int(ws_n), 1), dtype=torch.float32, device=dev))
    dW = out if out is not None else torch.empty((M, N), dtype=torch.float32, device=dev)
    ldw = dW.shape[1]
    fn_name = {"bf16": "usip_mlp_wgrad_bf16", "f32x3": "usip_mlp_wgrad_f32x3",
# ... 1440 lines not shown
```

Measured before the change: 3776 point-clouds/s.

## Fold group-max pooled gradient scatter into the x2 data-gradient GEMM epilogue

Adds a fork variant of the x2f direct data-gradient GEMM kernel. Its epilogue adds dpooled to the argmax position of each group while storing dh, and it double-buffers the next tile's dpooled/arg values in LDS. The pooled gradient then no longer has to be scattered back through a separate group-max backward pass, which saves a kernel and a read-modify-write of the activation gradient. The cost is extra LDS, extra buffer loads inside the epilogue and more Python plumbing. It also carries a risk if the fork gating conditions or the returned tuples are mismatched.

```diff
diff --git a/include/usip_hip.h b/include/usip_hip.h
--- a/include/usip_hip.h
+++ b/include/usip_hip.h
@@ -140,6 +140,10 @@
                               const float* pool_dp, const int32_t* pool_arg, int pool_group, float* Y,
                               const float* red_y, const float* red_coef, float* red_out, float* red_gsum,
                               int red_group, int M, int K, int P, int nb, void* stream);
+int usip_mlp_gemm_x2h_fork_supported(int M, int K, int P, int nb, int fork_group);
+int usip_mlp_gemm_x2h_fork_f32(const void* planes, const float* X, const float* X2, const float* coef, float* Y, int y_rows,
+                               const float* fork_dp, const int32_t* fork_arg, int fork_group, int M, int K, int P, int nb,
+                               void* stream);
 int usip_mlp_gemm_x2r_tiles(int P, int nb);
 int usip_mlp_gemm_x2r_f32(const void* planes, const float* X, const float* X2, const float* coef, int pro,
                           const float* bias, const float* rowbias, int rb_group, const float* pool_dp,
diff --git a/usip_amd/_lib.py b/usip_amd/_lib.py
--- a/usip_amd/_lib.py
+++ b/usip_amd/_lib.py
@@ -83,6 +83,9 @@
     "usip_mlp_gemm_x2d_red_tiles": ([_int, _int, _int, _int, _int], _int),
     "usip_mlp_gemm_x2h_red_f32": ([ctypes.c_void_p, _f32p, _f32p, _f32p, _int, _f32p, _i32p, _int, _f32p, _f32p, _f32p, _f32p,
                                    _f32p, _int, _int, _int, _int, _int, _stream], _int),
+    "usip_mlp_gemm_x2h_fork_supported": ([_int, _int, _int, _int, _int], _int),
+    "usip_mlp_gemm_x2h_fork_f32": ([ctypes.c_void_p, _f32p, _f32p, _f32p, _f32p, _int, _f32p, _i32p, _int, _int, _int, _int,
+                                    _int, _stream], _int),
     "usip_mlp_wgrad_f32x3_used": ([_int, _int, _int, _int], _int),
     "usip_bn_pool_backward_reduce_f32": ([_f32p, _i32p, _f32p, _f32p, _f32p, _f32p, _f32p, _f32p, _int, _f32p, _f32p,
                                           _f32p, _f32p, _int, _int, _int, _int, _int, _stream], _int),
diff --git a/usip_amd/csrc/gemm_x2f.hip b/usip_amd/csrc/gemm_x2f.hip
--- a/usip_amd/csrc/gemm_x2f.hip
+++ b/usip_amd/csrc/gemm_x2f.hip
@@ -174,6 +174,81 @@
     }
 }
 
+constexpr int FFRS = FBM + 4;
+constexpr int FFARR = 16 * FFRS * 4;
+constexpr int FFORK = 2 * FFARR;
+
+struct ForkFill { u32x4 d[4], g[4]; };
+
+__device__ __forceinline__ void fork_fetch(ForkFill& F, __amdgpu_buffer_rsrc_t rFd, __amdgpu_buffer_rsrc_t rFa, int voff, int npc)
+{
+#pragma unroll
+    for (int j = 0; j < 4; ++j)
+        if (j < npc) {
+            F.d[j] = __builtin_bit_cast(u32x4, __builtin_amdgcn_raw_buffer_load_b128(rFd, voff, 16 * j, 0));
+            F.g[j] = __builtin_bit_cast(u32x4, __builtin_amdgcn_raw_buffer_load_b128(rFa, voff, 16 * j, 0));
+        }
+}
+
+__device__ __forceinline__ void fork_put(const ForkFill& F, unsigned char* fk, int npc)
+{
+    unsigned* dst = reinterpret_cast<unsigned*>(fk) + threadIdx.x;
+#pragma unroll
+    for (int j = 0; j < 4; ++j)
+        if (j < npc) {
+#pragma unroll
+            for (int u = 0; u < 4; ++u) {
+                dst[(4 * j + u) * FFRS] = F.d[j][u];
+                dst[FFARR / 4 + (4 * j + u) * FFRS] = F.g[j][u];
+            }
+        }
+}
+
+__device__ __forceinline__ void epilogue_x2f_direct_fork(const GemmArgs& a, f32x16 (&acc)[8][2], float out_scale, int b, int m0, int p0,
+                                                         const unsigned char* fk, unsigned char* fkn, bool fill, int nvoff,
+                                                         __amdgpu_buffer_rsrc_t rFd, __amdgpu_buffer_rsrc_t rFa, int npc)
+{
+    const int tid = threadIdx.x, lane = tid & 63, c = lane & 31, half = lane >> 5;
+    const int wave = __builtin_amdgcn_readfirstlane(tid >> 6);
+    const __amdgpu_buffer_rsrc_t rY = __builtin_amdgcn_make_buffer_rsrc(
+        (void*)(a.Y + (long long)b * a.y_rows * a.P), 0, (unsigned)a.y_rows * (unsigned)a.P * 4u, 0x00020000);
+    const int voff = ((m0 + 4 * half) * a.P + p0 + wave * 64 + 2 * c) * 4;
+    const int rowb = a.P * 4;
+    const int pl = wave * 64 + 2 * c;
+    const int gi = pl / a.fork_group, kin = pl - gi * a.fork_group;
+    const unsigned char* fl = fk + (gi * FFRS + 4 * half) * 4;
+    auto fetch = [&](int ig, u32x4& d, u32x4& r) {
+        d = *reinterpret_cast<const u32x4*>(fl + ig * 32);
+        r = *reinterpret_cast<const u32x4*>(fl + FFARR + ig * 32);
+    };
+    ForkFill F;
+    u32x4 cd, ca, nd, na;
+    fetch(0, cd, ca);
+#pragma unroll
+    for (int ig = 0; ig < 32; ++ig) {
+        const int i = ig >> 2, g = ig & 3;
+        if (ig == 24 && fill) fork_fetch(F, rFd, rFa, nvoff, npc);
+        if (ig < 31) fetch(ig + 1, nd, na);
+        u32x2 v[4];
+#pragma unroll
+        for (int e = 0; e < 4; ++e) {
+            const float dp = __uint_as_float(cd[e]);
+            const int ar = (int)ca[e];
+            float x = f_aread(acc[i][0], 4 * g + e) * out_scale, y = f_aread(acc[i][1], 4 * g + e) * out_scale;
+            x = (ar == kin) ? x + dp : x;
+            y = (ar == kin + 1) ? y + dp : y;
+            v[e] = u32x2{__float_as_uint(x), __float_as_uint(y)};
+        }
+#pragma unroll
+        for (int e = 0; e < 4; ++e)
+            __builtin_amdgcn_raw_buffer_store_b64(v[e], rY, voff, (i * 32 + 8 * g + e) * rowb, st_aux<ST_X2F_DGRAD>());
+        asm volatile("s_nop 7" ::: "memory");
+        __builtin_amdgcn_sched_barrier(0);
+        cd = nd; ca = na;
+    }
+    if (fill) fork_put(F, fkn, npc);
+}
+
 __host__ __device__ constexpr int f_ns(int sl) { return (sl % 6) >= 2 ? (sl / 6) * 4 + (sl % 6) - 2 : -1; }
 
 #ifdef USIP_X2F_TRACE
@@ -197,10 +272,10 @@
 #define X2F_TP(REG_, IDX_)
 #endif
 
-template <int PRO, int EPI, bool DIRECT>
-__global__ __launch_bounds__(FNT) __attribute__((amdgpu_waves_per_eu(1, 1))) void gemm_x2f_kernel(
-    const GemmArgs a, const uint4* __restrict__ planes)
-{
+template <int PRO, int EPI, bool DIRECT, bool FORK>
+__device__ __forceinline__ void gemm_x2f_body(const GemmArgs& a, const uint4* __restrict__ planes)
+{
+    static_assert(!FORK || (DIRECT && PRO == PRO_BN_BWD), "FORK: the plain data-gradient form");
     constexpr bool POOL = (PRO == PRO_BN_BWD_POOL);
     constexpr bool TWO = (PRO == PRO_BN_BWD) || POOL;
     constexpr int NC = TWO ? 4 : 2;
@@ -208,7 +283,9 @@
     constexpr int KPAD = KMAX + 16;
     constexpr int RING = FSLOTS * FSTAGE;
     constexpr int SCR = DIRECT ? 64 : FSCR_FLOATS * 4;
-    __shared__ __attribute__((aligned(16))) unsigned char smem[RING + SCR + NC * KPAD * 4];
+    constexpr int FOFF = RING + SCR + NC * KPAD * 4;
+    static_assert(FOFF % 16 == 0, "16-B pieces");
+    __shared__ __attribute__((aligned(16))) unsigned char smem[FOFF + (FORK ? 2 * FFORK : 0)];
     float* scr = reinterpret_cast<float*>(smem + RING);
     float* cf = reinterpret_cast<float*>(smem + RING + SCR);
 
@@ -267,6 +344,13 @@
                                                                          POOL ? pool_bytes : 4u, 0x00020000);
     const __amdgpu_buffer_rsrc_t rPa = __builtin_amdgcn_make_buffer_rsrc((void*)(POOL ? (const float*)a.pool_arg : a.X), 0,
                                                                          POOL ? pool_bytes : 4u, 0x00020000);
+    const int fgrp = FORK ? a.P / a.fork_group : 0, npc = FORK ? FBN / (4 * a.fork_group) : 0;
+    const unsigned fork_bytes = (unsigned)a.nb * (unsigned)a.M * (unsigned)fgrp * 4u;
+    const __amdgpu_buffer_rsrc_t rFd = __builtin_amdgcn_make_buffer_rsrc((void*)(FORK ? a.fork_dp : a.X), 0,
+                                                                         FORK ? fork_bytes : 4u, 0x00020000);
+    const __amdgpu_buffer_rsrc_t rFa = __builtin_amdgcn_make_buffer_rsrc((void*)(FORK ? (const float*)a.fork_arg : a.X), 0,
+                                                                         FORK ? fork_bytes : 4u, 0x00020000);
+    auto fork_voff = [&](int b, int m0, int p0) { return (((b * a.M + m0 + tid) * fgrp) + p0 / (FORK ? a.fork_group : 1)) * 4; };
     const int pl = wave * 64 + 2 * c;
     int xv[8], gv[POOL ? 8 : 1];
 #pragma unroll
@@ -442,6 +526,8 @@
     unsigned ah[2][4], al[2][4], bh[2][4], bl[2][4];
     Tile T = tile_of(v);
     {
+        [[maybe_unused]] ForkFill F0;
+        if constexpr (FORK) fork_fetch(F0, rFd, rFa, fork_voff(T.b, T.m0, T.p0), npc);
 #pragma unroll
         for (int st = 0; st < 3; ++st) { dma_pair(T.wo, st, 0); dma_pair(T.wo, st, 1); }
 #pragma unroll
@@ -451,11 +537,13 @@
         convert_all(0, xs0, ah, al);
 #pragma unroll
         for (int i = 0; i < 8; ++i) load_x1(T.xo + 2 * XBK * rs, T.go + 2 * XBK * rsg, xs0, i);
+        if constexpr (FORK) fork_put(F0, smem + FOFF, npc);
         asm volatile("s_waitcnt vmcnt(%0)" ::"n"(2 * NX) : "memory");
         __builtin_amdgcn_s_barrier();
         read_frag(0, 0, 0, FA); read_frag(0, 0, 1, FA);
     }
     int prev_m0 = 0, prev_tn128 = -1;
+    [[maybe_unused]] int fq = 0;
     for (;;) {
         const int vn = v + (int)gridDim.x;
         const bool more = vn < total;
@@ -484,7 +572,11 @@
         asm volatile("s_nop 7\n\ts_nop 7\n\ts_nop 7" ::: "memory");
         __builtin_amdgcn_sched_barrier(0);
         X2F_TP(trp, tix * 8 + 5)
-        if constexpr (DIRECT) epilogue_x2f_direct(a, acc, out_scale, T.b, T.m0, T.p0);
+        if constexpr (FORK) {
+            epilogue_x2f_direct_fork(a, acc, out_scale, T.b, T.m0, T.p0, smem + FOFF + fq * FFORK, smem + FOFF + (fq ^ 1) * FFORK,
+                                     more, fork_voff(Tn.b, Tn.m0, Tn.p0), rFd, rFa, npc);
+            fq ^= 1;
+        } else if constexpr (DIRECT) epilogue_x2f_direct(a, acc, out_scale, T.b, T.m0, T.p0);
         else if (a.rowbias) epilogue_x2f<EPI, true>(a, acc, out_scale, scr, T.b, T.m0, T.p0, prev_m0, prev_tn128, tpc * 2);
         else epilogue_x2f<EPI, false>(a, acc, out_scale, scr, T.b, T.m0, T.p0, prev_m0, prev_tn128, tpc * 2);
         prev_m0 = T.m0;
@@ -510,6 +602,19 @@
         g_x2f_trace[(blockIdx.x * 4 + wave) * 128 + 64 + lane] = trs;
     }
 #endif
+}
+
+template <int PRO, int EPI, bool DIRECT>
+__global__ __launch_bounds__(FNT) __attribute__((amdgpu_waves_per_eu(1, 1))) void gemm_x2f_kernel(
+    const GemmArgs a, const uint4* __restrict__ planes)
+{
+    gemm_x2f_body<PRO, EPI, DIRECT, false>(a, planes);
+}
+
+__global__ __launch_bounds__(FNT) __attribute__((amdgpu_waves_per_eu(1, 1))) void gemm_x2f_fork_kernel(
+    const GemmArgs a, const uint4* __restrict__ planes)
+{
+    gemm_x2f_body<PRO_BN_BWD, EPI_NONE, true, true>(a, planes);
 }
 
 }
@@ -530,6 +635,11 @@
     if ((reinterpret_cast<uintptr_t>(a.X) & 7u) != 0 || (reinterpret_cast<uintptr_t>(a.X2) & 7u) != 0) return false;
     if (pro == PRO_BN_BWD_POOL && (a.pool_group % 2 != 0 || FBN % a.pool_group != 0)) return false;
     if (pro != PRO_AFFINE_RELU && (a.stats || a.bias || a.rowbias)) return false;
+    if (a.fork_dp) {
+        if (pro != PRO_BN_BWD || !a.fork_arg || (a.fork_group != 16 && a.fork_group != 32 && a.fork_group != 64)) return false;
+        if ((long long)a.nb * a.M * (a.P / a.fork_group) * 4 >= (1LL << 31)) return false;
+        if (((reinterpret_cast<uintptr_t>(a.fork_dp) | reinterpret_cast<uintptr_t>(a.fork_arg)) & 15u) != 0) return false;
+    }
     return true;
 }
 
@@ -545,6 +655,8 @@
     if (pro == PRO_AFFINE_RELU) {
         if (a.stats) USIP_LAUNCH((gemm_x2f_kernel<PRO_AFFINE_RELU, EPI_STATS, false>), grid, block, 0, st, a, pl);
         else USIP_LAUNCH((gemm_x2f_kernel<PRO_AFFINE_RELU, EPI_NONE, false>), grid, block, 0, st, a, pl);
+    } else if (pro == PRO_BN_BWD && a.fork_dp) {
+        USIP_LAUNCH(gemm_x2f_fork_kernel, grid, block, 0, st, a, pl);
     } else if (pro == PRO_BN_BWD) {
         USIP_LAUNCH((gemm_x2f_kernel<PRO_BN_BWD, EPI_NONE, true>), grid, block, 0, st, a, pl);
     } else {
diff --git a/usip_amd/csrc/mlp_common.h b/usip_amd/csrc/mlp_common.h
--- a/usip_amd/csrc/mlp_common.h
+++ b/usip_amd/csrc/mlp_common.h
@@ -52,6 +52,7 @@
     int y_rows;
     int y_vec;
     const float* red_y; const float* red_coef; float* red_out; float* red_gsum; int red_group;
+    const float* fork_dp; const int* fork_arg; int fork_group;
 };
 
 template <int PRO>
diff --git a/usip_amd/csrc/shared_mlp_x3.hip b/usip_amd/csrc/shared_mlp_x3.hip
--- a/usip_amd/csrc/shared_mlp_x3.hip
+++ b/usip_amd/csrc/shared_mlp_x3.hip
@@ -1165,6 +1165,38 @@
     if ((usip_tuning_value(USIP_TUNE_X2_DIRECT) & 15) != 1 && (long long)K * P * 4 < (1LL << 31))
         return launch_gemm_x2d(a, pl, pro, st);
     return launch_x3p<4, 2, 2>(a, pl, pro, st);
+}
+
+static bool x2h_fork_args(GemmArgs& a, const float* X, const float* X2, const float* coef, float* Y, int y_rows,
+                          const float* fork_dp, const int32_t* fork_arg, int fork_group, int M, int K, int P, int nb)
+{
+    if (M < 1 || K < 1 || K > 512 || P < 1 || nb < 1 || fork_group < 1 || P % fork_group != 0) return false;
+    if (y_rows == 0) y_rows = M;
+    if (y_rows < M) return false;
+    a = GemmArgs{nullptr, 0, X, X2, coef, nullptr, Y, nullptr, M, K, P, nb, nullptr, 1, nullptr, nullptr, 0,
+                 0, y_rows, (P % 4 == 0 && (reinterpret_cast<uintptr_t>(Y) & 15u) == 0) ? 1 : 0};
+    a.fork_dp = fork_dp; a.fork_arg = fork_arg; a.fork_group = fork_group;
+    if (usip_mlp_x3p_tile_rows(M, P, nb) == 128 || usip_mlp_x3p_tile_cols(M, P, nb, PRO_BN_BWD, 0) == 256) return false;
+    if ((usip_tuning_value(USIP_TUNE_X2_DIRECT) & 15) == 1 || (long long)K * P * 4 >= (1LL << 31)) return false;
+    return gemm_x2f_takes(a, PRO_BN_BWD);
+}
+
+extern "C" int usip_mlp_gemm_x2h_fork_supported(int M, int K, int P, int nb, int fork_group)
+{
+    GemmArgs a;
+    float* const al = reinterpret_cast<float*>(uintptr_t(16));
+    return x2h_fork_args(a, al, al, al, al, 0, al, reinterpret_cast<const int32_t*>(al), fork_group, M, K, P, nb) ? 1 : 0;
+}
+
+extern "C" int usip_mlp_gemm_x2h_fork_f32(const void* planes, const float* X, const float* X2, const float* coef, float* Y,
+                                          int y_rows, const float* fork_dp, const int32_t* fork_arg, int fork_group,
+                                          int M, int K, int P, int nb, void* stream)
+{
+    if (!planes || !X || !X2 || !coef || !Y || !fork_dp || !fork_arg || (reinterpret_cast<uintptr_t>(planes) & 15u))
+        return USIP_EINVAL;
+    GemmArgs a;
+    if (!x2h_fork_args(a, X, X2, coef, Y, y_rows, fork_dp, fork_arg, fork_group, M, K, P, nb)) return USIP_EINVAL;
+    return launch_gemm_x2f(a, reinterpret_cast<const uint4*>(planes), PRO_BN_BWD, (hipStream_t)stream);
 }
 
 extern "C" int usip_mlp_gemm_x2d_red_tiles(int M, int K, int P, int nb, int red_group)
diff --git a/usip_amd/functional.py b/usip_amd/functional.py
--- a/usip_amd/functional.py
+++ b/usip_amd/functional.py
@@ -295,8 +295,9 @@
 
 class LazyAct:
 
-    def __init__(self, y: torch.Tensor, coef: torch.Tensor, relu: bool, shape, wsrc=None):
+    def __init__(self, y: torch.Tensor, coef: torch.Tensor, relu: bool, shape, wsrc=None, fork=None):
         self.y, self.coef, self.relu, self.shape = y, coef, relu, tuple(shape)
+        self.fork = fork
         self.wsrc = wsrc
 
     def materialize(self) -> torch.Tensor:
@@ -569,8 +570,10 @@
 
     @staticmethod
     def forward(ctx, h, hcoef, dims, pooled, w2, bias, gamma, beta, running_mean, running_var, training, momentum,
-                eps, relu, pooled_first, defer, sink):
+                eps, relu, pooled_first, defer, sink, fork_arg=None):
         ctx.sink = sink
+        ctx.fork_arg = fork_arg if (fork_arg is not None and tuple(fork_arg.shape) == (dims[0], dims[1], dims[2])
+                                    and pooled.shape[1] == dims[1]) else None
         B, Ch, M, K = dims
         Cp = pooled.shape[1]
         Cout = w2.shape[0]
@@ -598,7 +601,7 @@
     @staticmethod
     def backward(ctx, dz, _dcoef):
         if dz is None:
-            return (None,) * 17
+            return (None,) * 18
         h3, hcoef, pooled, w2, y, coef, mean, invstd, gamma = ctx.saved_tensors
         B, Ch, Cp, Cout, M, K, poff, hoff = ctx.dims
         dz = dz.contiguous().view(B, Cout, M * K)
@@ -609,6 +612,10 @@
         dpooled = dh = dw = None
         if ctx.needs_input_grad[3]:
             dpooled = ops.mlp_gemm(w2c, sdy, tag="dgrad_pooled", M=Cp, a_offset=poff)[0]
+        fork = None
+        if (ops.POOL_GRAD_FOLD and ctx.fork_arg is not None and dpooled is not None and ctx.needs_input_grad[0]
+                and bool(GRAD_SINK)):
+            fork = (dpooled.contiguous(), ctx.fork_arg, K)
         want = FUSED_NARROW_BWD and ctx.needs_input_grad[0] and ctx.needs_input_grad[4] and ctx.relu
         x2 = want and ops.layer_backward_x2_supported(Ch, Cout, M * K, (dz, y, h3), coef4, hcoef)
         fused = x2 or (want and ops.narrow_backward_supported(Ch, Cout, M * K, (dz, y, h3)))
@@ -623,7 +630,13 @@
                 _register_pre_bn_sums(res[0], [res[2]])
             dh = res[0].view(ctx.h_shape)
         if ctx.needs_input_grad[0] and not fused:
-            dh = _dgrad(h3, w2c, dz, pro=2, X2=y, coef=coef4, M=Ch, a_offset=hoff, xcoef=hcoef).view(ctx.h_shape)
+            if fork is not None and not GEMM_RED:
+                dh, _, took = ops.mlp_gemm(w2c, dz, pro=2, X2=y, coef=coef4, tag="dgrad", M=Ch, a_offset=hoff, fork=fork)
+                dh = dh.view(ctx.h_shape)
+                if took:
+                    dpooled = None
+            else:
+                dh = _dgrad(h3, w2c, dz, pro=2, X2=y, coef=coef4, M=Ch, a_offset=hoff, xcoef=hcoef).view(ctx.h_shape)
         if ctx.needs_input_grad[4] and not fused:
             dw = sink[0].view(w2c.shape) if sink else torch.empty_like(w2c)
             with ops.reduce_now(not sink):
@@ -632,7 +645,7 @@
         db = torch.zeros_like(gamma) if (ctx.needs_input_grad[5] and not sink) else None
         if sink:
             dw = db = dgamma = dbeta = None
-        return (dh, None, None, dpooled, dw, db, dgamma, dbeta) + (None,) * 9
+        return (dh, None, None, dpooled, dw, db, dgamma, dbeta) + (None,) * 10
 
 
 def conv1x1_bn_act_pooled(h, pooled: torch.Tensor, weight: torch.Tensor, bias: Optional[torch.Tensor], bn,
@@ -646,11 +659,13 @@
         e = pooled.unsqueeze(3).expand(-1, -1, -1, K)
         return conv1x1_bn_act(torch.cat((e, ht) if pooled_first else (ht, e), dim=1), weight, bias, bn, relu,
                               defer=defer)
-    hcoef = None
+    hcoef = fork_arg = None
     if isinstance(h, LazyAct):
         if not h.relu:
             h = h.materialize()
         else:
+            if h.fork is not None and h.fork[0] is pooled:
+                fork_arg = h.fork[1]
             h, hcoef = h.y, h.coef
     require_device(h, "the shared MLP")
     w2 = weight.reshape(weight.shape[0], weight.shape[1])
@@ -658,7 +673,7 @@
         bn.num_batches_tracked.add_(1)
     out, coef = _SharedMLPLayerPooled.apply(h, hcoef, tuple(hshape), pooled, w2, bias, bn.weight, bn.bias,
                                             bn.running_mean, bn.running_var, True, bn.momentum, bn.eps, relu,
-                                            pooled_first, defer, _sink(weight, bias, bn.weight, bn.bias))
+                                            pooled_first, defer, _sink(weight, bias, bn.weight, bn.bias), fork_arg)
     oshape = (hshape[0], w2.shape[0], hshape[2], K)
     return LazyAct(out, coef, relu, oshape) if defer else out.view(oshape)
 
@@ -733,10 +748,11 @@
         ctx.K = y4.shape[3]
         ctx.relu = bool(relu)
         ctx.set_materialize_grads(False)
-        return pooled, y4.view_as(y4)
-
-    @staticmethod
-    def backward(ctx, dpooled, dy):
+        ctx.mark_non_differentiable(arg)
+        return pooled, y4.view_as(y4), arg
+
+    @staticmethod
+    def backward(ctx, dpooled, dy, _darg=None):
         arg, y4, coef, yarg = ctx.saved_tensors
         if dpooled is None:
             return dy, None, None
@@ -756,8 +772,8 @@
 
 def group_max_fork(z):
     if isinstance(z, LazyAct) and _group_sums_supported(z.shape[3]):
-        pooled, y = _GroupMaxActFork.apply(z.y.view(z.shape), z.coef, z.relu)
-        return pooled, LazyAct(y.view(z.y.shape), z.coef, z.relu, z.shape)
+        pooled, y, arg = _GroupMaxActFork.apply(z.y.view(z.shape), z.coef, z.relu)
+        return pooled, LazyAct(y.view(z.y.shape), z.coef, z.relu, z.shape, fork=(pooled, arg))
     return group_max(z), z
 
 
diff --git a/usip_amd/ops.py b/usip_amd/ops.py
--- a/usip_amd/ops.py
+++ b/usip_amd/ops.py
@@ -392,12 +392,13 @@
 NARROW_FWD = _os.environ.get("USIP_NARROW_FWD", "1") not in ("0", "off")
 X2R = _os.environ.get("USIP_X2R", "1") not in ("0", "off")
 X2R_NARROW = _os.environ.get("USIP_X2R_NARROW", "1") not in ("0", "off")
+POOL_GRAD_FOLD = _os.environ.get("USIP_POOL_GRAD_FOLD", "1") not in ("0", "off")
 
 
 def mlp_gemm(At: torch.Tensor, X: torch.Tensor, bias=None, want_stats: bool = False, pro: int = 0,
              X2=None, coef=None, tag: str = "fwd", rowbias=None, rb_group: int = 1,
              M: Optional[int] = None, a_offset: int = 0, pool=None, a_trans: bool = False, out=None,
-             out_row_offset: int = 0, red=None, red_group: int = 0):
+             out_row_offset: int = 0, red=None, red_group: int = 0, fork=None):
     _need(At, "At", torch.float32)
     if a_trans:
         M_rows, lda = At.shape
@@ -446,7 +447,7 @@
                                                               _opt(rowbias), int(rb_group), y_ptr, int(y_rows),
                                                               _opt(stats), M, K, P, nb, _stream(X)),
                        "usip_mlp_narrow_forward_f32")
-        return (Y, stats, None) if red is not None else (Y, stats)
+        return (Y, stats, None) if red is not None else ((Y, stats, False) if fork is not None else (Y, stats))
     fn_name = {"bf16": "usip_mlp_gemm_bf16", "f32x3": "usip_mlp_gemm_f32x3",
                "f32x2": "usip_mlp_gemm_f32x3"}.get(_matmul_mode, "usip_mlp_gemm_f32")
     x3 = _x3_family() and (x2r_direct or bool(_lib.lib().usip_mlp_gemm_f32x3_used(M, K, P, nb)))
@@ -479,7 +480,7 @@
                                                         _opt(pool_dp), _opt(pool_arg), int(pool_group), y_ptr,
                                                         int(y_rows), _opt(stats), M, K, P, nb, _stream(X)),
                        "usip_mlp_gemm_x2r_f32")
-            return (Y, stats, None) if red is not None else (Y, stats)
+            return (Y, stats, None) if red is not None else ((Y, stats, False) if fork is not None else (Y, stats))
         red_tiles = 0
         if (red is not None and x2h and not x2r and pro >= 2 and out is None and bias is None and rowbias is None
                 and red[1] is not None and red[1].shape[0] >= 4 and tuple(red[0].shape) == (nb, M, P)
@@ -496,19 +497,32 @@
             r = RedSums(flat, M, blocks=red_tiles)
             r.gsum = gsum
             return Y, stats, r
+        if (fork is not None and x2h and pro == 2 and red is None and bias is None and rowbias is None and not want_stats
+                and POOL_GRAD_FOLD):
+            f_dp, f_arg, f_group = fork
+            _need(f_dp, "fork dpooled", torch.float32)
+            _need(f_arg, "fork arg", torch.int32)
+            if (f_group > 0 and P % f_group == 0 and tuple(f_dp.shape) == (nb, M, P // f_group) and f_arg.shape == f_dp.shape
+                    and f_dp.data_ptr() % 16 == 0 and f_arg.data_ptr() % 16 == 0 and X.data_ptr() % 16 == 0
+                    and X2.data_ptr() % 16 == 0 and y_ptr.value % 16 == 0
+                    and _lib.lib().usip_mlp_gemm_x2h_fork_supported(M, K, P, nb, int(f_group))):
+                _lib.check(_lib.lib().usip_mlp_gemm_x2h_fork_f32(_ptr(planes), _ptr(X), _ptr(X2), _ptr(coef), y_ptr,
+                                                                 int(y_rows), _ptr(f_dp), _ptr(f_arg), int(f_group), M, K, P,
+                                                                 nb, _stream(X)), "usip_mlp_gemm_x2h_fork_f32")
+                return Y, stats, True
         if x3p:
             fn = "usip_mlp_gemm_x2h_f32" if x2h else "usip_mlp_gemm_x3p_f32"
             _lib.check(getattr(_lib.lib(), fn)(_ptr(planes), None if pool is not None else _ptr(X), _opt(X2),
                                                _opt(coef), int(pro), _opt(bias), _opt(rowbias), int(rb_group),
                                                _opt(pool_dp), _opt(pool_arg), int(pool_group), y_ptr,
                                                int(y_rows), _opt(stats), M, K, P, nb, _stream(X)), fn)
-            return (Y, stats, None) if red is not None else (Y, stats)
+            return (Y, stats, None) if red is not None else ((Y, stats, False) if fork is not None else (Y, stats))
         _lib.check(getattr(_lib.lib(), fn_name)(a_ptr, -lda if a_trans else lda,
                                                 None if pool is not None else _ptr(X), _opt(X2),
                                                 _opt(coef), int(pro), _opt(bias), _opt(rowbias), int(rb_group),
                                                 _opt(pool_dp), _opt(pool_arg), int(pool_group),
                                                 y_ptr, int(y_rows), _opt(stats), M, K, P, nb, _stream(X)), fn_name)
-    return (Y, stats, None) if red is not None else (Y, stats)
+    return (Y, stats, None) if red is not None else ((Y, stats, False) if fork is not None else (Y, stats))
 
 
 def bn_finalize(stats, count, gamma, beta, eps, momentum, running_mean, running_var):
```

After: 3817 point-clouds/s, median of 6. 1.01x the previous value.
